# chriskery/slurm-bridge-operator

Measured on AMD Instinct MI355X. Metric: placements/sec + job×node fit evals/sec, 100k nodes×1M jobs, 1–8 MI355X, higher is better.
Workload: dtype int32

## Files before the change

include/fitgpu.h:

```cpp
#ifndef FITGPU_H
#define FITGPU_H

#include <stddef.h>
#include <stdint.h>

#ifdef __cplusplus
extern "C" {
#endif

#define FITGPU_ABI_VERSION 8

#define FIT_OK 0
#define FIT_E_INVAL (-1)
#define FIT_E_HIP (-2)
#define FIT_E_RCCL (-3)
#define FIT_E_OOM (-4)
#define FIT_E_NODEV (-5)
#define FIT_E_STATE (-6)
#define FIT_E_PARSE (-7)
#define FIT_E_UNLIMITED (-8)

#define FIT_UNPLACED (-1)
#define FIT_REJECTED (-2)

// ... 264 lines not shown
    int32_t need;
    int32_t evict_nodes;
    int32_t victims;
    int32_t top_prio;
    int32_t members;
    int32_t fit;
    int32_t able;
    int32_t outranked;
    int32_t reserved;
} fit_evict_k;
int fit_preempt_k(fit_ctx* ctx, int32_t j, const int32_t* cpu, const int32_t* mem, const int32_t* gpu,
                  const int32_t* wall, const uint16_t* part, const uint16_t* nodes_k ,
                  const int32_t* prio, int32_t kmax, fit_evict_k* out, int32_t* out_node ,
                  int32_t* out_victims );
int fit_preempt_k_device(fit_ctx* ctx, int32_t j, const int32_t* cpu, const int32_t* mem, const int32_t* gpu,
                         const int32_t* wall, const uint16_t* part, const uint16_t* nodes_k, const int32_t* prio,
                         int32_t kmax, fit_evict_k* out, int32_t* out_node, int32_t* out_victims);
int fit_preempt_k_ms(fit_ctx* ctx, double* ms);
int fit_preempt_k_message(const fit_evict_k* r, char* buf, int32_t buflen);

int fit_load_victims_tl(fit_ctx* ctx, const int32_t* vic_off , const int32_t* vic_prio,
                        const int32_t* vic_end, const int32_t* vic_cpu, const int32_t* vic_mem,
                        const int32_t* vic_gpu);
int fit_load_victims_tl_device(fit_ctx* ctx, const int32_t* vic_off, int64_t n_vic, const int32_t* vic_prio,
                               const int32_t* vic_end, const int32_t* vic_cpu, const int32_t* vic_mem,
                               const int32_t* vic_gpu);

int fit_preempt_tl(fit_ctx* ctx, int32_t j, const int32_t* cpu, const int32_t* mem, const int32_t* gpu,
                   const int32_t* wall, const uint16_t* part, const int32_t* prio, fit_evict* out);
int fit_preempt_tl_device(fit_ctx* ctx, int32_t j, const int32_t* cpu, const int32_t* mem, const int32_t* gpu,
                          const int32_t* wall, const uint16_t* part, const int32_t* prio, fit_evict* out);
int fit_preempt_tl_ms(fit_ctx* ctx, double* ms);

typedef struct {
    int64_t cpu, mem, gpu;
    int32_t nodes;
    int32_t max_cpu, max_mem, max_gpu;
} fit_free;
int fit_free_tl(fit_ctx* ctx, int32_t parts, fit_free* out );
int fit_free_tl_device(fit_ctx* ctx, int32_t parts, fit_free* out);
int fit_free_tl_ms(fit_ctx* ctx, double* ms);
int fit_free_message(const fit_free* r, char* buf, int32_t buflen);

int fit_parse_duration(const char* s, int64_t* out_ns);

typedef struct {
    int64_t nodes, mem_per_node, cpu_per_node, wall_ns;
} fit_resources;
int fit_parse_resources(const char* text, fit_resources* out);

typedef struct {
    int64_t cpus, memory, gpus, allo_cpus, allo_memory, allo_gpus;
} fit_node;
int fit_parse_nodes(const char* text, fit_node* out, int32_t cap);
int fit_parse_partition(const char* text, char* buf, int32_t buflen);
int fit_parse_partitions_names(const char* text, char* buf, int32_t buflen);

typedef struct {
    int64_t nodes, cpus_per_task, ntasks, ntasks_per_node, mem_per_cpu, wall_ns;
    char array[64];
} fit_job_resources;
int fit_extract_batch_resources(const char* script, fit_job_resources* out);
void fit_apply_spec(fit_job_resources* r, int64_t nodes, int64_t cpus_per_task,
                    int64_t mem_per_cpu, int64_t ntasks_per_node, const char* array,
                    int64_t ntasks);
int64_t fit_array_len(const char* array);
void fit_pod_request(const fit_job_resources* r, int64_t* cpu, int64_t* memory);
int fit_job_demand(const fit_job_resources* r, int32_t* cpu, int32_t* mem_mib, int32_t* wall_min,
                   uint16_t* nodes_k);
void fit_partition_capacity(const fit_node* nodes, int32_t n, int64_t* cpu, int64_t* memory,
                            int64_t* gpu, int64_t* pods);

int fit_ingest_nodes(const char* text, const char* partitions, int32_t np, int32_t cap,
                     int32_t* cpu_free, int32_t* mem_free, int32_t* gpu_free, int32_t* avail_min,
                     uint32_t* part_mask, char* names, int32_t names_len);
int fit_expand_hostlist(const char* expr, char* buf, int32_t buflen);
int fit_node_names(const char* entries, int32_t n, char* buf, int32_t buflen);

typedef struct fit_admitter fit_admitter;
typedef struct {
    int64_t priority;
    int32_t cpu;
    int32_t mem_mib;
    int32_t gpu;
    int32_t wall_min;
    uint16_t part;
    uint16_t nodes_k;
    uint16_t flags;
    uint16_t reserved;
} fit_admit_req;
#define FIT_REQ_ARRAY 1
typedef struct {
    int32_t node[FIT_MAX_K];
    int64_t batch;
    int32_t batch_jobs;
    int32_t order;
    int64_t ticket;
} fit_admit_res;
int fit_admitter_create(fit_ctx* ctx, int32_t max_batch, int32_t max_wait_us, fit_admitter** out);
int fit_admit(fit_admitter* a, const fit_admit_req* req, fit_admit_res* res);
int fit_admit_group(fit_admitter* a, const fit_admit_req* reqs, int32_t n, fit_admit_res* res);
int fit_admitter_load_nodes(fit_admitter* a, int32_t n, const int32_t* cpu_free,
                            const int32_t* mem_free, const int32_t* gpu_free,
                            const int32_t* avail_min, const uint32_t* part_mask);
#define FIT_TABLE_STATE 1
#define FIT_TABLE_PIN 2
typedef struct {
    int32_t n;
    const int32_t* cpu_free;
    const int32_t* mem_free;
    const int32_t* gpu_free;
    const int32_t* avail_min;
    const uint32_t* part_mask;
    const char* names;
    int32_t flags;
    int64_t generation;
} fit_node_table;
int fit_admitter_load_table(fit_admitter* a, const fit_node_table* t);
int64_t fit_admitter_generation(fit_admitter* a);
int fit_admitter_script(fit_admitter* a, const int64_t* tickets, int32_t n, const char* script,
                        char* out, int32_t outlen, int32_t* pinned);
int fit_admitter_partition_free(fit_admitter* a, int32_t p, int64_t* cpu, int64_t* mem_mib,
                                int64_t* gpu);
int fit_admitter_confirm(fit_admitter* a, int64_t ticket);
int fit_admitter_release(fit_admitter* a, int64_t ticket);
int fit_admitter_set_ttl(fit_admitter* a, int32_t loads);
int fit_admitter_explain(fit_admitter* a, const fit_admit_req* reqs, int32_t n, fit_why* out);
int fit_admitter_room(fit_admitter* a, const fit_admit_req* reqs, int32_t n, struct fit_room* out);
int fit_admitter_reservations(fit_admitter* a);
int fit_admitter_pending(fit_admitter* a);
void fit_admitter_destroy(fit_admitter* a);

typedef struct {
    const char* nodes;
    const char* cpus_per_task;
    const char* mem_per_cpu;
    const char* ntasks_per_node;
    const char* array;
    const char* ntasks;
} fit_pod_labels;
int fit_array_tasks(const char* array, int64_t* tasks, int64_t* max_running);
int32_t fit_set_max_array_size(int32_t n);
int fit_pod_demand(const fit_pod_labels* labels, const char* script, uint16_t part,
                   int64_t priority, fit_admit_req* out, int32_t cap);
int fit_script_with_nodelist(const char* script, const char* names, int32_t n_names,
                             const int32_t* node, int32_t k, char* out, int32_t outlen);
int fit_partition_limits(int64_t wall_time_s, int64_t cpu_per_node, int64_t mem_per_node,
                         int32_t* max_time_min, int32_t* max_cpus_per_node,
                         int32_t* max_mem_per_node);
int fit_node_columns(const fit_node* nodes, int32_t n, uint32_t part_mask, int32_t* cpu_free,
                     int32_t* mem_free, int32_t* gpu_free, int32_t* avail_min,
                     uint32_t* mask);

#ifdef __cplusplus
}
#endif
#endif
```

slurm-bridge-operator_amd/csrc/engine.cpp:

```cpp
#include <errno.h>
#include <fcntl.h>
#include <hip/hip_runtime_api.h>
#include <hip/hip_vector_types.h>
#include <rccl/rccl.h>
#include <sys/file.h>
#include <sys/stat.h>
#include <unistd.h>

#include <algorithm>
#include <chrono>
#include <cstdarg>
#include <cstdio>
#include <cstdlib>
#include <cstring>
#include <initializer_list>
#include <map>
#include <mutex>
#include <new>
#include <string>
#include <vector>

#include "../../include/fitgpu.h"
#include "fit_device.h"

// ... 33 lines not shown
            return fail(FIT_E_RCCL, "%s failed: %s", #expr, ncclGetErrorString(r_));        \
    } while (0)

template <class T>
struct DBuf {
    T* p = nullptr;
    size_t cap = 0;
    int ensure(size_t n) {
        if (n <= cap) return 0;
        if (p) (void)hipFree(p);
        p = nullptr;
        cap = 0;
        size_t want = std::max<size_t>(n, 64);
        if (hipMalloc(&p, want * sizeof(T)) != hipSuccess) {
            p = nullptr;
            return fail(FIT_E_OOM, "hipMalloc(%zu bytes) failed", want * sizeof(T));
        }
        cap = want;
        return 0;
    }
    void release() {
        if (p) (void)hipFree(p);
        p = nullptr;
        cap = 0;
    }
    DBuf() = default;
    DBuf(const DBuf&) = delete;
    DBuf& operator=(const DBuf&) = delete;
    ~DBuf() { release(); }
};

template <class T>
struct HBuf {
    T* p = nullptr;
    size_t cap = 0;
    int ensure(size_t n) {
        if (n <= cap) return 0;
        if (p) (void)hipHostFree(p);
        p = nullptr;
        cap = 0;
        size_t want = std::max<size_t>(n, 64);
        if (hipHostMalloc(&p, want * sizeof(T), hipHostMallocDefault) != hipSuccess) {
            p = nullptr;
            return fail(FIT_E_OOM, "hipHostMalloc(%zu bytes) failed", want * sizeof(T));
        }
        cap = want;
        return 0;
    }
    void release() {
        if (p) (void)hipHostFree(p);
        p = nullptr;
        cap = 0;
    }
    HBuf() = default;
    HBuf(const HBuf&) = delete;
    HBuf& operator=(const HBuf&) = delete;
    ~HBuf() { release(); }
};

template <class Row>
struct QueryBufs {
    DBuf<Row> out;
    DBuf<int32_t> bad;
    HBuf<Row> h;
    double ms = -1;
};

int find_root(int* par, int x) {
    while (par[x] != x) x = par[x] = par[par[x]];
    return x;
}

double now_ms() {
    using namespace std::chrono;
    return duration<double, std::milli>(steady_clock::now().time_since_epoch()).count();
}

struct DevArb {
    std::mutex mu;
    int fd = -1;
    std::string path;
};

constexpr const char* FIT_LOCK_DIR_DEFAULT = "/var/run/fitgpu";
int resolve_lock_dir(std::string& dir) {
    const char* e = getenv("FIT_LOCK_DIR");
    if (e && *e) {
        dir = e;
        return 0;
    }
    struct stat sb;
    if (stat(FIT_LOCK_DIR_DEFAULT, &sb) == 0 && S_ISDIR(sb.st_mode)) {
        dir = FIT_LOCK_DIR_DEFAULT;
        return 0;
    }
    dir = "/tmp";
    return 1;
}

DevArb* dev_arb(int device, std::string& err) {
    static std::mutex m;
    static std::map<int, DevArb*> tab;
    std::lock_guard<std::mutex> g(m);
    DevArb*& a = tab[device];
    if (!a) a = new DevArb();
    if (a->fd < 0) {
        char bus[64] = {0};
        if (hipDeviceGetPCIBusId(bus, sizeof bus, device) != hipSuccess) snprintf(bus, sizeof bus, "dev%d", device);
        for (char* q = bus; *q; ++q)
            if (*q == ':' || *q == '/') *q = '_';
        std::string dir;
        (void)resolve_lock_dir(dir);
        a->path = dir + "/fitgpu-" + bus + ".lock";
        a->fd = open(a->path.c_str(), O_RDWR | O_CREAT | O_CLOEXEC, 0666);
        if (a->fd >= 0) (void)fchmod(a->fd, 0666);
        else a->fd = open(a->path.c_str(), O_RDONLY | O_CLOEXEC);
        if (a->fd < 0) {
            err = a->path + ": " + strerror(errno);
            return nullptr;
        }
    }
    return a;
}

struct ArbGuard {
    DevArb* a = nullptr;
    double waited_ms = 0;
    int take(int device) {
        const double t0 = now_ms();
        std::string err;
        DevArb* d = dev_arb(device, err);
        if (!d) return fail(FIT_E_STATE, "device lock %s (set FIT_LOCK_DIR to a writable directory)", err.c_str());
        d->mu.lock();
        int r;
        do r = flock(d->fd, LOCK_EX);
        while (r != 0 && errno == EINTR);
        if (r != 0) {
            d->mu.unlock();
            return fail(FIT_E_STATE, "flock %s: %s", d->path.c_str(), strerror(errno));
        }
        a = d;
        waited_ms = now_ms() - t0;
        return 0;
    }
    ~ArbGuard() {
        if (!a) return;
        (void)flock(a->fd, LOCK_UN);
        a->mu.unlock();
    }
};

}

struct CtxHandles {
    ncclComm_t comm = nullptr;
    hipStream_t st = nullptr;
    hipEvent_t ev[6] = {};
    hipStream_t st2 = nullptr;
    hipEvent_t ev_join = nullptr;
    unsigned* resident = nullptr;
    CtxHandles() = default;
    CtxHandles(const CtxHandles&) = delete;
    CtxHandles& operator=(const CtxHandles&) = delete;
    ~CtxHandles() {
        for (auto& e : ev)
            if (e) (void)hipEventDestroy(e);
        if (ev_join) (void)hipEventDestroy(ev_join);
        if (resident) (void)hipHostFree(resident);
        if (st2) (void)hipStreamDestroy(st2);
        if (st) (void)hipStreamDestroy(st);
        if (comm) (void)ncclCommDestroy(comm);
    }
};

struct fit_ctx : CtxHandles {
    int device = 0;
    int rank = 0, world = 1;
    int shard_mode = FIT_SHARD_AUTO;
    fit_exchange_fn xchg = nullptr;
    void* xchg_user = nullptr;
    HBuf<uint8_t> h_x;
    DBuf<uint64_t> xcount;
    bool force_coll = false;
    bool collective() const { return world > 1 || force_coll; }
    bool persistent = true;
    int32_t small_batch = 2048;
    int32_t small_direct = 128;
    bool small_args = true, sync_spin = true;
    int cls_mode = 3;
    int32_t last_multi = 0;
    bool cls_nodes_ok = false;
    int32_t cls_maxn = 0;
    DBuf<int16_t> jcls;
    DBuf<uint8_t> cls_tab;
    DBuf<int4> cls_dem;
    DBuf<int32_t> cls_n;
    DBuf<unsigned> cls_err;
    HBuf<int32_t> h_cls_n;
    HBuf<unsigned> h_cls_err;
    DBuf<int32_t> small_placed;
    HBuf<int32_t> h_small;
    DBuf<uint8_t> jpack;
    HBuf<uint8_t> h_jpack;
    QueryBufs<fit_why> ex;
    QueryBufs<fit_eta> wh;
    QueryBufs<struct fit_room> rm;
    QueryBufs<fit_eta_k> wk;
    DBuf<int32_t> wk_node, wk_diff;
    HBuf<int32_t> h_wk_node;
    DBuf<unsigned long long> wk_top;
    DBuf<int32_t> ptlk_cnt;
    HBuf<int32_t> h_ptlk;
    DBuf<int32_t> tlr_node, tlr_start, tlr_state, tlr_inv, tlr_cnt, tlr_first, tlr_fill, tlr_touched, tlr_flag, tlr_g;
    DBuf<TlWin> tlr_win;
    DBuf<unsigned long long> tlr_tot;
    HBuf<int32_t> h_tlr_g;
    HBuf<unsigned long long> h_tlr_tot;
    double utl_ms = -1, htl_ms = -1;
    DBuf<int32_t> atl_tc, atl_tm, atl_tg, atl_g;
    HBuf<int32_t> h_atl;
    double atl_ms = -1;
    DBuf<int64_t> free_acc;
    DBuf<fit_free> free_rows;
    double free_ms = -1;
    DBuf<int32_t> vs_off, vs_prio, vs_cpu, vs_mem, vs_gpu, vic_bad, voff;
    HBuf<int32_t> h_vic_bad;
    DBuf<VicEnt> vent;
    bool have_vic = false;
    QueryBufs<fit_evict> pe;
    DBuf<int32_t> pe_prio;
    HBuf<int32_t> h_pe_prio;
    DBuf<uint4> pe_part;
    QueryBufs<fit_evict_k> pk;
    DBuf<int32_t> pk_node, pk_vic;
    HBuf<int32_t> h_pk_pick;
    DBuf<int32_t> vs_end, vtl_off;
    DBuf<VicTl> vtl_ent;
    bool have_vtl = false;
    int32_t vtl_shift = 0;
    QueryBufs<fit_evict> pt;
    int cus = 256;
    DBuf<uint8_t> ectl, ering;
    DBuf<CompState> ecs;
    DBuf<CompOut> eco;
    DBuf<int64_t> ebusy;
    HBuf<CompState> h_ecs;
    HBuf<CompOut> h_eco;
    HBuf<int64_t> h_ebusy;
    HBuf<uint32_t> h_err;
    HBuf<TripRec> h_trip;
    DBuf<NodeRec> rec_bak;
    unsigned wd_ticks = 1000000000u;
    HBuf<uint64_t> h_count;
    int wmin = 256, wmax = 8192;

    int32_t n = 0;
    int32_t nn = 0;
    int ncomp = 0;
    int comp_of_part[32];
    std::vector<int32_t> nb;
    DBuf<NodeRec> rec;
    DBuf<int32_t> col_cpu, col_mem, col_gpu, col_av, perm;
    DBuf<uint32_t> col_mask;
    DBuf<int32_t> rb_cpu, rb_mem, rb_gpu;
    std::vector<uint32_t> h_mask;
    std::vector<int32_t> h_perm;
    bool have_nodes = false;
    int64_t loads = 0;

    int32_t np = 0;
    int32_t ptab[128];
    DBuf<int32_t> d_ptab;

    DBuf<int32_t> jcpu, jmem, jgpu, jwall, out, jl, jpk;
    DBuf<uint16_t> jpart, jk;
    DBuf<int8_t> jcomp;
    DBuf<int32_t> jmin;
    DBuf<uint64_t> cand, bnd;
    DBuf<JobRec> wjob;
    DBuf<CompPlan> plan;
    DBuf<CommitResult> res;
    HBuf<CompPlan> h_plan;
    HBuf<CommitResult> h_res;
    DBuf<int32_t> jls;
    HBuf<int32_t> h_jls;

    int32_t tl_slots = 0, tl_slot_min = 0;
    bool have_tl = false;
    DBuf<Seg> slab;
    DBuf<TlHdr> tlhdr;
    DBuf<int32_t> outs, rel_off, rel_slot, rel_cpu, rel_mem, rel_gpu;
    DBuf<uint32_t> tl_err;
    HBuf<uint32_t> h_tl_err;
};

namespace {

int build_ptab(fit_ctx* c) {
    for (int p = 0; p < 32; ++p) c->ptab[96 + p] = c->comp_of_part[p];
    if (c->d_ptab.ensure(128)) return FIT_E_OOM;
    HIP_TRY(hipMemcpyAsync(c->d_ptab.p, c->ptab, sizeof c->ptab, hipMemcpyHostToDevice, c->st));
    return 0;
}

int load_nodes_common(fit_ctx* c, int32_t n) {
    int par[32];
    for (int i = 0; i < 32; ++i) par[i] = i;
    bool used[32] = {false};
    for (int32_t x = 0; x < n; ++x) {
        uint32_t m = c->h_mask[x];
        if (!m) continue;
        int lo = __builtin_ctz(m);
        for (uint32_t r = m; r; r &= r - 1) {
            int b = __builtin_ctz(r);
            used[b] = true;
            int ra = find_root(par, lo), rb = find_root(par, b);
            if (ra != rb) par[std::max(ra, rb)] = std::min(ra, rb);
        }
    }
    int root_comp[32];
    for (int i = 0; i < 32; ++i) root_comp[i] = -1;
    c->ncomp = 0;
    for (int p = 0; p < 32; ++p) {
        c->comp_of_part[p] = -1;
        if (!used[p]) continue;
        int r = find_root(par, p);
        if (root_comp[r] < 0) root_comp[r] = c->ncomp++;
        c->comp_of_part[p] = root_comp[r];
    }
    c->nb.assign(c->ncomp + 1, 0);
    for (int32_t x = 0; x < n; ++x)
        if (c->h_mask[x]) c->nb[c->comp_of_part[__builtin_ctz(c->h_mask[x])] + 1]++;
    for (int k = 0; k < c->ncomp; ++k) {
        if (c->nb[k + 1] > MAX_COMPONENT_NODES)
            return fail(FIT_E_INVAL, "partition component %d has %d nodes (limit %d)", k,
                        c->nb[k + 1], MAX_COMPONENT_NODES);
        c->nb[k + 1] += c->nb[k];
    }
    c->nn = c->nb[c->ncomp];
    {
        int parts_of[32] = {0};
        for (int p = 0; p < 32; ++p)
            if (c->comp_of_part[p] >= 0) ++parts_of[c->comp_of_part[p]];
        c->cls_nodes_ok = c->ncomp > 0 && c->ncomp <= 32;
        c->cls_maxn = 0;
        for (int k = 0; k < c->ncomp; ++k) {
            const int32_t nk = c->nb[k + 1] - c->nb[k];
            c->cls_maxn = std::max(c->cls_maxn, nk);
            if (parts_of[k] != 1) c->cls_nodes_ok = false;
        }
        if (c->cls_maxn > class_max_nodes() || class_lds_bytes(c->cls_maxn) > 160 * 1024)
            c->cls_nodes_ok = false;
    }
    std::vector<int32_t> fill(c->nb.begin(), c->nb.end() - 1), perm(std::max(c->nn, 1));
    for (int32_t x = 0; x < n; ++x)
        if (c->h_mask[x]) perm[fill[c->comp_of_part[__builtin_ctz(c->h_mask[x])]]++] = x;
    if (c->perm.ensure(std::max(c->nn, 1)) || c->rec.ensure(std::max(c->nn, 1))) return FIT_E_OOM;
    HIP_TRY(hipMemcpyAsync(c->perm.p, perm.data(), sizeof(int32_t) * c->nn, hipMemcpyHostToDevice,
                           c->st));
    HIP_TRY(launch_gather_nodes(c->st, c->col_cpu.p, c->col_mem.p, c->col_gpu.p, c->col_av.p,
                                c->col_mask.p, c->perm.p, c->nn, c->rec.p));
    int rc = build_ptab(c);
    if (rc) return rc;
    HIP_TRY(hipStreamSynchronize(c->st));
    perm.resize(c->nn);
    c->h_perm.swap(perm);
    c->n = n;
    c->have_nodes = true;
    c->have_tl = false;
    ++c->loads;
    return 0;
}

int alloc_cols(fit_ctx* c, int32_t n) {
    size_t m = std::max<int32_t>(n, 1);
    if (c->col_cpu.ensure(m) || c->col_mem.ensure(m) || c->col_gpu.ensure(m) ||
        c->col_av.ensure(m) || c->col_mask.ensure(m))
        return FIT_E_OOM;
    return 0;
}

int xchg(fit_ctx* c, int op, void* dbuf, int64_t count) {
    if (!c->collective() || count == 0) return 0;
    if (!c->xchg) {
        switch (op) {
            case FIT_XCHG_ALLGATHER_U64: {
                uint64_t* b = static_cast<uint64_t*>(dbuf);
                NCCL_TRY(ncclAllGather(b + (size_t)c->rank * count, b, count, ncclUint64, c->comm,
                                       c->st));
                return 0;
            }
            case FIT_XCHG_MIN_U64:
                NCCL_TRY(ncclAllReduce(dbuf, dbuf, count, ncclUint64, ncclMin, c->comm, c->st));
                return 0;
            case FIT_XCHG_MAX_I32:
                NCCL_TRY(ncclAllReduce(dbuf, dbuf, count, ncclInt32, ncclMax, c->comm, c->st));
                return 0;
            case FIT_XCHG_MIN_I32:
                NCCL_TRY(ncclAllReduce(dbuf, dbuf, count, ncclInt32, ncclMin, c->comm, c->st));
                return 0;
        }
        return fail(FIT_E_INVAL, "exchange op %d", op);
    }
    const size_t elem = (op == FIT_XCHG_ALLGATHER_U64 || op == FIT_XCHG_MIN_U64) ? 8 : 4;
    const size_t bytes = elem * (size_t)count * (op == FIT_XCHG_ALLGATHER_U64 ? c->world : 1);
    if (c->h_x.ensure(bytes)) return FIT_E_OOM;
    HIP_TRY(hipMemcpyAsync(c->h_x.p, dbuf, bytes, hipMemcpyDeviceToHost, c->st));
    HIP_TRY(hipStreamSynchronize(c->st));
    if (c->xchg(c->xchg_user, op, c->h_x.p, count) != 0)
        return fail(FIT_E_RCCL, "host exchange op %d failed", op);
    HIP_TRY(hipMemcpyAsync(dbuf, c->h_x.p, bytes, hipMemcpyHostToDevice, c->st));
    return 0;
}

const char* trip_site_name(unsigned s) {
    switch (s) {
        case TRIP_WORKER_RING: return "scan worker waiting for a task";
        case TRIP_ROUND_START: return "committer waiting for the round before last";
        case TRIP_HELPER_TILE: return "commit helper waiting for a scan tile";
        case TRIP_HELPER_SNAP: return "commit helper waiting for the decider";
        case TRIP_DECIDER_REC: return "decider waiting for a helper record";
        case TRIP_SINGLE_TILE: return "single-wave commit waiting for a scan tile";
        case TRIP_NO_PROGRESS: return "round resolved no job";
        case TRIP_NO_KERNEL: return "no scan kernel for the key count";
        default: return "unknown";
    }
}

int trip_error(fit_ctx* c, const char* engine) {
    const TripRec& t = *c->h_trip.p;
    return fail(FIT_E_HIP,
                "%s watchdog tripped (code %u): site %u (%s), component %u, round %u, arg %u, "
                "block %u, q_head %u, q_tail %u, pubt %u, tdone %u / need %u, waited %.3f ms, "
                "%.3f ms into the launch (deadline %.3f ms)",
                engine, c->h_err.p[0], t.site, trip_site_name(t.site), t.comp, t.round, t.arg,
                t.block, t.q_head, t.q_tail, t.pubt, t.tdone, t.need, t.waited / 1e5, t.when / 1e5,
                c->wd_ticks / 1e5);
}
struct EngineComps {
    std::vector<int> comps;
    int nc = 0;
    int32_t maxnodes = 0;
    int64_t wcap = 0;
};

EngineComps engine_comps(fit_ctx* c, const std::vector<int32_t>& jb, const std::vector<char>& owned) {
    EngineComps E;
    for (int k = 0; k < c->ncomp; ++k)
        if (owned[k] && jb[k + 1] > jb[k]) {
            E.comps.push_back(k);
            E.maxnodes = std::max(E.maxnodes, c->nb[k + 1] - c->nb[k]);
        }
    E.nc = (int)E.comps.size();
    E.wcap = std::min(c->wmax, 8192);
    return E;
}

int fold_comp_out(fit_ctx* c, const std::vector<int32_t>& jb, const std::vector<int>& comps, fit_stats& S) {
    double commit_max = 0;
    for (size_t i = 0; i < comps.size(); ++i) {
        const CompOut& o = c->h_eco.p[i];
        const int k = comps[i];
        if (o.done_jobs != jb[k + 1] - jb[k])
            return fail(FIT_E_HIP, "component %d resolved %lld of %d jobs", k, (long long)o.done_jobs,
                        jb[k + 1] - jb[k]);
        S.placed += o.placed;
        S.rounds = std::max<int64_t>(S.rounds, o.rounds);
        S.stops_rescan += o.stops_rescan;
        S.stops_dirty += o.stops_dirty;
        commit_max = std::max(commit_max, o.t_commit / 1e5);
    }
    S.ms_commit += commit_max;
    return 0;
}

template <class Slice>
int engine_plan(fit_ctx* c, const std::vector<int32_t>& jb, const EngineComps& E, int64_t keys, Slice slice) {
    const int nc = E.nc;
    const int64_t wcap = E.wcap, per_comp_cand = wcap * keys;
    if (c->ecs.ensure(nc) || c->eco.ensure(nc) || c->h_ecs.ensure(nc) || c->h_eco.ensure(nc) ||
        c->plan.ensure(2 * nc) ||
        c->cand.ensure((size_t)2 * nc * per_comp_cand + (size_t)2 * nc * PAIR_AREA) ||
        c->bnd.ensure((size_t)2 * nc * wcap) || c->wjob.ensure((size_t)2 * nc * wcap) ||
        c->ectl.ensure(engine_ctl_bytes()) || c->ering.ensure(engine_ring_bytes()) ||
        c->h_err.ensure(4))
        return FIT_E_OOM;
    if ((int64_t)2 * nc * per_comp_cand + (int64_t)2 * nc * PAIR_AREA > INT32_MAX)
        return fail(FIT_E_INVAL, "candidate buffer exceeds 2^31 entries (%d components)", nc);
    int32_t max_slices = 1;
    for (int i = 0; i < nc; ++i) {
        const int k = E.comps[i];
        CompState& s = c->h_ecs.p[i];
        s.nb = s.sb = c->nb[k];
        s.ne = s.se = c->nb[k + 1];
        slice(s.ne - s.nb, s);
        max_slices = std::max(max_slices, s.nslice);
        s.jstart = jb[k];
        s.jend = jb[k + 1];
        s.cand_off = (int64_t)i * per_comp_cand;
        s.slot0 = (int32_t)(i * wcap);
        s.cand_alt = (int64_t)(nc + i) * per_comp_cand;
        s.slot_alt = (int32_t)((nc + i) * wcap);
        s.pair_off = (int32_t)(2 * nc * per_comp_cand + (int64_t)2 * i * PAIR_AREA);
        s.wmin = std::min(c->wmin, (int)wcap);
        s.wmax = (int32_t)wcap;
    }
    if ((int64_t)2 * ring_comps(nc) * ((wcap + SCAN_JOBS - 1) / SCAN_JOBS + 1) * max_slices >
        (int64_t)engine_ring_tasks())
        return fail(FIT_E_INVAL, "task ring too small: %d components x %lld tiles x %d slices",
                    nc, (long long)((wcap + SCAN_JOBS - 1) / SCAN_JOBS), max_slices);
    return 0;
}

template <class Launch, class Settle>
int engine_launch(fit_ctx* c, const std::vector<int32_t>& jb, const EngineComps& E, int workers,
                  const char* name, Launch launch, Settle settle, fit_stats& S) {
    const int nc = E.nc;
    hipStream_t st = c->st;
    if (c->ebusy.ensure(2 * workers) || c->h_ebusy.ensure(2 * workers) || c->h_trip.ensure(1))
        return FIT_E_OOM;
    HIP_TRY(hipMemcpyAsync(c->ecs.p, c->h_ecs.p, sizeof(CompState) * nc, hipMemcpyHostToDevice, st));
    HIP_TRY(hipMemsetAsync(c->ectl.p, 0, engine_ctl_bytes(), st));
    HIP_TRY(hipMemsetAsync(c->ering.p, 0, engine_ring_bytes(), st));
    HIP_TRY(hipMemsetAsync(c->bnd.p, 0xff, sizeof(uint64_t) * 2 * nc * E.wcap, st));
    {
        ArbGuard arb;
        int rc = arb.take(c->device);
        if (rc) return rc;
        S.ms_arb_wait = arb.waited_ms;
        HIP_TRY(hipEventRecord(c->ev[0], st));
        rc = launch();
        if (rc) return rc;
        HIP_TRY(hipEventRecord(c->ev[1], st));
        HIP_TRY(hipMemcpyAsync(c->h_eco.p, c->eco.p, sizeof(CompOut) * nc, hipMemcpyDeviceToHost, st));
        HIP_TRY(hipMemcpyAsync(c->h_ebusy.p, c->ebusy.p, sizeof(int64_t) * 2 * workers,
                               hipMemcpyDeviceToHost, st));
        HIP_TRY(hipMemcpyAsync(c->h_err.p, c->ectl.p + engine_ctl_error_offset(), 4, hipMemcpyDeviceToHost, st));
        HIP_TRY(hipMemcpyAsync(c->h_trip.p, c->ectl.p + engine_ctl_trip_offset(), sizeof(TripRec),
                               hipMemcpyDeviceToHost, st));
        HIP_TRY(hipStreamSynchronize(st));
    }
    if (int rc = settle(c->h_err.p[0] ? trip_error(c, name) : 0)) return rc;
    float ms = 0.f;
    HIP_TRY(hipEventElapsedTime(&ms, c->ev[0], c->ev[1]));
    S.ms_device += ms;
    int64_t busy = 0;
    for (int i = 0; i < workers; ++i) {
        busy += c->h_ebusy.p[2 * i];
        S.evals += c->h_ebusy.p[2 * i + 1];
    }
    S.ms_scan += busy / 1e5 / workers;
    return fold_comp_out(c, jb, E.comps, S);
}

int run_persistent(fit_ctx* c, const std::vector<int32_t>& jb, const std::vector<char>& owned,
                   const int32_t* cpu, const int32_t* mem, const int32_t* gpu, const int32_t* wall,
                   const uint16_t* part, const uint16_t* nk, int32_t* out, int32_t kmax,
                   fit_stats& S) {
    hipStream_t st = c->st;
    const EngineComps E = engine_comps(c, jb, owned);
    const int nc = E.nc;
    if (nc == 0) return 0;
    int sub_target = 256, ks_min = 4;
    if (const char* e = getenv("FIT_SUB_TARGET")) sub_target = std::max(MIN_SUB, atoi(e));
    if (const char* e = getenv("FIT_KS_MIN")) ks_min = std::max(2, std::min(KS, atoi(e)));
    while (ks_min < kmax) ks_min *= 2;
    int rc = engine_plan(c, jb, E, (int64_t)MAX_SLICES * KS, [&](int32_t len, CompState& s) {
        for (s.ks = KS;; s.ks /= 2) {
            const int slices = MAX_SLICES * KS / s.ks;
            s.sub = std::max(MIN_SUB, (len + SCAN_WAVES * slices - 1) / (SCAN_WAVES * slices));
            s.nslice = std::max(1, (len + SCAN_WAVES * s.sub - 1) / (SCAN_WAVES * s.sub));
            if (s.sub <= sub_target || s.ks / 2 < ks_min) break;
        }
    });
    if (rc) return rc;
    size_t lds = engine_lds_bytes(E.maxnodes);
    if (const char* e = getenv("FIT_ENGINE_LDS_MIN")) lds = std::max(lds, (size_t)atol(e));
    int per_cu = engine_blocks_per_cu(lds);
    if (per_cu <= 0) return fail(FIT_E_HIP, "k_engine does not fit on a CU (lds %zu)", lds);
    int workers = std::max(8, std::max(1, per_cu - 1) * c->cus - nc);
    if (const char* e = getenv("FIT_WORKERS")) workers = std::max(1, atoi(e));
    EngineCompIds ids;
    memset(&ids, 0, sizeof ids);
    for (int i = 0; i < nc; ++i) ids.id[i] = (int8_t)E.comps[i];
    static const bool no_backup = getenv("FIT_REC_BACKUP") && atoi(getenv("FIT_REC_BACKUP")) == 0;
    if (c->rec_bak.ensure(std::max(c->nn, 1))) return FIT_E_OOM;
    if (!no_backup)
        HIP_TRY(hipMemcpyAsync(c->rec_bak.p, c->rec.p, sizeof(NodeRec) * c->nn, hipMemcpyDeviceToDevice, st));
    return engine_launch(
        c, jb, E, workers, "placement engine",
        [&]() -> int {
            HIP_TRY(launch_engine(nc + workers, lds, st, c->ectl.p, c->ering.p, c->ecs.p, c->eco.p,
                                  c->plan.p, nc, c->rec.p, c->jl.p, cpu, mem, gpu, wall, part, nk,
                                  c->cand.p, c->bnd.p, c->wjob.p, out, kmax, c->ebusy.p, c->jpk.p,
                                  c->wd_ticks, c->jmin.p, ids));
            return 0;
        },
        [&](int trip) -> int {
            if (!trip) return 0;
            if (no_backup) {
                c->have_nodes = c->have_tl = false;
                return trip;
            }
            HIP_TRY(hipMemcpyAsync(c->rec.p, c->rec_bak.p, sizeof(NodeRec) * c->nn, hipMemcpyDeviceToDevice, st));
            HIP_TRY(hipStreamSynchronize(st));
            return trip;
        },
        S);
}

int run_class(fit_ctx* c, int32_t J, const std::vector<int32_t>& jb, const std::vector<char>& owned,
              const int32_t* wall, const uint16_t* nk, int32_t* out, int32_t kmax, fit_stats& S) {
    const int C = c->ncomp;
    hipStream_t st = c->st;
    if (c->eco.ensure(C) || c->h_eco.ensure(C) || c->cls_err.ensure(1) || c->h_cls_err.ensure(1) ||
        c->rec_bak.ensure(std::max(c->nn, 1)))
        return FIT_E_OOM;
    int32_t* jbd = c->jls.p + joblists_scratch_ints(J) + 2;
    HIP_TRY(hipMemsetAsync(c->cls_err.p, 0, sizeof(unsigned), st));
    HIP_TRY(hipMemcpyAsync(c->rec_bak.p, c->rec.p, sizeof(NodeRec) * c->nn, hipMemcpyDeviceToDevice, st));
    const size_t lds = class_lds_bytes(c->cls_maxn);
    HIP_TRY(hipEventRecord(c->ev[0], st));
    uint32_t own = 0;
    for (int k = 0; k < C; ++k)
        if (owned[k]) own |= 1u << k;
    HIP_TRY(launch_class(st, C, lds, c->rec.p, c->nb.data(), own, jbd, c->jl.p, wall, nk, c->jcls.p,
                         c->cls_dem.p, c->cls_n.p, kmax, out, c->eco.p, c->cls_err.p));
    HIP_TRY(hipEventRecord(c->ev[1], st));
    HIP_TRY(launch_class_out(st, out, (int64_t)J * kmax, c->rec.p));
    HIP_TRY(hipMemcpyAsync(c->h_eco.p, c->eco.p, sizeof(CompOut) * C, hipMemcpyDeviceToHost, st));
    HIP_TRY(hipMemcpyAsync(c->h_cls_err.p, c->cls_err.p, sizeof(unsigned), hipMemcpyDeviceToHost, st));
    HIP_TRY(hipStreamSynchronize(st));
    if (c->h_cls_err.p[0]) {
        HIP_TRY(hipMemcpyAsync(c->rec.p, c->rec_bak.p, sizeof(NodeRec) * c->nn, hipMemcpyDeviceToDevice, st));
        HIP_TRY(hipStreamSynchronize(st));
        return fail(FIT_E_HIP, "class engine: an in-block wait exceeded its bound (error %u)", c->h_cls_err.p[0]);
    }
    float ms = 0.f;
    HIP_TRY(hipEventElapsedTime(&ms, c->ev[0], c->ev[1]));
    S.ms_device += ms;
    double commit_max = 0;
    for (int k = 0; k < C; ++k) {
        if (!owned[k]) continue;
        const CompOut& o = c->h_eco.p[k];
        if (o.done_jobs != jb[k + 1] - jb[k])
            return fail(FIT_E_HIP, "component %d resolved %lld of %d jobs", k, (long long)o.done_jobs,
                        jb[k + 1] - jb[k]);
        S.placed += o.placed;
        S.evals += o.evals;
        S.rounds = std::max<int64_t>(S.rounds, o.rounds);
        S.stops_rescan += o.stops_rescan;
        S.stops_dirty += o.stops_dirty;
        commit_max = std::max(commit_max, o.t_commit / 1e5);
    }
    S.ms_commit += commit_max;
    S.engine = 3;
    return 0;
}

int enqueue_classify(fit_ctx* c, int32_t J, const int32_t* cpu, const int32_t* mem, const int32_t* gpu,
                     const uint16_t* part) {
    const int C = c->ncomp;
    hipStream_t st = c->st;
    const size_t ts = (size_t)C * class_table_slots() * class_slot_bytes();
    if (c->jcls.ensure(std::max(J, 1)) || c->cls_tab.ensure(ts) || c->cls_dem.ensure((size_t)C * class_max()) ||
        c->cls_n.ensure(C) || c->h_cls_n.ensure(C))
        return FIT_E_OOM;
    HIP_TRY(hipMemsetAsync(c->cls_tab.p, 0, ts, st));
    HIP_TRY(hipMemsetAsync(c->cls_n.p, 0, sizeof(int32_t) * C, st));
    HIP_TRY(launch_classify(st, c->jcomp.p, cpu, mem, gpu, part, J, c->cls_tab.p, c->cls_dem.p, c->cls_n.p,
                            c->jcls.p));
    HIP_TRY(hipMemcpyAsync(c->h_cls_n.p, c->cls_n.p, sizeof(int32_t) * C, hipMemcpyDeviceToHost, st));
    return 0;
}

bool classes_fit(const fit_ctx* c) {
    for (int k = 0; k < c->ncomp; ++k)
        if (c->h_cls_n.p[k] > class_max()) return false;
    return true;
}

int build_job_lists(fit_ctx* c, int32_t J, fit_stats& S, std::vector<int32_t>& jb,
                    const int32_t* cpu = nullptr, const int32_t* mem = nullptr, const int32_t* gpu = nullptr,
                    const uint16_t* part = nullptr, bool classify = false, bool* cls_ok = nullptr) {
    const int C = c->ncomp;
    hipStream_t st = c->st;
    if (c->jl.ensure(std::max(J, 1)) || c->jpk.ensure(J + 1) ||
        c->jls.ensure(std::max<size_t>(joblists_scratch_ints(J), 1) + 2 * (C + 1) + 2) ||
        c->h_jls.ensure(2 * (C + 1) + 2))
        return FIT_E_OOM;
    int32_t* g = c->jls.p + joblists_scratch_ints(J);
    int32_t* jbd = g + 2;
    int32_t* mbd = jbd + C + 1;
    HIP_TRY(launch_joblists(st, c->jcomp.p, J, C, c->jls.p, g, jbd, mbd, c->jl.p, c->jpk.p));
    HIP_TRY(hipMemcpyAsync(c->h_jls.p, g, sizeof(int32_t) * (2 * (C + 1) + 2), hipMemcpyDeviceToHost, st));
    if (classify) {
        const int rc = enqueue_classify(c, J, cpu, mem, gpu, part);
        if (rc) return rc;
    }
    HIP_TRY(hipStreamSynchronize(st));
    if (c->h_jls.p[1]) return fail(FIT_E_INVAL, "a job has a negative demand or nodes_k > kmax");
    if (cls_ok) *cls_ok = classify && classes_fit(c);
    S.rejected = c->h_jls.p[0];
    jb.assign(c->h_jls.p + 2, c->h_jls.p + 2 + C + 1);
    c->last_multi = c->h_jls.p[2 + C + 1 + C];
    for (int k = 0; k < C; ++k) S.useful_evals += (int64_t)(jb[k + 1] - jb[k]) * c->n;
    return 0;
}

int classify_jobs(fit_ctx* c, int32_t J, const int32_t* cpu, const int32_t* mem, const int32_t* gpu,
                  const uint16_t* part, bool* cls_ok) {
    const int rc = enqueue_classify(c, J, cpu, mem, gpu, part);
    if (rc) return rc;
    HIP_TRY(hipStreamSynchronize(c->st));
    *cls_ok = classes_fit(c);
    return 0;
}

hipError_t sync_small(fit_ctx* c) {
    if (c->sync_spin) {
        hipError_t e = hipEventRecord(c->ev[2], c->st);
        if (e != hipSuccess) return e;
        const double t0 = now_ms();
        while ((e = hipEventQuery(c->ev[2])) == hipErrorNotReady && now_ms() - t0 < 2.0) {
        }
        if (e != hipErrorNotReady) return e;
    }
    return hipStreamSynchronize(c->st);
}

int place_direct(fit_ctx* c, int32_t J, const int32_t* cpu, const int32_t* mem, const int32_t* gpu,
                 const int32_t* wall, const uint16_t* part, const uint16_t* nk, int32_t kmax,
                 int32_t* out, int32_t* h_out, fit_stats& S, const SmallBatch* hb = nullptr) {
    const int C = c->ncomp;
    const int G = std::max(C, 1);
    hipStream_t st = c->st;
    const size_t rows = (size_t)J * kmax;
    const size_t nback = (h_out ? rows : 0) + 2 + G;
    if (c->small_placed.ensure(2 + G) || c->h_small.ensure(nback)) return FIT_E_OOM;
    int32_t* stat = h_out ? out + rows : c->small_placed.p;
    SmallComps sc;
    for (int k = 0; k <= 32; ++k) sc.nb[k] = c->nb[std::min(k, C)];
    HIP_TRY(hipEventRecord(c->ev[0], st));
    if (hb)
        HIP_TRY(launch_small_args(st, C, c->rec.p, sc, c->d_ptab.p, c->np, *hb, nk != nullptr, J, kmax, out, stat));
    else
        HIP_TRY(launch_small(st, C, c->rec.p, sc, c->d_ptab.p, c->np, cpu, mem, gpu, wall, part, nk, J, kmax,
                             out, stat));
    HIP_TRY(hipEventRecord(c->ev[1], st));
    HIP_TRY(hipMemcpyAsync(c->h_small.p, h_out ? out : stat, sizeof(int32_t) * nback, hipMemcpyDeviceToHost,
                           st));
    HIP_TRY(sync_small(c));
    const int32_t* hs = c->h_small.p + (h_out ? rows : 0);
    if (hs[1]) return fail(FIT_E_INVAL, "a job has a negative demand or nodes_k > kmax");
    if (h_out) memcpy(h_out, c->h_small.p, sizeof(int32_t) * rows);
    S.rejected = hs[0];
    for (int k = 0; k < C; ++k) S.placed += hs[2 + k];
    float ms = 0.f;
    HIP_TRY(hipEventElapsedTime(&ms, c->ev[0], c->ev[1]));
    S.ms_device = S.ms_commit = ms;
    S.rounds = C > 0 && J > S.rejected ? 1 : 0;
    S.components = C;
    S.engine = 2;
    return 0;
}

template <class Scan, class Commit>
int run_rounds(fit_ctx* c, const std::vector<int32_t>& jb, const std::vector<char>& owned, bool node_sharded,
               int keys, int slices, int min_sub, Scan scan, Commit commit, fit_stats& S) {
    const int C = c->ncomp;
    hipStream_t st = c->st;
    const int shards = node_sharded ? c->world : 1;
    const int srank = node_sharded ? c->rank : 0;
    std::vector<int32_t> cur(jb.begin(), jb.end() - 1), win(C, c->wmin);
    if (c->plan.ensure(C + 1) || c->res.ensure(C + 1) || c->h_plan.ensure(C + 1) ||
        c->h_res.ensure(C + 1))
        return FIT_E_OOM;
    float ms;
    for (;;) {
        int64_t blocks = 0, slots = 0, cand_n = 0, evals = 0;
        int epl = 1;
        int32_t maxlen = 0;
        for (int k = 0; k < C; ++k) {
            CompPlan& P = c->h_plan.p[k];
            memset(&P, 0, sizeof P);
            P.nb = c->nb[k];
            P.ne = c->nb[k + 1];
            const int32_t len = P.ne - P.nb;
            const int32_t per = (len + shards - 1) / shards;
            P.sb = std::min(P.ne, P.nb + per * srank);
            P.se = std::min(P.ne, P.sb + per);
            P.ks = keys;
            P.sub = std::max(min_sub, (per + SCAN_WAVES * slices - 1) / (SCAN_WAVES * slices));
            P.nslice = std::max(1, (per + SCAN_WAVES * P.sub - 1) / (SCAN_WAVES * P.sub));
            epl = std::max(epl, (shards * P.nslice * keys + 63) / 64);
            P.jbase = cur[k];
            P.w = owned[k] ? std::min(win[k], jb[k + 1] - cur[k]) : 0;
            P.blk0 = (int32_t)blocks;
            P.cand_off = cand_n;
            P.slot0 = (int32_t)slots;
            if (P.w > 0) {
                blocks += (int64_t)((P.w + SCAN_JOBS - 1) / SCAN_JOBS) * P.nslice;
                cand_n += (int64_t)P.w * P.nslice * keys;
                slots += P.w;
                evals += (int64_t)P.w * (P.se - P.sb);
                maxlen = std::max(maxlen, len);
            }
        }
        if (slots == 0) break;
        S.rounds++;
        S.evals += evals;
        if (c->cand.ensure((size_t)cand_n * shards) || c->bnd.ensure(slots) ||
            c->wjob.ensure(slots))
            return FIT_E_OOM;
        HIP_TRY(hipMemcpyAsync(c->plan.p, c->h_plan.p, sizeof(CompPlan) * C, hipMemcpyHostToDevice,
                               st));
        HIP_TRY(hipMemsetAsync(c->bnd.p, 0xff, sizeof(uint64_t) * slots, st));
        HIP_TRY(hipEventRecord(c->ev[0], st));
        HIP_TRY(scan((int)blocks, c->cand.p + (size_t)srank * cand_n));
        HIP_TRY(hipEventRecord(c->ev[1], st));
        if (node_sharded) {
            int rc = xchg(c, FIT_XCHG_ALLGATHER_U64, c->cand.p, cand_n);
            if (!rc) rc = xchg(c, FIT_XCHG_MIN_U64, c->bnd.p, slots);
            if (rc) return rc;
        }
        HIP_TRY(hipEventRecord(c->ev[2], st));
        HIP_TRY(commit(epl, maxlen, cand_n, shards));
        HIP_TRY(hipEventRecord(c->ev[3], st));
        HIP_TRY(hipMemcpyAsync(c->h_res.p, c->res.p, sizeof(CommitResult) * C,
                               hipMemcpyDeviceToHost, st));
        HIP_TRY(hipStreamSynchronize(st));
        HIP_TRY(hipEventElapsedTime(&ms, c->ev[0], c->ev[1]));
        S.ms_scan += ms;
        HIP_TRY(hipEventElapsedTime(&ms, c->ev[1], c->ev[2]));
        S.ms_exchange += ms;
        HIP_TRY(hipEventElapsedTime(&ms, c->ev[2], c->ev[3]));
        S.ms_commit += ms;
        for (int k = 0; k < C; ++k) {
            const CompPlan& P = c->h_plan.p[k];
            if (P.w == 0) continue;
            const CommitResult& R = c->h_res.p[k];
            if (R.done < 0 || R.done > P.w)
                return fail(FIT_E_HIP, "commit returned %d of window %d", R.done, P.w);
            cur[k] += R.done;
            S.placed += R.placed;
            if (R.stop == 1) S.stops_rescan++;
            if (R.stop == 2) S.stops_dirty++;
            const int32_t nw = R.stop ? 2 * R.done : 2 * P.w;
            win[k] = std::max(c->wmin, std::min(c->wmax, nw));
        }
    }
    S.ms_device = S.ms_scan + S.ms_exchange + S.ms_commit;
    return 0;
}

int place_impl(fit_ctx* c, int32_t J, const int32_t* cpu, const int32_t* mem, const int32_t* gpu,
               const int32_t* wall, const uint16_t* part, const uint16_t* nk, int32_t kmax,
               int32_t* out, fit_stats* stats, int32_t* h_out = nullptr, bool* h_out_done = nullptr,
               const SmallBatch* hb = nullptr) {
    const double t0 = now_ms();
    fit_stats S;
    memset(&S, 0, sizeof S);
    S.jobs = J;
    hipStream_t st = c->st;
    if (J <= c->small_direct && !c->collective()) {
        const int rc = place_direct(c, J, cpu, mem, gpu, wall, part, nk, kmax, out, h_out, S, hb);
        if (rc) return rc;
        if (h_out_done) *h_out_done = h_out != nullptr;
        S.unplaced = J - S.placed - S.rejected;
        S.ms_total = now_ms() - t0;
        if (stats) *stats = S;
        return 0;
    }
    if (c->jcomp.ensure(std::max(J, 1)) || c->jmin.ensure(3 * ENGINE_MAXC)) return FIT_E_OOM;
    HIP_TRY(hipMemsetAsync(c->jmin.p, JMIN_FILL, sizeof(int32_t) * 3 * ENGINE_MAXC, st));
    HIP_TRY(launch_prefilter(st, cpu, mem, gpu, wall, part, nk, J, kmax, c->d_ptab.p, c->np, out,
                             c->jcomp.p, c->jmin.p));
    const int C = c->ncomp;
    std::vector<int32_t> jb;
    const int pre_mode = !c->collective() ? 0
                         : (c->shard_mode == FIT_SHARD_AUTO ? (C >= c->world ? FIT_SHARD_COMPONENTS : FIT_SHARD_NODES)
                                                            : c->shard_mode);
    const bool cls_able = c->cls_nodes_ok && pre_mode != FIT_SHARD_NODES;
    const bool try_cls = (c->cls_mode == 1 || c->cls_mode == 2) && cls_able && (c->cls_mode == 2 || J > c->small_batch);
    bool cls_ok = false;
    int rc0 = build_job_lists(c, J, S, jb, cpu, mem, gpu, part, try_cls, &cls_ok);
    if (rc0) return rc0;
    const int32_t live = J - S.rejected;
    if (c->cls_mode == 3 && cls_able && live > c->small_batch && 2 * (int64_t)c->last_multi >= live) {
        rc0 = classify_jobs(c, J, cpu, mem, gpu, part, &cls_ok);
        if (rc0) return rc0;
    }
    const bool use_cls = cls_ok && (c->cls_mode == 2 || live > c->small_batch);

    int mode = 0;
    std::vector<char> owned(C, 1);
    if (c->collective()) {
        mode = c->shard_mode;
        if (mode == FIT_SHARD_AUTO) mode = C >= c->world ? FIT_SHARD_COMPONENTS : FIT_SHARD_NODES;
        if (mode == FIT_SHARD_COMPONENTS) {
            std::vector<int> order(C);
            for (int k = 0; k < C; ++k) order[k] = k;
            auto work = [&](int k) { return (int64_t)(jb[k + 1] - jb[k]) * (c->nb[k + 1] - c->nb[k]); };
            std::stable_sort(order.begin(), order.end(), [&](int a, int b) { return work(a) > work(b); });
            std::vector<int64_t> load(c->world, 0);
            for (int k : order) {
                int r = (int)(std::min_element(load.begin(), load.end()) - load.begin());
                load[r] += work(k) + 1;
                owned[k] = r == c->rank;
            }
        }
    }
    S.shard_mode = mode;
    S.components = C;
    const bool node_sharded = mode == FIT_SHARD_NODES;

    const bool small = J - S.rejected <= c->small_batch;
    if (use_cls) {
        int rc = run_class(c, J, jb, owned, wall, nk, out, kmax, S);
        if (rc) return rc;
    } else if (c->persistent && !node_sharded && !small) {
        int rc = run_persistent(c, jb, owned, cpu, mem, gpu, wall, part, nk, out, kmax, S);
        if (rc) return rc;
        S.engine = 1;
    } else {
        int rc = run_rounds(
            c, jb, owned, node_sharded, KS, MAX_SLICES, MIN_SUB,
            [&](int blocks, uint64_t* cand) {
                return launch_scan(blocks, st, c->rec.p, c->jl.p, cpu, mem, gpu, wall, part, nk, c->plan.p, C,
                                   cand, c->bnd.p, c->wjob.p);
            },
            [&](int epl, int32_t maxlen, int64_t cand_n, int shards) {
                return launch_commit(C, epl, (size_t)((maxlen + 31) / 32) * 4, st, c->rec.p, c->plan.p,
                                     c->cand.p, cand_n, shards, c->bnd.p, c->wjob.p, out, kmax, c->res.p);
            },
            S);
        if (rc) return rc;
    }
    if (mode == FIT_SHARD_COMPONENTS) {
        int rc = xchg(c, FIT_XCHG_MAX_I32, out, (int64_t)J * kmax);
        if (!rc) rc = xchg(c, FIT_XCHG_MIN_I32, c->rec.p, (int64_t)c->nn * 8);
        if (rc) return rc;
        if (c->xcount.ensure(c->world) || c->h_count.ensure(c->world)) return FIT_E_OOM;
        c->h_count.p[c->rank] = (uint64_t)S.placed;
        HIP_TRY(hipMemcpyAsync(c->xcount.p + c->rank, c->h_count.p + c->rank, 8,
                               hipMemcpyHostToDevice, st));
        rc = xchg(c, FIT_XCHG_ALLGATHER_U64, c->xcount.p, 1);
        if (rc) return rc;
        HIP_TRY(hipMemcpyAsync(c->h_count.p, c->xcount.p, 8 * c->world, hipMemcpyDeviceToHost, st));
        HIP_TRY(hipStreamSynchronize(st));
        S.placed = 0;
        for (int r = 0; r < c->world; ++r) S.placed += (int64_t)c->h_count.p[r];
    }
    S.unplaced = J - S.placed - S.rejected;
    S.ms_total = now_ms() - t0;
    if (stats) *stats = S;
    return 0;
}

int run_persistent_tl(fit_ctx* c, const std::vector<int32_t>& jb, const int32_t* cpu,
                      const int32_t* mem, const int32_t* gpu, const int32_t* wall,
                      const uint16_t* part, int32_t* out, int32_t* outs, fit_stats& S) {
    hipStream_t st = c->st;
    const EngineComps E = engine_comps(c, jb, std::vector<char>(c->ncomp, 1));
    const int nc = E.nc;
    if (nc == 0) return 0;
    const int R = engine_tl_runs(E.maxnodes);
    if (R < 1) return fail(FIT_E_INVAL, "partition component of %d nodes is too large for the "
                                        "timeline engine's LDS", E.maxnodes);
    int slices = TL_SLICES, tl_min_sub = TL_MIN_SUB;
    if (const char* e = getenv("FIT_TL_SLICES")) slices = std::max(1, std::min(atoi(e), TL_SLICES));
    if (const char* e = getenv("FIT_TL_MINSUB")) tl_min_sub = std::max(1, atoi(e));
    int rc = engine_plan(c, jb, E, (int64_t)slices * TL_KS, [&](int32_t len, CompState& s) {
        s.ks = TL_KS;
        s.sub = std::max(tl_min_sub, (len + SCAN_WAVES * slices - 1) / (SCAN_WAVES * slices));
        s.nslice = std::max(1, (len + SCAN_WAVES * s.sub - 1) / (SCAN_WAVES * s.sub));
    });
    if (rc) return rc;
    const size_t lds = engine_tl_lds_bytes(E.maxnodes);
    bool split = FIT_TL_SPLIT_DEF != 0;
    if (const char* e = getenv("FIT_TL_SPLIT")) split = atoi(e) != 0;
    const size_t lds_w = split ? engine_tl_scan_lds_bytes() : lds;
    const int per_cu = engine_tl_blocks_per_cu(lds, split ? 1 : 0);
    if (per_cu <= 0) return fail(FIT_E_HIP, "k_engine_tl does not fit on a CU (lds %zu)", lds);
    const int per_cu_w = split ? engine_tl_blocks_per_cu(lds_w, 2) : per_cu;
    if (per_cu_w <= 0) return fail(FIT_E_HIP, "k_engine_tl workers do not fit on a CU");
    int workers = split ? std::max(8, per_cu_w * std::max(1, c->cus - nc)) : std::max(8, per_cu * c->cus - nc);
    if (const char* e = getenv("FIT_WORKERS")) workers = std::max(1, atoi(e));
    if (split && !c->st2) {
        if (hipStreamCreateWithFlags(&c->st2, hipStreamNonBlocking) != hipSuccess ||
            hipEventCreateWithFlags(&c->ev_join, hipEventDisableTiming) != hipSuccess ||
            hipHostMalloc(&c->resident, 64, hipHostMallocMapped | hipHostMallocCoherent) != hipSuccess)
            return fail(FIT_E_HIP, "split launch: stream / event / mapped flag");
    }
    auto launch = [&](int blocks, size_t l, hipStream_t s, int mode, unsigned* dres) {
        return launch_engine_tl(blocks, l, s, c->ectl.p, c->ering.p, c->ecs.p, c->eco.p, c->plan.p, nc,
                                c->slab.p, c->tlhdr.p, c->jl.p, cpu, mem, gpu, wall, part, c->cand.p,
                                c->bnd.p, c->wjob.p, c->perm.p, out, outs, c->tl_slots, c->tl_slot_min, R,
                                c->ebusy.p, mode, dres, c->wd_ticks);
    };
    bool resident_late = false;
    rc = engine_launch(
        c, jb, E, workers, "timeline engine",
        [&]() -> int {
            if (!split) {
                HIP_TRY(launch(nc + workers, lds, st, 0, nullptr));
                return 0;
            }
            __atomic_store_n(c->resident, 0u, __ATOMIC_RELEASE);
            unsigned* dres = nullptr;
            HIP_TRY(hipHostGetDevicePointer(reinterpret_cast<void**>(&dres), c->resident, 0));
            HIP_TRY(launch(nc, lds, st, 1, dres));
            const auto t0 = std::chrono::steady_clock::now();
            while (__atomic_load_n(c->resident, __ATOMIC_ACQUIRE) < (unsigned)nc) {
                if (std::chrono::steady_clock::now() - t0 > std::chrono::seconds(10)) {
                    resident_late = true;
                    break;
                }
            }
            HIP_TRY(hipStreamWaitEvent(c->st2, c->ev[0], 0));
            HIP_TRY(launch(workers, lds_w, c->st2, 2, nullptr));
            HIP_TRY(hipEventRecord(c->ev_join, c->st2));
            HIP_TRY(hipStreamWaitEvent(st, c->ev_join, 0));
            return 0;
        },
        [&](int trip) -> int {
            if (trip || resident_late) c->have_tl = false;
            if (trip) return trip;
            if (resident_late) return fail(FIT_E_HIP, "timeline engine: committer blocks not resident after 10 s");
            return 0;
        },
        S);
    if (rc) return rc;
    S.engine = 1;
    return 0;
}

int place_tl_impl(fit_ctx* c, int32_t J, const int32_t* cpu, const int32_t* mem,
                  const int32_t* gpu, const int32_t* wall, const uint16_t* part, int32_t* out,
                  int32_t* outs, fit_stats* stats) {
    const double t0 = now_ms();
    fit_stats S;
    memset(&S, 0, sizeof S);
    S.jobs = J;
    hipStream_t st = c->st;
    if (c->jcomp.ensure(std::max(J, 1))) return FIT_E_OOM;
    HIP_TRY(launch_prefilter(st, cpu, mem, gpu, wall, part, nullptr, J, 1, c->d_ptab.p, c->np, out,
                             c->jcomp.p));
    if (J > 0) HIP_TRY(hipMemsetAsync(outs, 0xff, sizeof(int32_t) * J, st));
    const int C = c->ncomp;
    std::vector<int32_t> jb;
    int rc = build_job_lists(c, J, S, jb);
    if (rc) return rc;
    const bool node_sharded = c->collective();
    S.shard_mode = node_sharded ? FIT_SHARD_NODES : 0;
    S.components = C;
    if (c->persistent && !node_sharded && J - S.rejected > c->small_batch) {
        rc = run_persistent_tl(c, jb, cpu, mem, gpu, wall, part, out, outs, S);
        if (rc) return rc;
        S.unplaced = J - S.placed - S.rejected;
        S.ms_total = now_ms() - t0;
        if (stats) *stats = S;
        return 0;
    }
    int32_t maxlen = 1;
    for (int k = 0; k < C; ++k) maxlen = std::max(maxlen, c->nb[k + 1] - c->nb[k]);
    const size_t lds = commit_tl_lds_bytes(maxlen);
    const int runs = commit_tl_runs(maxlen);
    const int shards = node_sharded ? c->world : 1;
    int slices = std::max(1, TL_SLICES / shards), tl_min_sub = TL_MIN_SUB;
    if (const char* e = getenv("FIT_TL_SLICES")) slices = std::max(1, std::min(atoi(e), 512 / (TL_KS * shards)));
    if (const char* e = getenv("FIT_TL_MINSUB")) tl_min_sub = std::max(1, atoi(e));
    if (runs < 1)
        return fail(FIT_E_INVAL, "partition component of %d nodes is too large for the timeline "
                                 "commit's LDS", maxlen);
// ... 26 lines not shown
constexpr int32_t kExplainSortJobs = 256;

struct JobCols {
    const int32_t *cpu, *mem, *gpu, *wall;
    const uint16_t *part, *nk;
};

ExplainComps query_comps(const fit_ctx* c) {
    ExplainComps ec;
    ec.ncomp = c->ncomp;
    for (int k = 0; k <= 32; ++k) ec.nb[k] = c->nb[std::min(k, c->ncomp)];
    return ec;
}
int query_joblist(fit_ctx* c, int32_t J, int32_t threshold, const int32_t** jl, const int32_t** live) {
    const int C = c->ncomp;
    *jl = *live = nullptr;
    if (J <= threshold || C <= 1) return 0;
    if (c->jl.ensure(J) || c->jpk.ensure(J + 1) ||
        c->jls.ensure(std::max<size_t>(joblists_scratch_ints(J), 1) + 2 * (C + 1) + 2))
        return FIT_E_OOM;
    int32_t* g = c->jls.p + joblists_scratch_ints(J);
    int32_t* jbd = g + 2;
    HIP_TRY(launch_joblists(c->st, c->jcomp.p, J, C, c->jls.p, g, jbd, jbd + C + 1, c->jl.p, c->jpk.p));
    *jl = c->jl.p;
    *live = jbd + C;
    return 0;
}

template <class Classify, class Walk>
int query_impl(fit_ctx* c, int32_t J, int32_t* bad, Classify classify, Walk walk) {
    if (c->jcomp.ensure(std::max(J, 1))) return FIT_E_OOM;
    HIP_TRY(hipMemsetAsync(bad, 0, sizeof(int32_t), c->st));
    HIP_TRY(classify());
    const int32_t *jl, *live;
    if (const int rc = query_joblist(c, J, kExplainSortJobs, &jl, &live)) return rc;
    HIP_TRY(walk(query_comps(c), jl, live));
    return 0;
}

int explain_impl(fit_ctx* c, int32_t J, const JobCols& d, fit_why* out, int32_t* bad) {
    return query_impl(
        c, J, bad,
        [&] {
            return launch_explain_classify(c->st, c->d_ptab.p, c->np, d.cpu, d.mem, d.gpu, d.wall, d.part, d.nk, J,
                                           out, c->jcomp.p, bad);
        },
        [&](const ExplainComps& ec, const int32_t* jl, const int32_t* live) {
            return launch_explain(c->st, c->rec.p, ec, d.cpu, d.mem, d.gpu, d.wall, d.part, J, c->jcomp.p, jl, live,
                                  explain_slices(J, c->cls_maxn, c->cus), out);
        });
}

static_assert(ETA_NOW == FIT_ETA_NOW && ETA_PARTITION == FIT_ETA_PARTITION && ETA_LIMIT_TIME == FIT_ETA_LIMIT_TIME &&
                  ETA_LIMIT_CPUS == FIT_ETA_LIMIT_CPUS && ETA_LIMIT_MEM == FIT_ETA_LIMIT_MEM &&
                  ETA_NO_NODES == FIT_ETA_NO_NODES && ETA_LATER == FIT_ETA_LATER && ETA_HORIZON == FIT_ETA_HORIZON,
              "fit_device.h and fitgpu.h disagree");
static_assert(sizeof(fit_eta) == 32, "fit_eta is 32 bytes");
constexpr int kWhenMinNodes = 4;

int when_impl(fit_ctx* c, int32_t J, const JobCols& d, fit_eta* out, int32_t* bad) {
    return query_impl(
        c, J, bad,
        [&] {
            return launch_when_classify(c->st, c->d_ptab.p, c->np, d.cpu, d.mem, d.gpu, d.wall, d.part, J,
                                        c->tl_slot_min, out, c->jcomp.p, bad);
        },
        [&](const ExplainComps& ec, const int32_t* jl, const int32_t* live) {
            return launch_when(c->st, c->tlhdr.p, c->slab.p, ec, c->tl_slots, c->tl_slot_min, d.cpu, d.mem, d.gpu,
                               d.part, J, c->jcomp.p, jl, live,
                               explain_slices(J, c->cls_maxn, c->cus, kWhenMinNodes), out);
        });
}

static_assert(ROOM_SOME == FIT_ROOM_SOME && ROOM_PARTITION == FIT_ROOM_PARTITION &&
                  ROOM_LIMIT_TIME == FIT_ROOM_LIMIT_TIME && ROOM_LIMIT_CPUS == FIT_ROOM_LIMIT_CPUS &&
                  ROOM_LIMIT_MEM == FIT_ROOM_LIMIT_MEM && ROOM_NO_NODES == FIT_ROOM_NO_NODES &&
                  ROOM_NONE == FIT_ROOM_NONE,
              "fit_device.h and fitgpu.h disagree");
static_assert(sizeof(struct fit_room) == 40 && offsetof(struct fit_room, copies) == 16 &&
                  offsetof(struct fit_room, best_node) == 24,
              "fit_room is 40 bytes, copies at 16");
static_assert(FIT_ROOM_UNBOUNDED == INT32_MAX, "FIT_ROOM_UNBOUNDED is INT32_MAX");

int room_impl(fit_ctx* c, int32_t J, const JobCols& d, struct fit_room* out, int32_t* bad) {
    return query_impl(
        c, J, bad,
        [&] {
            return launch_room_classify(c->st, c->d_ptab.p, c->np, d.cpu, d.mem, d.gpu, d.wall, d.part, J, out,
                                        c->jcomp.p, bad);
        },
        [&](const ExplainComps& ec, const int32_t* jl, const int32_t* live) {
            return launch_room(c->st, c->rec.p, ec, d.cpu, d.mem, d.gpu, d.wall, d.part, J, c->jcomp.p, jl, live,
                               explain_slices(J, c->cls_maxn, c->cus), out);
        });
}

static_assert(PRE_FITS == FIT_PRE_FITS && PRE_PARTITION == FIT_PRE_PARTITION && PRE_LIMIT_TIME == FIT_PRE_LIMIT_TIME &&
                  PRE_LIMIT_CPUS == FIT_PRE_LIMIT_CPUS && PRE_LIMIT_MEM == FIT_PRE_LIMIT_MEM &&
                  PRE_NO_NODES == FIT_PRE_NO_NODES && PRE_EVICT == FIT_PRE_EVICT && PRE_NONE == FIT_PRE_NONE,
              "fit_device.h and fitgpu.h disagree");
static_assert(FIT_PRE_PARTITION == FIT_WHY_PARTITION && FIT_PRE_LIMIT_TIME == FIT_WHY_LIMIT_TIME &&
                  FIT_PRE_LIMIT_CPUS == FIT_WHY_LIMIT_CPUS && FIT_PRE_LIMIT_MEM == FIT_WHY_LIMIT_MEM &&
                  FIT_PRE_NO_NODES == FIT_WHY_NO_NODES,
              "codes 1..5 of FIT_PRE_* are FIT_WHY_*'s");
static_assert(sizeof(fit_evict) == 32 && offsetof(fit_evict, code) == 0 && offsetof(fit_evict, node) == 4 &&
                  offsetof(fit_evict, victims) == 8 && offsetof(fit_evict, top_prio) == 12 &&
                  offsetof(fit_evict, members) == 16 && offsetof(fit_evict, fit) == 20 &&
                  offsetof(fit_evict, able) == 24 && offsetof(fit_evict, outranked) == 28,
              "fit_evict is 32 bytes: code, node, victims, top_prio, then the four counters");

int preempt_impl(fit_ctx* c, int32_t J, const JobCols& d, const int32_t* prio, fit_evict* out, int32_t* bad) {
    const int S = preempt_slices(J, c->cls_maxn, c->cus);
    if (c->pe_part.ensure(preempt_partials(J, S))) return FIT_E_OOM;
    return query_impl(
        c, J, bad,
        [&] {
            return launch_preempt_classify(c->st, c->d_ptab.p, c->np, c->ncomp, d.cpu, d.mem, d.gpu, d.wall, d.part, J,
                                           out, c->jcomp.p, bad);
        },
        [&](const ExplainComps& ec, const int32_t* jl, const int32_t* live) {
            return launch_preempt(c->st, c->rec.p, c->voff.p, c->vent.p, ec, d.cpu, d.mem, d.gpu, d.wall, d.part, prio,
                                  J, c->jcomp.p, jl, live, S, c->pe_part.p, out);
        });
}

static_assert(sizeof(fit_evict_k) == 40 && offsetof(fit_evict_k, code) == 0 && offsetof(fit_evict_k, need) == 4 &&
                  offsetof(fit_evict_k, evict_nodes) == 8 && offsetof(fit_evict_k, victims) == 12 &&
                  offsetof(fit_evict_k, top_prio) == 16 && offsetof(fit_evict_k, members) == 20 &&
                  offsetof(fit_evict_k, fit) == 24 && offsetof(fit_evict_k, able) == 28 &&
                  offsetof(fit_evict_k, outranked) == 32 && offsetof(fit_evict_k, reserved) == 36,
              "fit_evict_k is 40 bytes: code, need, evict_nodes, victims, top_prio, the four counters, reserved");

int preempt_k_impl(fit_ctx* c, int32_t J, const JobCols& d, const int32_t* prio, int32_t kmax, fit_evict_k* out,
                   int32_t* out_node, int32_t* out_vic, int32_t* bad) {
    const int S = preempt_slices(J, c->cls_maxn, c->cus);
    if (c->pe_part.ensure(preempt_k_partials(J, S, kmax))) return FIT_E_OOM;
    return query_impl(
        c, J, bad,
        [&] {
            return launch_preempt_k_classify(c->st, c->d_ptab.p, c->np, c->ncomp, d.cpu, d.mem, d.gpu, d.wall, d.part,
                                             d.nk, kmax, J, out, out_node, out_vic, c->jcomp.p, bad);
        },
        [&](const ExplainComps& ec, const int32_t* jl, const int32_t* live) {
            return launch_preempt_k(c->st, c->rec.p, c->voff.p, c->vent.p, ec, d.cpu, d.mem, d.gpu, d.wall, d.part,
                                    prio, kmax, J, c->jcomp.p, jl, live, S, c->pe_part.p, out, out_node, out_vic);
        });
}

int load_victims_impl(fit_ctx* c, const int32_t* h_off, const int32_t* off, const int32_t* prio, const int32_t* cpu,
                      const int32_t* mem, const int32_t* gpu) {
    std::vector<int32_t> hv((size_t)c->nn + 1, 0);
    if (h_off)
        for (int32_t i = 0; i < c->nn; ++i) {
            const int32_t x = c->h_perm[i];
            hv[i + 1] = hv[i] + (h_off[x + 1] - h_off[x]);
        }
    c->have_vic = false;
    if (c->voff.ensure(hv.size()) || c->vent.ensure(std::max<int32_t>(hv[c->nn], 1))) return FIT_E_OOM;
    HIP_TRY(hipMemcpyAsync(c->voff.p, hv.data(), sizeof(int32_t) * hv.size(), hipMemcpyHostToDevice, c->st));
    if (hv[c->nn] > 0)
        HIP_TRY(launch_vic_build(c->st, off, prio, cpu, mem, gpu, c->perm.p, c->nn, c->voff.p, c->vent.p));
    HIP_TRY(hipStreamSynchronize(c->st));
    c->have_vic = true;
    return 0;
}

int check_victims_state(fit_ctx* c) {
    if (!c) return fail(FIT_E_INVAL, "null ctx");
    if (!c->have_nodes) return fail(FIT_E_STATE, "fit_load_nodes not called");
    if (c->collective())
        return fail(FIT_E_STATE, "fit_load_victims on a sharded context (world > 1 / FIT_FLAG_COLLECTIVES)");
    return 0;
}

int preempt_tl_impl(fit_ctx* c, int32_t J, const JobCols& d, const int32_t* prio, fit_evict* out, int32_t* bad) {
    const int S = preempt_slices(J, c->cls_maxn, c->cus);
    if (c->pe_part.ensure(preempt_partials(J, S))) return FIT_E_OOM;
    return query_impl(
        c, J, bad,
        [&] {
            return launch_preempt_classify(c->st, c->d_ptab.p, c->np, c->ncomp, d.cpu, d.mem, d.gpu, d.wall, d.part, J,
                                           out, c->jcomp.p, bad);
        },
        [&](const ExplainComps& ec, const int32_t* jl, const int32_t* live) {
            return launch_preempt_tl(c->st, c->tlhdr.p, c->slab.p, c->vtl_off.p, c->vtl_ent.p, ec, c->tl_slots,
                                     c->tl_slot_min, c->vtl_shift, d.cpu, d.mem, d.gpu, d.wall, d.part, prio, J,
                                     c->jcomp.p, jl, live, S, c->pe_part.p, out);
        });
}

int load_victims_tl_impl(fit_ctx* c, const int32_t* h_off, const int32_t* off, const int32_t* prio, const int32_t* end,
                         const int32_t* cpu, const int32_t* mem, const int32_t* gpu) {
    std::vector<int32_t> hv((size_t)c->nn + 1, 0);
    if (h_off)
        for (int32_t i = 0; i < c->nn; ++i) {
            const int32_t x = c->h_perm[i];
            hv[i + 1] = hv[i] + (h_off[x + 1] - h_off[x]);
        }
    c->have_vtl = false;
    if (c->vtl_off.ensure(hv.size()) || c->vtl_ent.ensure(std::max<int32_t>(hv[c->nn], 1))) return FIT_E_OOM;
    HIP_TRY(hipMemcpyAsync(c->vtl_off.p, hv.data(), sizeof(int32_t) * hv.size(), hipMemcpyHostToDevice, c->st));
    if (hv[c->nn] > 0)
        HIP_TRY(launch_vtl_build(c->st, off, prio, end, cpu, mem, gpu, c->perm.p, c->nn, c->vtl_off.p, c->vtl_ent.p));
    HIP_TRY(hipStreamSynchronize(c->st));
    c->vtl_shift = 0;
    c->have_vtl = true;
    return 0;
}

int check_victims_tl_state(fit_ctx* c) {
    if (!c) return fail(FIT_E_INVAL, "null ctx");
    if (!c->have_nodes) return fail(FIT_E_STATE, "fit_load_nodes not called");
    if (c->collective())
        return fail(FIT_E_STATE, "fit_load_victims_tl on a sharded context (world > 1 / FIT_FLAG_COLLECTIVES)");
    if (!c->have_tl) return fail(FIT_E_STATE, "fit_load_timeline not called");
    return 0;
}

static_assert(sizeof(fit_eta_k) == 40 && offsetof(fit_eta_k, members) == 20 && offsetof(fit_eta_k, reserved) == 36,
              "fit_eta_k is 40 bytes");

int whenk_slices(int32_t nj, int32_t maxn, int cus) {
    const int64_t groups = ((int64_t)std::max(nj, 1) + WHENK_GROUP - 1) / WHENK_GROUP;
    const int64_t want = std::max<int64_t>(2, ((int64_t)cus * 4 + groups - 1) / groups);
    const int64_t fit = ((int64_t)maxn + 255) / 256;
    return (int)std::max<int64_t>(1, std::min<int64_t>({want, fit, (int64_t)WHENK_MAX_SLICES}));
}

int when_k_impl(fit_ctx* c, int32_t J, const JobCols& d, int32_t kmax, fit_eta_k* out, int32_t* out_node,
                int32_t* bad) {
    hipStream_t st = c->st;
    const int C = c->ncomp, H = c->tl_slots;
    const int32_t chunk = std::min<int32_t>(J, WHENK_CHUNK);
    const int S = whenk_slices(chunk, c->cls_maxn, c->cus);
    if (c->jcomp.ensure(std::max(J, 1)) || c->wk_diff.ensure((size_t)chunk * (H + 1)) ||
        c->wk_top.ensure((size_t)chunk * S * WHENK_KEYS))
        return FIT_E_OOM;
    HIP_TRY(hipMemsetAsync(bad, 0, sizeof(int32_t), st));
    HIP_TRY(launch_whenk_classify(st, c->d_ptab.p, c->np, d.cpu, d.mem, d.gpu, d.wall, d.part, d.nk, kmax, J,
                                  c->tl_slot_min, out, out_node, c->jcomp.p, bad));
    if (C < 1) return 0;
    const int32_t *jl, *live;
    if (const int rc = query_joblist(c, J, WHENK_GROUP, &jl, &live)) return rc;
    const ExplainComps ec = query_comps(c);
    for (int32_t t0 = 0; t0 < J; t0 += WHENK_CHUNK)
        HIP_TRY(launch_whenk_chunk(st, c->tlhdr.p, c->slab.p, ec, H, c->tl_slot_min, d.cpu, d.mem, d.gpu, d.wall,
                                   d.part, t0, std::min<int32_t>(J - t0, WHENK_CHUNK), J, kmax, c->jcomp.p, jl, live, S,
                                   c->wk_diff.p, c->wk_top.p, out, out_node));
    return 0;
}

struct TlBack {
    void* host = nullptr;
    const void* dev = nullptr;
    size_t bytes = 0;
};
constexpr int kTlNoWrite = 1;

template <class Check, class Verdict, class Write>
int tl_write_impl(fit_ctx* c, const char* name, TlBack flags, Check check, Verdict verdict, TlBack result, Write write,
                  double* dev_ms) {
    hipStream_t st = c->st;
    float ms = 0.f;
    *dev_ms = 0;
    if (flags.bytes) {
        HIP_TRY(hipEventRecord(c->ev[0], st));
        HIP_TRY(check());
        HIP_TRY(hipEventRecord(c->ev[1], st));
        HIP_TRY(hipMemcpyAsync(flags.host, flags.dev, flags.bytes, hipMemcpyDeviceToHost, st));
        HIP_TRY(hipStreamSynchronize(st));
        const int rc = verdict();
        if (rc < 0) return rc;
        HIP_TRY(hipEventElapsedTime(&ms, c->ev[0], c->ev[1]));
        *dev_ms = ms;
        if (rc == kTlNoWrite) return 0;
    }
    HIP_TRY(hipEventRecord(c->ev[3], st));
    int kept = 0;
    hipError_t e = write(kept);
    if (e != hipSuccess && kept) return kept;
    if (e == hipSuccess) e = hipEventRecord(c->ev[4], st);
    if (e == hipSuccess && result.bytes)
        e = hipMemcpyAsync(result.host, result.dev, result.bytes, hipMemcpyDeviceToHost, st);
    if (e == hipSuccess) e = hipStreamSynchronize(st);
    if (e == hipSuccess) e = hipEventElapsedTime(&ms, c->ev[3], c->ev[4]);
    if (e != hipSuccess) {
        c->have_tl = false;
        return fail(FIT_E_HIP, "%s: %s; the timeline is dropped (fit_load_timeline)", name, hipGetErrorString(e));
    }
    *dev_ms += ms;
    return 0;
}

int place_tl_k_impl(fit_ctx* c, int32_t J, const JobCols& d, int32_t kmax, int32_t* out, int32_t* outs,
                    fit_stats* stats) {
    const double t0 = now_ms();
    fit_stats S;
    memset(&S, 0, sizeof S);
    S.jobs = J;
    S.engine = 4;
    const int C = c->ncomp, H = c->tl_slots;
    S.components = C;
    hipStream_t st = c->st;
    const size_t ns = 2 * ((size_t)C + 1) + 2;
    if (c->jcomp.ensure(J) || c->jl.ensure(J) || c->jpk.ensure((size_t)J + 1) ||
        c->jls.ensure(std::max<size_t>(joblists_scratch_ints(J), 1) + ns) || c->h_jls.ensure(ns) ||
        c->ptlk_cnt.ensure(1) || c->h_ptlk.ensure(1))
        return FIT_E_OOM;
    int32_t* g = c->jls.p + joblists_scratch_ints(J);
    int32_t* jbd = g + 2;
    int32_t maxlen = 0;
    int32_t chunk = PTLK_CHUNK;
    if (const char* e = getenv("FIT_PTLK_CHUNK")) chunk = std::max(1, std::min(atoi(e), PTLK_CHUNK));
    const int rc = tl_write_impl(
        c, "fit_place_tl_k", {c->h_jls.p, g, sizeof(int32_t) * ns},
        [&] {
            hipError_t e = launch_ptlk_classify(st, c->d_ptab.p, c->np, d.cpu, d.mem, d.gpu, d.wall, d.part, d.nk, kmax,
                                                J, out, outs, c->jcomp.p);
            if (e == hipSuccess)
                e = launch_joblists(st, c->jcomp.p, J, C, c->jls.p, g, jbd, jbd + C + 1, c->jl.p, c->jpk.p);
            return e;
        },
        [&]() -> int {
            if (c->h_jls.p[1]) return fail(FIT_E_INVAL, "a job has a negative demand or nodes_k > kmax");
            S.rejected = c->h_jls.p[0];
            for (int k = 0; k < C; ++k) maxlen = std::max(maxlen, c->h_jls.p[2 + k + 1] - c->h_jls.p[2 + k]);
            if (maxlen <= 0) return kTlNoWrite;
            HIP_TRY(hipMemsetAsync(c->ptlk_cnt.p, 0, sizeof(int32_t), st));
            return 0;
        },
        {c->h_ptlk.p, c->ptlk_cnt.p, sizeof(int32_t)},
        [&](int& kept) {
            const int threads = ptlk_threads(c->cls_maxn);
            const ExplainComps ec = query_comps(c);
            hipError_t e = hipSuccess;
            int32_t done = 0;
            for (; done < maxlen && e == hipSuccess; done += chunk)
                e = launch_ptlk_commit(st, threads, c->tlhdr.p, c->slab.p, ec, H, c->tl_slot_min, c->jl.p, jbd, done,
                                       chunk, d.cpu, d.mem, d.gpu, d.wall, d.part, d.nk, kmax, out, outs,
                                       c->ptlk_cnt.p);
            if (e != hipSuccess && done <= chunk)
                kept = fail(FIT_E_HIP, "k_ptlk_commit launch failed: %s", hipGetErrorString(e));
            return e;
        },
        &S.ms_device);
    if (rc) return rc;
    if (maxlen > 0) S.placed = c->h_ptlk.p[0];
    S.unplaced = J - S.placed - S.rejected;
    S.ms_total = now_ms() - t0;
// ... 200 lines not shown
}

template <class Row, class Impl, class Bad>
int query_device(fit_ctx* c, QueryBufs<Row>& Q, int32_t j, const JobCols& d, Row* out, Impl impl, Bad bad) {
    HIP_TRY(hipSetDevice(c->device));
    if (Q.bad.ensure(1) || Q.h.ensure(1)) return FIT_E_OOM;
    HIP_TRY(hipEventRecord(c->ev[0], c->st));
    const int rc = impl(c, j, d, out, Q.bad.p);
    if (rc) return rc;
    HIP_TRY(hipEventRecord(c->ev[1], c->st));
    HIP_TRY(hipMemcpyAsync(Q.h.p, Q.bad.p, sizeof(int32_t), hipMemcpyDeviceToHost, c->st));
    HIP_TRY(hipStreamSynchronize(c->st));
    if (Q.h.p[0].code) return bad();
    float ms = 0.f;
    HIP_TRY(hipEventElapsedTime(&ms, c->ev[0], c->ev[1]));
    Q.ms = ms;
    return 0;
}

int bad_explain_job() { return fail(FIT_E_INVAL, "a job has a negative demand or nodes_k > %d", FIT_MAX_K); }
int bad_when_job() { return fail(FIT_E_INVAL, "a job has a negative demand"); }
int bad_room_job() { return fail(FIT_E_INVAL, "a job has a negative demand"); }

int load_timeline_impl(fit_ctx* c, int32_t slots, int32_t slot_min, int64_t ne) {
    if (c->tlhdr.ensure(std::max(c->nn, 1)) ||
        c->slab.ensure((size_t)std::max(c->nn, 1) * TL_MAX_SLOTS) || c->tl_err.ensure(1) ||
        c->h_tl_err.ensure(1))
        return FIT_E_OOM;
    c->have_vtl = false;
    HIP_TRY(hipMemsetAsync(c->tl_err.p, 0, 4, c->st));
    HIP_TRY(launch_build_tl(c->st, c->col_cpu.p, c->col_mem.p, c->col_gpu.p, c->col_av.p,
                            c->col_mask.p, c->perm.p, c->nn, slots, slot_min, ne >= 0 ? c->rel_off.p : nullptr,
                            c->rel_slot.p, c->rel_cpu.p, c->rel_mem.p, c->rel_gpu.p, c->slab.p,
                            c->tlhdr.p, c->tl_err.p));
    HIP_TRY(hipMemcpyAsync(c->h_tl_err.p, c->tl_err.p, 4, hipMemcpyDeviceToHost, c->st));
    HIP_TRY(hipStreamSynchronize(c->st));
    if (c->h_tl_err.p[0])
        return fail(FIT_E_INVAL, "release events: slots must be non-decreasing per node and "
                                 "amounts >= 0");
    c->tl_slots = slots;
    c->tl_slot_min = slot_min;
    c->have_tl = true;
    return 0;
}

int check_timeline_args(fit_ctx* c, int32_t slots, int32_t slot_min) {
    if (!c) return fail(FIT_E_INVAL, "null ctx");
    if (!c->have_nodes) return fail(FIT_E_STATE, "fit_load_nodes not called");
    if (slots < 1 || slots > TL_MAX_SLOTS || slot_min < 1)
        return fail(FIT_E_INVAL, "horizon of %d slots x %d min (1..%d slots)", slots, slot_min,
                    TL_MAX_SLOTS);
    if (c->nn > (int32_t)TL_POS_MASK)
        return fail(FIT_E_INVAL, "%d nodes: the timeline key's %d-bit position holds at most %d", c->nn,
                    TL_POS_BITS, (int32_t)TL_POS_MASK);
    return 0;
}

}

extern "C" {

int fit_abi_version(void) { return FITGPU_ABI_VERSION; }

int fit_lock_dir(char* buf, int32_t buflen) {
    std::string dir;
    const int shared = resolve_lock_dir(dir);
    if (!buf || buflen <= (int32_t)dir.size()) return fail(FIT_E_INVAL, "fit_lock_dir: buffer too small");
    memcpy(buf, dir.c_str(), dir.size() + 1);
    return shared;
}

const char* fit_strerror(int code) {
    switch (code) {
        case FIT_OK: return "ok";
        case FIT_E_INVAL: return "invalid argument";
        case FIT_E_HIP: return "HIP runtime error";
        case FIT_E_RCCL: return "RCCL error";
        case FIT_E_OOM: return "out of memory";
        case FIT_E_NODEV: return "no usable gfx950 device";
        case FIT_E_STATE: return "call out of order";
        case FIT_E_PARSE: return "parse error";
        case FIT_E_UNLIMITED: return "duration is unlimited";
        default: return "unknown error";
    }
}

const char* fit_last_error(void) { return g_last_error.c_str(); }

int fit_nccl_unique_id(void* out128) {
    if (!out128) return fail(FIT_E_INVAL, "null id buffer");
    ncclUniqueId id;
    NCCL_TRY(ncclGetUniqueId(&id));
    static_assert(sizeof(ncclUniqueId) == 128, "ncclUniqueId size");
    memcpy(out128, &id, sizeof id);
    return 0;
}

int fit_create(const fit_opts* opts, fit_ctx** out_ctx) {
    if (!out_ctx) return fail(FIT_E_INVAL, "null out_ctx");
    *out_ctx = nullptr;
    fit_opts o;
    memset(&o, 0, sizeof o);
    o.device = -1;
    o.world = 1;
    if (opts) o = *opts;
    if (o.world < 1 || o.rank < 0 || o.rank >= o.world)
        return fail(FIT_E_INVAL, "rank %d / world %d", o.rank, o.world);
    int ndev = 0;
    if (hipGetDeviceCount(&ndev) != hipSuccess || ndev == 0)
        return fail(FIT_E_NODEV, "no HIP device visible");
    int dev = o.device;
    if (dev < 0 && hipGetDevice(&dev) != hipSuccess) dev = 0;
    if (dev >= ndev) return fail(FIT_E_INVAL, "device %d of %d", dev, ndev);
    hipDeviceProp_t prop;
    HIP_TRY(hipGetDeviceProperties(&prop, dev));
    if (strncmp(prop.gcnArchName, "gfx950", 6) != 0)
        return fail(FIT_E_NODEV, "device %d is %s, this build targets gfx950", dev,
                    prop.gcnArchName);
    HIP_TRY(hipSetDevice(dev));
    fit_ctx* c = new (std::nothrow) fit_ctx();
    if (!c) return fail(FIT_E_OOM, "context allocation");
    c->device = dev;
    c->cus = prop.multiProcessorCount;
    if (const char* ev = getenv("FIT_WATCHDOG_MS"))
        c->wd_ticks = (unsigned)std::min<double>(4.29e9, std::max(1.0, atof(ev) * 1e5));
    if (const char* ev = getenv("FIT_SMALL_BATCH")) c->small_batch = atoi(ev);
    if (const char* ev = getenv("FIT_SMALL_DIRECT")) c->small_direct = atoi(ev);
    if (const char* ev = getenv("FIT_SMALL_ARGS")) c->small_args = atoi(ev) != 0;
    if (const char* ev = getenv("FIT_SYNC_SPIN")) c->sync_spin = atoi(ev) != 0;
    if (const char* ev = getenv("FIT_CLASS")) c->cls_mode = atoi(ev) ? 1 : 0;
    if (const char* ev = getenv("FIT_ENGINE")) {
        c->persistent = strcmp(ev, "rounds") != 0;
        if (strcmp(ev, "persistent") == 0 || strcmp(ev, "class") == 0) c->small_batch = -1;
        c->small_direct = strcmp(ev, "direct") == 0 ? INT32_MAX : -1;
        c->cls_mode = strcmp(ev, "class") == 0 ? 2 : 0;
    }
    c->rank = o.rank;
    c->world = o.world;
    c->force_coll = (o.flags & FIT_FLAG_COLLECTIVES) != 0;
    c->shard_mode = o.shard_mode;
    c->xchg = o.exchange;
    c->xchg_user = o.exchange_user;
    if (o.window_min > 0) c->wmin = o.window_min;
    if (o.window_max > 0) c->wmax = std::max(o.window_max, c->wmin);
    for (int p = 0; p < 32; ++p) {
        c->comp_of_part[p] = -1;
        c->ptab[p] = c->ptab[32 + p] = c->ptab[64 + p] = -1;
        c->ptab[96 + p] = -1;
    }
    int rc = 0;
    if (hipStreamCreateWithFlags(&c->st, hipStreamNonBlocking) != hipSuccess) rc = FIT_E_HIP;
    for (auto& e : c->ev)
        if (!rc && hipEventCreate(&e) != hipSuccess) rc = FIT_E_HIP;
    if (!rc && c->world == 1 && c->force_coll && !c->xchg) {
        ncclUniqueId id;
        ncclResult_t r = ncclGetUniqueId(&id);
        if (r == ncclSuccess) r = ncclCommInitRank(&c->comm, 1, id, 0);
        if (r != ncclSuccess) rc = fail(FIT_E_RCCL, "ncclCommInitRank(1 rank): %s", ncclGetErrorString(r));
    } else if (!rc && c->world > 1 && !c->xchg) {
        if (!o.nccl_id) {
            rc = fail(FIT_E_INVAL, "world > 1 needs nccl_id");
        } else {
            ncclUniqueId id;
            memcpy(&id, o.nccl_id, sizeof id);
            ncclResult_t r = ncclCommInitRank(&c->comm, c->world, id, c->rank);
            if (r != ncclSuccess)
                rc = fail(FIT_E_RCCL, "ncclCommInitRank: %s", ncclGetErrorString(r));
        }
    } else if (rc) {
        fail(rc, "stream/event creation failed");
    }
    if (rc) {
        delete c;
        return rc;
    }
    *out_ctx = c;
    return 0;
}

int fit_set_watchdog_us(fit_ctx* c, int64_t us) {
    if (!c) return fail(FIT_E_INVAL, "null ctx");
    if (us <= 0) {
        c->wd_ticks = 1000000000u;
        if (const char* ev = getenv("FIT_WATCHDOG_MS"))
            c->wd_ticks = (unsigned)std::min<double>(4.29e9, std::max(1.0, atof(ev) * 1e5));
        return 0;
    }
    c->wd_ticks = (unsigned)std::min<int64_t>(us * 100, 4290000000ll);
    return 0;
}

void fit_destroy(fit_ctx* ctx) {
    if (!ctx) return;
    (void)hipSetDevice(ctx->device);
    (void)hipStreamSynchronize(ctx->st);
    delete ctx;
}

static int load_node_cols(fit_ctx* c, int32_t n, const int32_t* cpu, const int32_t* mem, const int32_t* gpu,
                          const int32_t* av, const uint32_t* mask, hipMemcpyKind kind) {
    if (!c) return fail(FIT_E_INVAL, "null ctx");
    if (n < 0 || n > FIT_MAX_NODES || (n > 0 && (!cpu || !mem || !gpu || !av || !mask)))
        return fail(FIT_E_INVAL, "bad node arrays");
    c->have_nodes = c->have_tl = false;
    c->have_vic = c->have_vtl = false;
    HIP_TRY(hipSetDevice(c->device));
    if (alloc_cols(c, n)) return FIT_E_OOM;
    const size_t b = sizeof(int32_t) * n;
    HIP_TRY(hipMemcpyAsync(c->col_cpu.p, cpu, b, kind, c->st));
    HIP_TRY(hipMemcpyAsync(c->col_mem.p, mem, b, kind, c->st));
    HIP_TRY(hipMemcpyAsync(c->col_gpu.p, gpu, b, kind, c->st));
    HIP_TRY(hipMemcpyAsync(c->col_av.p, av, b, kind, c->st));
    HIP_TRY(hipMemcpyAsync(c->col_mask.p, mask, b, kind, c->st));
    return 0;
}

int fit_load_nodes(fit_ctx* c, int32_t n, const int32_t* cpu, const int32_t* mem,
                   const int32_t* gpu, const int32_t* av, const uint32_t* mask) {
    const int rc = load_node_cols(c, n, cpu, mem, gpu, av, mask, hipMemcpyHostToDevice);
    if (rc) return rc;
    c->h_mask.assign(mask, mask + n);
    return load_nodes_common(c, n);
}

int fit_load_nodes_device(fit_ctx* c, int32_t n, const int32_t* cpu, const int32_t* mem,
                          const int32_t* gpu, const int32_t* av, const uint32_t* mask) {
    const int rc = load_node_cols(c, n, cpu, mem, gpu, av, mask, hipMemcpyDeviceToDevice);
    if (rc) return rc;
    c->h_mask.resize(n);
    HIP_TRY(hipMemcpyAsync(c->h_mask.data(), mask, sizeof(uint32_t) * n, hipMemcpyDeviceToHost, c->st));
    HIP_TRY(hipStreamSynchronize(c->st));
    return load_nodes_common(c, n);
}

int fit_load_partitions(fit_ctx* c, int32_t p, const int32_t* max_time,
                        const int32_t* max_cpus, const int32_t* max_mem) {
    if (!c) return fail(FIT_E_INVAL, "null ctx");
    if (p < 0 || p > FIT_MAX_PARTITIONS || (p > 0 && (!max_time || !max_cpus || !max_mem)))
        return fail(FIT_E_INVAL, "bad partition table (p=%d)", p);
    HIP_TRY(hipSetDevice(c->device));
    c->np = p;
    for (int i = 0; i < 32; ++i) {
        c->ptab[i] = i < p ? max_time[i] : -1;
        c->ptab[32 + i] = i < p ? max_cpus[i] : -1;
        c->ptab[64 + i] = i < p ? max_mem[i] : -1;
    }
    int rc = build_ptab(c);
    if (rc) return rc;
    HIP_TRY(hipStreamSynchronize(c->st));
    return 0;
}

static int check_place_args(fit_ctx* c, int32_t j, std::initializer_list<const void*> arrays, int32_t kmax) {
    const int rc = check_job_args(c, j, arrays, nullptr, 0);
    if (rc) return rc;
    if (kmax < 1 || kmax > FIT_MAX_K)
        return fail(FIT_E_INVAL, "kmax=%d outside [1, %d]", kmax, FIT_MAX_K);
    return 0;
}

constexpr int32_t kPackJobs = 16384;

int fit_place(fit_ctx* c, int32_t j, const int32_t* cpu, const int32_t* mem, const int32_t* gpu,
              const int32_t* wall, const uint16_t* part, const uint16_t* nk, int32_t kmax,
              int32_t* out, fit_stats* stats) {
    int rc = check_place_args(c, j, {cpu, mem, gpu, wall, part, out}, kmax);
    if (rc) return rc;
    HIP_TRY(hipSetDevice(c->device));
    size_t m = std::max(j, 1);
    if (c->out.ensure(m * kmax + 2 + FIT_MAX_PARTITIONS + 1)) return FIT_E_OOM;
    if (c->small_args && j <= SMALL_ARGJ && j <= c->small_direct && !c->collective()) {
        SmallBatch hb;
        memcpy(hb.cpu, cpu, sizeof(int32_t) * j);
        memcpy(hb.mem, mem, sizeof(int32_t) * j);
        memcpy(hb.gpu, gpu, sizeof(int32_t) * j);
        memcpy(hb.wall, wall, sizeof(int32_t) * j);
        memcpy(hb.part, part, sizeof(uint16_t) * j);
        if (nk) memcpy(hb.nk, nk, sizeof(uint16_t) * j);
        bool done = false;
        rc = place_impl(c, j, nullptr, nullptr, nullptr, nullptr, nullptr, nk, kmax, c->out.p, stats, out, &done,
                        &hb);
        if (rc) return rc;
        if (!done) return fail(FIT_E_HIP, "direct placement did not return its placements");
        return 0;
    }
    JobCols d;
    rc = j <= kPackJobs ? stage_packed(c, j, cpu, mem, gpu, wall, part, nk, d)
                        : stage_columns(c, j, cpu, mem, gpu, wall, part, true, nk, d);
    if (rc) return rc;
    bool done = false;
    rc = place_impl(c, j, d.cpu, d.mem, d.gpu, d.wall, d.part, d.nk, kmax, c->out.p, stats, out, &done);
    if (rc) return rc;
    if (done) return 0;
    HIP_TRY(hipMemcpyAsync(out, c->out.p, sizeof(int32_t) * j * kmax, hipMemcpyDeviceToHost,
                           c->st));
    HIP_TRY(hipStreamSynchronize(c->st));
    return 0;
}

int fit_place_device(fit_ctx* c, int32_t j, const int32_t* cpu, const int32_t* mem,
                     const int32_t* gpu, const int32_t* wall, const uint16_t* part,
                     const uint16_t* nk, int32_t kmax, int32_t* out, fit_stats* stats) {
    int rc = check_place_args(c, j, {cpu, mem, gpu, wall, part, out}, kmax);
    if (rc) return rc;
    HIP_TRY(hipSetDevice(c->device));
    rc = place_impl(c, j, cpu, mem, gpu, wall, part, nk, kmax, out, stats);
    if (rc) return rc;
    HIP_TRY(hipStreamSynchronize(c->st));
    return 0;
}

int fit_explain(fit_ctx* c, int32_t j, const int32_t* cpu, const int32_t* mem, const int32_t* gpu,
                const int32_t* wall, const uint16_t* part, const uint16_t* nk, fit_why* out) {
    const int rc = check_job_args(c, j, {cpu, mem, gpu, wall, part, out}, "fit_explain", -1);
    if (rc || j == 0) return rc;
    return query_host(c, c->ex, j, cpu, mem, gpu, wall, part, nk, out, explain_impl, bad_explain_job);
}

int fit_explain_device(fit_ctx* c, int32_t j, const int32_t* cpu, const int32_t* mem, const int32_t* gpu,
                       const int32_t* wall, const uint16_t* part, const uint16_t* nk, fit_why* out) {
    const int rc = check_job_args(c, j, {cpu, mem, gpu, wall, part, out}, "fit_explain", -1);
    if (rc || j == 0) return rc;
    return query_device(c, c->ex, j, {cpu, mem, gpu, wall, part, nk}, out, explain_impl, bad_explain_job);
}

int fit_explain_ms(fit_ctx* c, double* ms) {
    if (!c || !ms) return fail(FIT_E_INVAL, "null argument");
    if (c->ex.ms < 0) return fail(FIT_E_STATE, "no fit_explain_device yet");
    *ms = c->ex.ms;
    return 0;
}

int fit_when(fit_ctx* c, int32_t j, const int32_t* cpu, const int32_t* mem, const int32_t* gpu,
             const int32_t* wall, const uint16_t* part, fit_eta* out) {
    const int rc = check_job_args(c, j, {cpu, mem, gpu, wall, part, out}, "fit_when", 1);
    if (rc || j == 0) return rc;
    return query_host(c, c->wh, j, cpu, mem, gpu, wall, part, nullptr, out, when_impl, bad_when_job);
}

int fit_when_device(fit_ctx* c, int32_t j, const int32_t* cpu, const int32_t* mem, const int32_t* gpu,
                    const int32_t* wall, const uint16_t* part, fit_eta* out) {
    const int rc = check_job_args(c, j, {cpu, mem, gpu, wall, part, out}, "fit_when", 1);
    if (rc || j == 0) return rc;
    return query_device(c, c->wh, j, {cpu, mem, gpu, wall, part, nullptr}, out, when_impl, bad_when_job);
}

int fit_when_ms(fit_ctx* c, double* ms) {
    if (!c || !ms) return fail(FIT_E_INVAL, "null argument");
    if (c->wh.ms < 0) return fail(FIT_E_STATE, "no fit_when_device yet");
    *ms = c->wh.ms;
    return 0;
}

static int check_when_k_args(fit_ctx* c, int32_t j, std::initializer_list<const void*> arrays, int32_t kmax) {
    const int rc = check_job_args(c, j, arrays, "fit_when_k", 1);
    if (rc) return rc;
    if (kmax < 1 || kmax > FIT_MAX_K) return fail(FIT_E_INVAL, "kmax=%d (1..%d)", kmax, FIT_MAX_K);
    return 0;
}

static int bad_when_k_job() { return fail(FIT_E_INVAL, "a job has a negative demand or nodes_k > kmax"); }

int fit_when_k(fit_ctx* c, int32_t j, const int32_t* cpu, const int32_t* mem, const int32_t* gpu,
               const int32_t* wall, const uint16_t* part, const uint16_t* nk, int32_t kmax, fit_eta_k* out,
               int32_t* out_node) {
    const int rc = check_when_k_args(c, j, {cpu, mem, gpu, wall, part, out, out_node}, kmax);
    if (rc || j == 0) return rc;
    const size_t nn = (size_t)j * kmax;
    if (c->wk_node.ensure(nn) || c->h_wk_node.ensure(nn)) return FIT_E_OOM;
    const int r = query_host(
        c, c->wk, j, cpu, mem, gpu, wall, part, nk, out,
        [&](fit_ctx* x, int32_t n, const JobCols& d, fit_eta_k* rows, int32_t* bad) {
            const int e = when_k_impl(x, n, d, kmax, rows, x->wk_node.p, bad);
            if (e) return e;
            HIP_TRY(hipMemcpyAsync(x->h_wk_node.p, x->wk_node.p, sizeof(int32_t) * nn, hipMemcpyDeviceToHost, x->st));
            return 0;
        },
        bad_when_k_job);
    if (r) return r;
    memcpy(out_node, c->h_wk_node.p, sizeof(int32_t) * nn);
    return 0;
}

int fit_when_k_device(fit_ctx* c, int32_t j, const int32_t* cpu, const int32_t* mem, const int32_t* gpu,
                      const int32_t* wall, const uint16_t* part, const uint16_t* nk, int32_t kmax, fit_eta_k* out,
// ... 507 lines not shown

int fit_unplace_tl_device(fit_ctx* c, int32_t j, const int32_t* cpu, const int32_t* mem, const int32_t* gpu,
                          const int32_t* wall, const uint16_t* nk, int32_t kmax, const int32_t* node,
                          const int32_t* start, int64_t* applied) {
    const int rc = check_tl_rows_args(c, j, {cpu, mem, gpu, wall, node, start}, kmax, "fit_unplace_tl");
    if (rc) return rc;
    if (j == 0) {
        if (applied) *applied = 0;
        return 0;
    }
    HIP_TRY(hipSetDevice(c->device));
    return unplace_tl_impl(c, j, {cpu, mem, gpu, wall, nk, kmax, node, start}, applied);
}

int fit_unplace_tl_ms(fit_ctx* c, double* ms) { return tl_ms_get(c, &fit_ctx::utl_ms, "fit_unplace_tl", ms); }

int fit_hold_tl(fit_ctx* c, int32_t j, const int32_t* cpu, const int32_t* mem, const int32_t* gpu,
                const int32_t* wall, const uint16_t* nk, int32_t kmax, const int32_t* node, const int32_t* start,
                int32_t* out_state, int64_t* applied, int64_t* refused) {
    int rc = check_tl_rows_args(c, j, {cpu, mem, gpu, wall, node, start, out_state}, kmax, "fit_hold_tl");
    if (rc) return rc;
    if (j == 0) {
        if (applied) *applied = 0;
        if (refused) *refused = 0;
        return 0;
    }
    HIP_TRY(hipSetDevice(c->device));
    TlRows r;
    rc = stage_rows(c, j, cpu, mem, gpu, wall, nk, kmax, node, start, r);
    if (rc) return rc;
    if (c->tlr_state.ensure(j)) return FIT_E_OOM;
    rc = hold_tl_impl(c, j, r, c->tlr_state.p, applied, refused);
    if (rc) return rc;
    HIP_TRY(hipMemcpyAsync(out_state, c->tlr_state.p, sizeof(int32_t) * (size_t)j, hipMemcpyDeviceToHost, c->st));
    HIP_TRY(hipStreamSynchronize(c->st));
    return 0;
}

int fit_hold_tl_device(fit_ctx* c, int32_t j, const int32_t* cpu, const int32_t* mem, const int32_t* gpu,
                       const int32_t* wall, const uint16_t* nk, int32_t kmax, const int32_t* node,
                       const int32_t* start, int32_t* out_state, int64_t* applied, int64_t* refused) {
    const int rc = check_tl_rows_args(c, j, {cpu, mem, gpu, wall, node, start, out_state}, kmax, "fit_hold_tl");
    if (rc) return rc;
    if (j == 0) {
        if (applied) *applied = 0;
        if (refused) *refused = 0;
        return 0;
    }
    HIP_TRY(hipSetDevice(c->device));
    return hold_tl_impl(c, j, {cpu, mem, gpu, wall, nk, kmax, node, start}, out_state, applied, refused);
}

int fit_hold_tl_ms(fit_ctx* c, double* ms) { return tl_ms_get(c, &fit_ctx::htl_ms, "fit_hold_tl", ms); }

static int check_advance_tl_args(fit_ctx* c, int32_t a, const int32_t* tc, const int32_t* tm, const int32_t* tg) {
    const int rc = check_job_args(c, 0, {}, "fit_advance_tl", 1);
    if (rc) return rc;
    if (a < 0) return fail(FIT_E_INVAL, "a=%d", a);
    if (a > 0 && ((!tc != !tm) || (!tc != !tg))) return fail(FIT_E_INVAL, "some but not all tail pointers are NULL");
    return 0;
}

int fit_advance_tl(fit_ctx* c, int32_t a, const int32_t* tc, const int32_t* tm, const int32_t* tg) {
    const int rc = check_advance_tl_args(c, a, tc, tm, tg);
    if (rc || a == 0) return rc;
    HIP_TRY(hipSetDevice(c->device));
    if (!tc || c->n == 0) return advance_tl_impl(c, a, nullptr, nullptr, nullptr);
    const size_t m = c->n, b = sizeof(int32_t) * m;
    if (c->atl_tc.ensure(m) || c->atl_tm.ensure(m) || c->atl_tg.ensure(m)) return FIT_E_OOM;
    HIP_TRY(hipMemcpyAsync(c->atl_tc.p, tc, b, hipMemcpyHostToDevice, c->st));
    HIP_TRY(hipMemcpyAsync(c->atl_tm.p, tm, b, hipMemcpyHostToDevice, c->st));
    HIP_TRY(hipMemcpyAsync(c->atl_tg.p, tg, b, hipMemcpyHostToDevice, c->st));
    return advance_tl_impl(c, a, c->atl_tc.p, c->atl_tm.p, c->atl_tg.p);
}

int fit_advance_tl_device(fit_ctx* c, int32_t a, const int32_t* tc, const int32_t* tm, const int32_t* tg) {
    const int rc = check_advance_tl_args(c, a, tc, tm, tg);
    if (rc || a == 0) return rc;
    HIP_TRY(hipSetDevice(c->device));
    return advance_tl_impl(c, a, tc, tm, tg);
}

int fit_advance_tl_ms(fit_ctx* c, double* ms) { return tl_ms_get(c, &fit_ctx::atl_ms, "fit_advance_tl", ms); }

static int free_tl_impl(fit_ctx* c, int32_t parts, fit_free* rows) {
    static_assert(sizeof(fit_free) == FREE_ROW_BYTES, "fit_free is 40 bytes");
    const size_t n = (size_t)parts * c->tl_slots;
    if (c->free_acc.ensure(n * (FREE_ROW_BYTES / sizeof(int64_t)))) return FIT_E_OOM;
    int32_t chunk = FREE_CHUNK;
    if (const char* e = getenv("FIT_FREE_CHUNK")) chunk = std::max(1, std::min(atoi(e), FREE_MAX_CHUNK));
    HIP_TRY(hipEventRecord(c->ev[0], c->st));
    HIP_TRY(launch_free_tl(c->st, c->tlhdr.p, c->slab.p, c->nn, c->tl_slots, parts, chunk, c->free_acc.p, rows));
    HIP_TRY(hipEventRecord(c->ev[1], c->st));
    return 0;
}
static int free_tl_done(fit_ctx* c) {
    float ms = 0.f;
    HIP_TRY(hipStreamSynchronize(c->st));
    HIP_TRY(hipEventElapsedTime(&ms, c->ev[0], c->ev[1]));
    c->free_ms = ms;
    return 0;
}
static int check_free_tl_args(fit_ctx* c, int32_t parts, const fit_free* out) {
    if (!c || !out) return fail(FIT_E_INVAL, "null argument");
    if (parts < 1 || parts > 32) return fail(FIT_E_INVAL, "parts=%d (1..32)", parts);
    return check_job_args(c, 0, {}, "fit_free_tl", 1);
}

int fit_free_tl(fit_ctx* c, int32_t parts, fit_free* out) {
    int rc = check_free_tl_args(c, parts, out);
    if (rc) return rc;
    HIP_TRY(hipSetDevice(c->device));
    const size_t n = (size_t)parts * c->tl_slots;
    if (c->free_rows.ensure(n)) return FIT_E_OOM;
    rc = free_tl_impl(c, parts, c->free_rows.p);
    if (rc) return rc;
    HIP_TRY(hipMemcpyAsync(out, c->free_rows.p, sizeof(fit_free) * n, hipMemcpyDeviceToHost, c->st));
    return free_tl_done(c);
}

int fit_free_tl_device(fit_ctx* c, int32_t parts, fit_free* out) {
    int rc = check_free_tl_args(c, parts, out);
    if (rc) return rc;
    if ((uintptr_t)out & 7u) return fail(FIT_E_INVAL, "out is not 8-byte aligned");
    HIP_TRY(hipSetDevice(c->device));
    rc = free_tl_impl(c, parts, out);
    return rc ? rc : free_tl_done(c);
}

int fit_free_tl_ms(fit_ctx* c, double* ms) { return tl_ms_get(c, &fit_ctx::free_ms, "fit_free_tl", ms); }

int fit_read_timeline(fit_ctx* c, int32_t* cpu, int32_t* mem, int32_t* gpu) {
    if (!c) return fail(FIT_E_INVAL, "null ctx");
    if (!c->have_tl) return fail(FIT_E_STATE, "fit_load_timeline not called");
    if (c->n > 0 && (!cpu || !mem || !gpu)) return fail(FIT_E_INVAL, "null output");
    HIP_TRY(hipSetDevice(c->device));
    const size_t cells = (size_t)c->n * c->tl_slots;
    DBuf<int32_t> d[3];
    for (auto& x : d)
        if (x.ensure(std::max<size_t>(cells, 1))) return FIT_E_OOM;
    int rc = 0;
    for (auto& x : d)
        if (hipMemsetAsync(x.p, 0xff, sizeof(int32_t) * cells, c->st) != hipSuccess) rc = FIT_E_HIP;
    if (rc || launch_expand_tl(c->st, c->perm.p, c->slab.p, c->tlhdr.p, c->nn, c->tl_slots, d[0].p,
                         d[1].p, d[2].p) != hipSuccess ||
        hipMemcpyAsync(cpu, d[0].p, sizeof(int32_t) * cells, hipMemcpyDeviceToHost, c->st) != hipSuccess ||
        hipMemcpyAsync(mem, d[1].p, sizeof(int32_t) * cells, hipMemcpyDeviceToHost, c->st) != hipSuccess ||
        hipMemcpyAsync(gpu, d[2].p, sizeof(int32_t) * cells, hipMemcpyDeviceToHost, c->st) != hipSuccess ||
        hipStreamSynchronize(c->st) != hipSuccess)
        rc = fail(FIT_E_HIP, "timeline read-back failed");
    return rc;
}

}

namespace fitgpu {
void set_last_error(const char* msg) { g_last_error = msg; }

int64_t ctx_load_count(const fit_ctx* c) { return c && c->have_nodes ? c->loads : 0; }
int ctx_table(fit_ctx* c, std::vector<int32_t>& cpu, std::vector<int32_t>& mem,
              std::vector<int32_t>& gpu, std::vector<int32_t>& avail, std::vector<uint32_t>& mask) {
    if (!c) return fail(FIT_E_INVAL, "null ctx");
    if (!c->have_nodes) return fail(FIT_E_STATE, "no node table loaded");
    const size_t m = std::max<int32_t>(c->n, 1);
    cpu.resize(m), mem.resize(m), gpu.resize(m), avail.resize(m);
    const int rc = fit_read_nodes(c, cpu.data(), mem.data(), gpu.data());
    if (rc) return rc;
    HIP_TRY(hipMemcpy(avail.data(), c->col_av.p, sizeof(int32_t) * c->n, hipMemcpyDeviceToHost));
    cpu.resize(c->n), mem.resize(c->n), gpu.resize(c->n), avail.resize(c->n);
    mask = c->h_mask;
    return 0;
}
}
```

slurm-bridge-operator_amd/csrc/fit_device.h:

```cpp
#pragma once
#include <hip/hip_runtime_api.h>
#include <hip/hip_vector_types.h>
#include <stdint.h>

namespace fitgpu {

#ifndef FIT_KS
#define FIT_KS 16
#endif
constexpr int KS = FIT_KS;
static_assert(KS >= 2 && KS <= 16 && (KS & (KS - 1)) == 0, "FIT_KS must be a power of two in [2, 16]");
constexpr int SCAN_WAVES = 8;
constexpr int SCAN_JOBS = 64;
#ifndef FIT_MIN_SUB
#define FIT_MIN_SUB 64
#endif
constexpr int MIN_SUB = FIT_MIN_SUB;
#ifndef FIT_MAX_SLICES
#define FIT_MAX_SLICES (128 / FIT_KS)
#endif
constexpr int MAX_SLICES = FIT_MAX_SLICES;
#ifndef FIT_TL_KS
#define FIT_TL_KS 4
#endif
// ... 197 lines not shown
                            int32_t n, int32_t H, int32_t chunk, int32_t* g);
hipError_t launch_utl_group(hipStream_t st, int32_t nn, int32_t H, int32_t slot_min, const int32_t* jcpu,
                            const int32_t* jmem, const int32_t* jgpu, const int32_t* jwall, const uint16_t* jk,
                            int32_t kmax, const int32_t* node, const int32_t* start, int32_t t0, int32_t nj,
                            int32_t windows, int32_t n, const int32_t* inv, int32_t* cnt, int32_t* first,
                            int32_t* fill, int32_t* touched, TlWin* win, int32_t* flag, int32_t* g);
hipError_t launch_utl_chunk(hipStream_t st, TlHdr* hdr, Seg* slab, int32_t nn, int32_t H, int32_t slot_min,
                            const int32_t* jcpu, const int32_t* jmem, const int32_t* jgpu, const int32_t* jwall,
                            const uint16_t* jk, int32_t kmax, const int32_t* node, const int32_t* start, int32_t t0,
                            int32_t nj, int32_t windows, int32_t n, const int32_t* inv, int32_t* cnt, int32_t* first,
                            int32_t* fill, int32_t* touched, TlWin* win, int32_t* g);

hipError_t launch_atl_check(hipStream_t st, const int32_t* tc, const int32_t* tm, const int32_t* tg, int32_t n,
                            int32_t* flag);
hipError_t launch_atl_advance(hipStream_t st, TlHdr* hdr, Seg* slab, int32_t nn, int32_t n, int32_t H, int32_t a,
                              const int32_t* tc, const int32_t* tm, const int32_t* tg);

hipError_t launch_htl_hold(hipStream_t st, TlHdr* hdr, Seg* slab, int32_t nn, int32_t H, int32_t slot_min,
                           const int32_t* jcpu, const int32_t* jmem, const int32_t* jgpu, const int32_t* jwall,
                           const uint16_t* jk, int32_t kmax, const int32_t* node, const int32_t* start, int32_t nj,
                           int32_t windows, int32_t n, const int32_t* inv, int32_t* cnt, int32_t* first,
                           int32_t* fill, int32_t* touched, TlWin* win, int32_t* flag, int32_t* g);
hipError_t launch_htl_final(hipStream_t st, const uint16_t* jk, int32_t kmax, const int32_t* start, int32_t nj,
                            const int32_t* flag, int32_t* out_state, unsigned long long* tot);

constexpr int FREE_ROW_BYTES = 40;
constexpr int FREE_CHUNK = 64;
constexpr int FREE_MAX_CHUNK = 1 << 16;
hipError_t launch_free_tl(hipStream_t st, const TlHdr* hdr, const Seg* slab, int32_t nn, int32_t H, int32_t parts,
                          int32_t chunk, void* scratch, void* out);

enum RoomCode : int32_t {
    ROOM_SOME = LIM_NONE,
    ROOM_PARTITION = LIM_PARTITION,
    ROOM_LIMIT_TIME = LIM_LIMIT_TIME,
    ROOM_LIMIT_CPUS = LIM_LIMIT_CPUS,
    ROOM_LIMIT_MEM = LIM_LIMIT_MEM,
    ROOM_NO_NODES = 5,
    ROOM_NONE = 6,
};
hipError_t launch_room_classify(hipStream_t st, const int32_t* ptab, int32_t np, const int32_t* jcpu,
                                const int32_t* jmem, const int32_t* jgpu, const int32_t* jwall, const uint16_t* jpart,
                                int32_t nj, void* out, int8_t* jcomp, int32_t* bad);
hipError_t launch_room(hipStream_t st, const NodeRec* rec, const ExplainComps& C, const int32_t* jcpu,
                       const int32_t* jmem, const int32_t* jgpu, const int32_t* jwall, const uint16_t* jpart,
                       int32_t nj, const int8_t* jcomp, const int32_t* jl, const int32_t* live, int slices, void* out);

enum PreemptCode : int32_t {
    PRE_FITS = LIM_NONE,
    PRE_PARTITION = LIM_PARTITION,
    PRE_LIMIT_TIME = LIM_LIMIT_TIME,
    PRE_LIMIT_CPUS = LIM_LIMIT_CPUS,
    PRE_LIMIT_MEM = LIM_LIMIT_MEM,
    PRE_NO_NODES = 5,
    PRE_EVICT = 6,
    PRE_NONE = 7,
};
struct alignas(16) VicEnt {
    int32_t prio, cpu, mem, gpu;
};
constexpr int PRE_CHUNK = 16384;
hipError_t launch_vic_check(hipStream_t st, const int32_t* off, int32_t n, int64_t nvic, const int32_t* prio,
                            const int32_t* cpu, const int32_t* mem, const int32_t* gpu, int32_t* bad);
hipError_t launch_vic_build(hipStream_t st, const int32_t* off, const int32_t* prio, const int32_t* cpu,
                            const int32_t* mem, const int32_t* gpu, const int32_t* perm, int32_t nn,
                            const int32_t* voff, VicEnt* vent);
hipError_t launch_preempt_classify(hipStream_t st, const int32_t* ptab, int32_t np, int ncomp, const int32_t* jcpu,
                                   const int32_t* jmem, const int32_t* jgpu, const int32_t* jwall,
                                   const uint16_t* jpart, int32_t nj, void* out, int8_t* jcomp, int32_t* bad);
int preempt_slices(int32_t nj, int32_t maxn, int cus);
size_t preempt_partials(int32_t nj, int slices);
hipError_t launch_preempt(hipStream_t st, const NodeRec* rec, const int32_t* voff, const VicEnt* vent,
                          const ExplainComps& C, const int32_t* jcpu, const int32_t* jmem, const int32_t* jgpu,
                          const int32_t* jwall, const uint16_t* jpart, const int32_t* jprio, int32_t nj,
                          const int8_t* jcomp, const int32_t* jl, const int32_t* live, int slices, void* part,
                          void* out);

hipError_t launch_preempt_k_classify(hipStream_t st, const int32_t* ptab, int32_t np, int ncomp, const int32_t* jcpu,
                                     const int32_t* jmem, const int32_t* jgpu, const int32_t* jwall,
                                     const uint16_t* jpart, const uint16_t* jk, int32_t kmax, int32_t nj, void* out,
                                     int32_t* out_node, int32_t* out_vic, int8_t* jcomp, int32_t* bad);
size_t preempt_k_partials(int32_t nj, int slices, int32_t kmax);
hipError_t launch_preempt_k(hipStream_t st, const NodeRec* rec, const int32_t* voff, const VicEnt* vent,
                            const ExplainComps& C, const int32_t* jcpu, const int32_t* jmem, const int32_t* jgpu,
                            const int32_t* jwall, const uint16_t* jpart, const int32_t* jprio, int32_t kmax,
                            int32_t nj, const int8_t* jcomp, const int32_t* jl, const int32_t* live, int slices,
                            void* part, void* out, int32_t* out_node, int32_t* out_vic);

struct alignas(32) VicTl {
    int32_t prio, end, cpu, mem, gpu, pad[3];
};
hipError_t launch_vtl_check(hipStream_t st, const int32_t* off, int32_t n, int64_t nvic, const int32_t* prio,
                            const int32_t* end, const int32_t* cpu, const int32_t* mem, const int32_t* gpu, int32_t H,
                            int32_t* bad);
hipError_t launch_vtl_build(hipStream_t st, const int32_t* off, const int32_t* prio, const int32_t* end,
                            const int32_t* cpu, const int32_t* mem, const int32_t* gpu, const int32_t* perm, int32_t nn,
                            const int32_t* voff, VicTl* vent);
hipError_t launch_preempt_final(hipStream_t st, const int32_t* jl, const int32_t* live, int32_t nj, int32_t t0,
                                int32_t nt, int ncomp, int slices, const int8_t* jcomp, const void* part, void* out);
hipError_t launch_preempt_tl(hipStream_t st, const TlHdr* hdr, const Seg* slab, const int32_t* voff, const VicTl* vent,
                             const ExplainComps& C, int32_t H, int32_t slot_min, int32_t shift, const int32_t* jcpu,
                             const int32_t* jmem, const int32_t* jgpu, const int32_t* jwall, const uint16_t* jpart,
                             const int32_t* jprio, int32_t nj, const int8_t* jcomp, const int32_t* jl,
                             const int32_t* live, int slices, void* part, void* out);

enum TripSite : unsigned {
    TRIP_NONE = 0,
    TRIP_WORKER_RING = 1,
    TRIP_ROUND_START = 2,
    TRIP_HELPER_TILE = 3,
    TRIP_HELPER_SNAP = 4,
    TRIP_DECIDER_REC = 5,
    TRIP_SINGLE_TILE = 6,
    TRIP_NO_PROGRESS = 7,
    TRIP_NO_KERNEL = 8,
    TRIP_PEER = 9,
};
struct TripRec {
    unsigned claim, site, comp, round;
    unsigned arg, q_head, q_tail, pubt;
    unsigned tdone, need, block, pad;
    unsigned long long waited;
    unsigned long long when;
};


hipError_t launch_scan(int blocks, hipStream_t st, const NodeRec* rec, const int32_t* jl,
                       const int32_t* jcpu, const int32_t* jmem, const int32_t* jgpu,
                       const int32_t* jwall, const uint16_t* jpart, const uint16_t* jk,
                       const CompPlan* plan, int ncomp, uint64_t* cand, uint64_t* bnd,
                       JobRec* wjob);
hipError_t launch_commit(int ncomp, int epl, size_t lds_bytes, hipStream_t st, NodeRec* rec,
                         const CompPlan* plan, const uint64_t* cand, int64_t rank_stride,
                         int nranks, const uint64_t* bnd, const JobRec* wjob, int32_t* out,
                         int kmax, CommitResult* res);
hipError_t launch_prefilter(hipStream_t st, const int32_t* jcpu, const int32_t* jmem,
                            const int32_t* jgpu, const int32_t* jwall, const uint16_t* jpart, const uint16_t* jk,
                            int32_t nj, int32_t kmax, const int32_t* ptab, int32_t np,
                            int32_t* out, int8_t* jcomp, int32_t* jmin = nullptr);
size_t joblists_scratch_ints(int32_t nj);
hipError_t launch_joblists(hipStream_t st, const int8_t* jcomp, int32_t nj, int ncomp,
                           int32_t* scratch, int32_t* g, int32_t* jb, int32_t* mb, int32_t* jl,
                           int32_t* jpk);
hipError_t launch_small_args(hipStream_t st, int ncomp, NodeRec* rec, const SmallComps& C, const int32_t* ptab,
                             int32_t np, const SmallBatch& B, bool has_nk, int32_t nj, int32_t kmax, int32_t* out,
                             int32_t* stat);
hipError_t launch_small(hipStream_t st, int ncomp, NodeRec* rec, const SmallComps& C,
                        const int32_t* ptab, int32_t np, const int32_t* jcpu, const int32_t* jmem,
                        const int32_t* jgpu, const int32_t* jwall, const uint16_t* jpart,
                        const uint16_t* jk, int32_t nj, int32_t kmax, int32_t* out, int32_t* stat);
hipError_t launch_gather_nodes(hipStream_t st, const int32_t* cpu, const int32_t* mem,
                               const int32_t* gpu, const int32_t* av, const uint32_t* mask,
                               const int32_t* perm, int32_t nn, NodeRec* rec);
hipError_t launch_scatter_nodes(hipStream_t st, const NodeRec* rec, int32_t nn, int32_t* cpu,
                                int32_t* mem, int32_t* gpu);
size_t engine_lds_bytes(int32_t max_component_nodes);
size_t class_lds_bytes(int32_t max_component_nodes);
int class_max();
int class_table_slots();
size_t class_slot_bytes();
int class_max_nodes();
hipError_t launch_classify(hipStream_t st, const int8_t* jcomp, const int32_t* jcpu, const int32_t* jmem,
                           const int32_t* jgpu, const uint16_t* jpart, int32_t nj, void* tab, int4* dem,
                           int32_t* ncls, int16_t* jcls);
hipError_t launch_class(hipStream_t st, int ncomp, size_t lds, NodeRec* rec, const int32_t* nbv, uint32_t owned,
                        const int32_t* jb, const int32_t* jl, const int32_t* jwall, const uint16_t* jk,
                        const int16_t* jcls, const int4* dem, const int32_t* ncls, int32_t kmax, int32_t* out,
                        CompOut* co, unsigned* err);
hipError_t launch_class_out(hipStream_t st, int32_t* out, int64_t n, const NodeRec* rec);
size_t engine_ctl_bytes();
size_t engine_ctl_error_offset();
size_t engine_ctl_trip_offset();
size_t engine_ring_bytes();
size_t engine_ring_tasks();
int engine_ring_groups();
int engine_blocks_per_cu(size_t lds);
hipError_t launch_engine(int blocks, size_t lds, hipStream_t st, void* ctl, void* ring,
                         const void* cs, void* co, CompPlan* plans, int ncomp, NodeRec* rec,
                         const int32_t* jl, const int32_t* jcpu, const int32_t* jmem,
                         const int32_t* jgpu, const int32_t* jwall, const uint16_t* jpart,
                         const uint16_t* jk, uint64_t* cand, uint64_t* bnd, JobRec* wjob,
                         int32_t* out, int kmax, int64_t* wbusy, const int32_t* jpk, unsigned wd,
                         const int32_t* jmin, const EngineCompIds& ids);
hipError_t launch_build_tl(hipStream_t st, const int32_t* cpu, const int32_t* mem,
                           const int32_t* gpu, const int32_t* av, const uint32_t* mask,
                           const int32_t* perm, int32_t nn, int32_t H, int32_t slot_min,
                           const int32_t* off, const int32_t* rs, const int32_t* rc,
                           const int32_t* rm, const int32_t* rg, Seg* slab, TlHdr* hdr,
                           uint32_t* err);
hipError_t launch_scan_tl(int blocks, hipStream_t st, const Seg* slab, const TlHdr* hdr,
                          const int32_t* jl, const int32_t* jcpu, const int32_t* jmem,
                          const int32_t* jgpu, const int32_t* jwall, const uint16_t* jpart,
                          const CompPlan* plan, int ncomp, uint64_t* cand, uint64_t* bnd,
                          JobRec* wjob, int32_t H, int32_t slot_min);
size_t commit_tl_lds_bytes(int32_t max_component_nodes);
int commit_tl_runs(int32_t max_component_nodes);
hipError_t launch_commit_tl(int ncomp, int epl, size_t lds, hipStream_t st, Seg* slab,
                            TlHdr* hdr, const CompPlan* plan, const uint64_t* cand,
                            int64_t rank_stride, int nranks, const uint64_t* bnd,
                            const JobRec* wjob, const int32_t* perm, int32_t* out, int32_t* outs,
                            CommitResult* res, int32_t H, int32_t R);
int engine_tl_runs(int32_t max_component_nodes);
size_t engine_tl_lds_bytes(int32_t max_component_nodes);
int engine_tl_blocks_per_cu(size_t lds, int mode);
size_t engine_tl_scan_lds_bytes();
hipError_t launch_engine_tl(int blocks, size_t lds, hipStream_t st, void* ctl, void* ring,
                            const void* cs, void* co, CompPlan* plans, int ncomp, Seg* slab,
                            TlHdr* hdr, const int32_t* jl, const int32_t* jcpu,
                            const int32_t* jmem, const int32_t* jgpu, const int32_t* jwall,
                            const uint16_t* jpart, uint64_t* cand, uint64_t* bnd, JobRec* wjob,
                            const int32_t* perm, int32_t* out, int32_t* outs, int32_t H,
                            int32_t slot_min, int32_t R, int64_t* wbusy, int mode,
                            unsigned* resident, unsigned wd);
hipError_t launch_expand_tl(hipStream_t st, const int32_t* perm, const Seg* slab,
                            const TlHdr* hdr, int32_t nn, int32_t H, int32_t* oc, int32_t* om,
                            int32_t* og);

}
```

slurm-bridge-operator_amd/csrc/fit_kernels.hip:

```cpp
#include "fit_common.h"

namespace fitgpu {

__global__ __launch_bounds__(SCAN_WAVES * 64) void k_scan(
    const NodeRec* __restrict__ rec, const int32_t* __restrict__ jl,
    const int32_t* __restrict__ jcpu, const int32_t* __restrict__ jmem,
    const int32_t* __restrict__ jgpu, const int32_t* __restrict__ jwall,
    const uint16_t* __restrict__ jpart, const uint16_t* __restrict__ jk,
    const CompPlan* __restrict__ plan, int ncomp, uint64_t* __restrict__ cand,
    uint64_t* __restrict__ bnd, JobRec* __restrict__ wjob) {
    __shared__ uint64_t xk[SCAN_WAVES / 2][KS][64];
    const int c = find_comp(plan, ncomp, blockIdx.x);
    const CompPlan P = plan[c];
    const int local = blockIdx.x - P.blk0;
    const int tile = __builtin_amdgcn_readfirstlane(local / P.nslice);
    const int s = __builtin_amdgcn_readfirstlane(local - tile * P.nslice);
    scan_tile<false, KS>(P, tile, s, rec, jl, jcpu, jmem, jgpu, jwall, jpart, jk, cand, bnd, wjob, xk);
}

template <int EPL>
__global__ __launch_bounds__(64) void k_commit(
    NodeRec* __restrict__ rec, const CompPlan* __restrict__ plan,
    const uint64_t* __restrict__ cand, int64_t rank_stride, int nranks,
    const uint64_t* __restrict__ bnd, const JobRec* __restrict__ wjob,
    int32_t* __restrict__ out, int kmax, CommitResult* __restrict__ res) {
    extern __shared__ uint32_t bitmap[];
    const int c = blockIdx.x;
    const CompPlan P = plan[c];
    if (P.w == 0) {
        if (threadIdx.x == 0) res[c] = CommitResult{0, 0, 0, 0};
        return;
    }
    const CommitResult R =
        commit_window<EPL>(c, P, rec, cand, rank_stride, nranks, bnd, wjob, out, kmax, bitmap);
    if (threadIdx.x == 0) res[c] = R;
}

__device__ __forceinline__ int job_code(int q, const int32_t* __restrict__ jcpu, const int32_t* __restrict__ jmem,
                                        const int32_t* __restrict__ jgpu, const int32_t* __restrict__ jwall,
                                        const uint16_t* __restrict__ jpart, const uint16_t* __restrict__ jk,
                                        int32_t kmax, const int32_t* __restrict__ ptab, int32_t np,
                                        bool* rej, int* k) {
    const int p = jpart[q];
    *k = jk ? max((int)jk[q], 1) : 1;
    bool r = p >= np;
    if (!r) {
        const int mt = ptab[p], mc = ptab[32 + p], mm = ptab[64 + p];
        r = (mt >= 0 && jwall[q] > mt) || (mc >= 0 && jcpu[q] > mc) || (mm >= 0 && jmem[q] > mm);
    }
    *rej = r;
    int comp = r ? -2 : ptab[96 + p];
    if (comp >= 0 && *k > 1) comp |= 0x40;
    if (*k > kmax || jcpu[q] < 0 || jmem[q] < 0 || jwall[q] < 0 || (jgpu && jgpu[q] < 0)) comp = -3;
    return comp;
}

template <bool MIN>
__global__ __launch_bounds__(256) void k_prefilter(
    const int32_t* __restrict__ jcpu, const int32_t* __restrict__ jmem,
    const int32_t* __restrict__ jgpu, const int32_t* __restrict__ jwall, const uint16_t* __restrict__ jpart,
    const uint16_t* __restrict__ jk, int32_t nj, int32_t kmax,
    const int32_t* __restrict__ ptab ,
    int32_t np, int32_t* __restrict__ out, int8_t* __restrict__ jcomp, int32_t* __restrict__ jmin) {
    __shared__ int32_t smin[MIN ? 3 * ENGINE_MAXC : 1];
    if constexpr (MIN) {
        if (threadIdx.x < 3 * ENGINE_MAXC) smin[threadIdx.x] = INT32_MAX;
        __syncthreads();
    }
    const int q = blockIdx.x * blockDim.x + threadIdx.x;
    if (q < nj) {
        bool rej;
        int k;
        const int code = job_code(q, jcpu, jmem, jgpu, jwall, jpart, jk, kmax, ptab, np, &rej, &k);
        jcomp[q] = (int8_t)code;
        for (int i = 0; i < kmax; ++i) out[(int64_t)q * kmax + i] = (rej && i < k) ? -2 : -1;
        if constexpr (MIN) {
            if (code >= 0) {
                const int cc = code & 0x3f;
                atomicMin(&smin[3 * cc], jcpu[q]);
                atomicMin(&smin[3 * cc + 1], jmem[q]);
                atomicMin(&smin[3 * cc + 2], jgpu ? jgpu[q] : 0);
            }
        }
    }
    if constexpr (MIN) {
        __syncthreads();
        if (threadIdx.x < 3 * ENGINE_MAXC) {
            const int32_t v = smin[threadIdx.x];
            if (v != INT32_MAX &&
                v < __hip_atomic_load(&jmin[threadIdx.x], __ATOMIC_RELAXED, __HIP_MEMORY_SCOPE_AGENT))
                atomicMin(&jmin[threadIdx.x], v);
        }
    }
}

__global__ void k_gather_nodes(const int32_t* __restrict__ cpu, const int32_t* __restrict__ mem,
                               const int32_t* __restrict__ gpu, const int32_t* __restrict__ av,
                               const uint32_t* __restrict__ mask, const int32_t* __restrict__ perm,
                               int32_t nn, NodeRec* __restrict__ rec) {
    const int i = blockIdx.x * blockDim.x + threadIdx.x;
    if (i >= nn) return;
    const int x = perm[i];
    NodeRec r;
    r.cpu = max(cpu[x], -1);
    r.mem = max(mem[x], -1);
    r.gpu = max(gpu[x], -1);
    r.avail = max(av[x], -1);
    r.mask = mask[x];
    r.orig = x;
    r.pad0 = r.pad1 = 0;
    rec[i] = r;
}

__global__ void k_scatter_nodes(const NodeRec* __restrict__ rec, int32_t nn,
                                int32_t* __restrict__ cpu, int32_t* __restrict__ mem,
                                int32_t* __restrict__ gpu) {
    const int i = blockIdx.x * blockDim.x + threadIdx.x;
    if (i >= nn) return;
    const NodeRec r = rec[i];
    if (r.cpu >= 0) cpu[r.orig] = r.cpu;
    if (r.mem >= 0) mem[r.orig] = r.mem;
    if (r.gpu >= 0) gpu[r.orig] = r.gpu;
}


constexpr int JL_BLOCK = 1024;
constexpr int JL_MAXC = ENGINE_MAXC;

__global__ __launch_bounds__(JL_BLOCK) void k_jl_count(const int8_t* __restrict__ jcomp, int32_t nj,
                                                       int ncomp, int32_t* __restrict__ bc,
                                                       int32_t* __restrict__ bm,
                                                       int32_t* __restrict__ g) {
    __shared__ int32_t wc[JL_BLOCK / 64][JL_MAXC], wm[JL_BLOCK / 64][JL_MAXC];
    const int q = blockIdx.x * JL_BLOCK + threadIdx.x;
    const int wave = threadIdx.x >> 6, lane = threadIdx.x & 63;
    const int k = q < nj ? jcomp[q] : -1;
    const int comp = k >= 0 ? (k & 0x3f) : -1;
    const bool multi = k >= 0 && (k & 0x40);
    for (int cc = 0; cc < ncomp; ++cc) {
        const uint64_t m = __ballot(comp == cc), mm = __ballot(comp == cc && multi);
        if (lane == 0) {
            wc[wave][cc] = __popcll(m);
            wm[wave][cc] = __popcll(mm);
        }
    }
    __shared__ int32_t brj, bbad;
    if (threadIdx.x == 0) brj = bbad = 0;
    __syncthreads();
    const uint64_t rj = __ballot(k == -2), bad = __ballot(k == -3);
    if (lane == 0 && rj) atomicAdd(&brj, (int)__popcll(rj));
    if (lane == 0 && bad) bbad = 1;
    __syncthreads();
    if (threadIdx.x == 0 && brj) atomicAdd(&g[0], brj);
    if (threadIdx.x == 0 && bbad) atomicOr(&g[1], 1);
    if ((int)threadIdx.x < ncomp) {
        int a = 0, b = 0;
        for (int w = 0; w < JL_BLOCK / 64; ++w) {
            a += wc[w][threadIdx.x];
            b += wm[w][threadIdx.x];
        }
        bc[blockIdx.x * JL_MAXC + threadIdx.x] = a;
        bm[blockIdx.x * JL_MAXC + threadIdx.x] = b;
    }
}

__global__ __launch_bounds__(1024) void k_jl_scan(int nblocks, int ncomp, int32_t* __restrict__ bc,
                                                  int32_t* __restrict__ bm, int32_t* __restrict__ jb,
                                                  int32_t* __restrict__ mb) {
    __shared__ int32_t pa[32][JL_MAXC + 1], pb[32][JL_MAXC + 1];
    const int cc = threadIdx.x & 31, r = threadIdx.x >> 5;
    const int chunk = (nblocks + 31) / 32, i0 = r * chunk, i1 = min(nblocks, i0 + chunk);
    int a = 0, b = 0;
    if (cc < ncomp)
        for (int i = i0; i < i1; ++i) {
            a += bc[i * JL_MAXC + cc];
            b += bm[i * JL_MAXC + cc];
        }
    pa[r][cc] = a;
    pb[r][cc] = b;
    __syncthreads();
    if (threadIdx.x < 32) {
        int x = 0, y = 0;
        for (int k = 0; k < 32; ++k) {
            const int u = pa[k][cc], v = pb[k][cc];
            pa[k][cc] = x;
            pb[k][cc] = y;
            x += u;
            y += v;
        }
        pa[0][JL_MAXC] = 0;
        if (cc < ncomp) {
            jb[cc] = x;
            mb[cc] = y;
        }
    }
    __syncthreads();
    if (threadIdx.x == 0) {
        int x = 0, y = 0;
        for (int k = 0; k < ncomp; ++k) {
            const int u = jb[k], v = mb[k];
            jb[k] = x;
            mb[k] = y;
            x += u;
            y += v;
        }
        jb[ncomp] = x;
        mb[ncomp] = y;
    }
    if (cc < ncomp) {
        a = pa[r][cc];
        b = pb[r][cc];
        for (int i = i0; i < i1; ++i) {
            const int u = bc[i * JL_MAXC + cc], v = bm[i * JL_MAXC + cc];
            bc[i * JL_MAXC + cc] = a;
            bm[i * JL_MAXC + cc] = b;
            a += u;
            b += v;
        }
    }
}

__global__ __launch_bounds__(JL_BLOCK) void k_jl_scatter(
    const int8_t* __restrict__ jcomp, int32_t nj, int ncomp, const int32_t* __restrict__ bc,
    const int32_t* __restrict__ bm, const int32_t* __restrict__ jb, const int32_t* __restrict__ mb,
    int32_t* __restrict__ jl, int32_t* __restrict__ jpk) {
    __shared__ int32_t wc[JL_BLOCK / 64][JL_MAXC], wm[JL_BLOCK / 64][JL_MAXC];
    const int q = blockIdx.x * JL_BLOCK + threadIdx.x;
    const int wave = threadIdx.x >> 6, lane = threadIdx.x & 63;
    const int k = q < nj ? jcomp[q] : -1;
    const int comp = k >= 0 ? (k & 0x3f) : -1;
    const bool multi = k >= 0 && (k & 0x40);
    int rank = 0, mrank = 0;
    for (int cc = 0; cc < ncomp; ++cc) {
        const uint64_t m = __ballot(comp == cc), mm = __ballot(comp == cc && multi);
        if (lane == 0) {
            wc[wave][cc] = __popcll(m);
            wm[wave][cc] = __popcll(mm);
        }
        if (comp == cc) {
            rank = __builtin_amdgcn_mbcnt_hi((uint32_t)(m >> 32), __builtin_amdgcn_mbcnt_lo((uint32_t)m, 0));
            mrank = __builtin_amdgcn_mbcnt_hi((uint32_t)(mm >> 32), __builtin_amdgcn_mbcnt_lo((uint32_t)mm, 0));
        }
    }
    __syncthreads();
    if (comp >= 0) {
        int wo = 0, wmo = 0;
        for (int w = 0; w < wave; ++w) {
            wo += wc[w][comp];
            wmo += wm[w][comp];
        }
        const int pos = jb[comp] + bc[blockIdx.x * JL_MAXC + comp] + wo + rank;
        const int before = mb[comp] + bm[blockIdx.x * JL_MAXC + comp] + wmo + mrank;
        jl[pos] = q;
        jpk[pos + 1] = before + (multi ? 1 : 0);
    }
    if (q == 0) jpk[0] = 0;
}
}

namespace fitgpu {

hipError_t launch_scan(int blocks, hipStream_t st, const NodeRec* rec, const int32_t* jl,
                       const int32_t* jcpu, const int32_t* jmem, const int32_t* jgpu,
                       const int32_t* jwall, const uint16_t* jpart, const uint16_t* jk,
// ... 190 lines not shown
            rk[i] = x.mask;
            ro[i] = x.orig;
        }
        for (int base = 0; base < nj; base += SMALL_THREADS) {
            const int q = base + (int)threadIdx.x;
            bool mine = false;
            int k = 1;
            if (q < nj) {
                bool rej;
                const int code = job_code(q, jcpu, jmem, jgpu, jwall, jpart, jk, kmax, ptab, np, &rej, &k);
                mine = code >= 0 && (code & 0x3f) == c;
            }
            const uint64_t m = __ballot(mine);
            if (lane == 0) wcnt[wave] = __popcll(m);
            __syncthreads();
            int off = 0, tot = 0;
#pragma unroll
            for (int w = 0; w < SMALL_THREADS / 64; ++w) {
                const int n = wcnt[w];
                off += w < wave ? n : 0;
                tot += n;
            }
            if (mine) {
                const int at = off + __popcll(m & ((1ull << lane) - 1ull));
                list[at] = q * 32 + k;
                ljob[at] = make_int4(jcpu[q], jmem[q], jgpu[q], jwall[q]);
                lpart[at] = jpart[q];
            }
            __syncthreads();
            for (int t = 0; t < tot; ++t) {
                const int e = list[t];
                const int4 f = ljob[t];
                JobRec J;
                J.q = e >> 5;
                J.cpu = f.x;
                J.mem = f.y;
                J.gpu = f.z;
                J.wall = f.w;
                J.pbit = 1u << lpart[t];
                placed += regs ? small_place_job_regs(rec, nb, rpt, J, e & 31, kmax, out, wmin, sel, rc, rm, rg, ra,
                                                      rk, ro)
                               : small_place_job(rec, nb, ne, J, e & 31, kmax, out, wmin, sel);
            }
            __syncthreads();
        }
    }
    if (threadIdx.x == 0) {
        stat[2 + c] = placed;
        if (c == 0) {
            stat[0] = s_rej;
            stat[1] = 0;
        }
    }
}

__global__ __launch_bounds__(SMALL_THREADS) void k_small(
    NodeRec* rec, SmallComps C, int32_t ncomp, const int32_t* __restrict__ ptab, int32_t np,
    const int32_t* __restrict__ jcpu, const int32_t* __restrict__ jmem,
    const int32_t* __restrict__ jgpu, const int32_t* __restrict__ jwall,
    const uint16_t* __restrict__ jpart, const uint16_t* __restrict__ jk, int32_t nj, int32_t kmax,
    int32_t* __restrict__ out, int32_t* __restrict__ stat) {
    small_body(rec, C, ncomp, ptab, np, jcpu, jmem, jgpu, jwall, jpart, jk, nj, kmax, out, stat);
}

__global__ __launch_bounds__(SMALL_THREADS) void k_small_args(
    NodeRec* rec, SmallComps C, int32_t ncomp, const int32_t* __restrict__ ptab, int32_t np, SmallBatch B,
    int32_t has_nk, int32_t nj, int32_t kmax, int32_t* __restrict__ out, int32_t* __restrict__ stat) {
    __shared__ SmallBatch sb;
    for (int i = threadIdx.x; i < nj; i += SMALL_THREADS) {
        sb.cpu[i] = B.cpu[i];
        sb.mem[i] = B.mem[i];
        sb.gpu[i] = B.gpu[i];
        sb.wall[i] = B.wall[i];
        sb.part[i] = B.part[i];
        sb.nk[i] = B.nk[i];
    }
    __syncthreads();
    small_body(rec, C, ncomp, ptab, np, sb.cpu, sb.mem, sb.gpu, sb.wall, sb.part, has_nk ? sb.nk : nullptr, nj, kmax,
               out, stat);
}

hipError_t launch_small_args(hipStream_t st, int ncomp, NodeRec* rec, const SmallComps& C, const int32_t* ptab,
                             int32_t np, const SmallBatch& B, bool has_nk, int32_t nj, int32_t kmax, int32_t* out,
                             int32_t* stat) {
    if (nj > SMALL_ARGJ) return hipErrorInvalidValue;
    hipLaunchKernelGGL(k_small_args, dim3(ncomp > 0 ? ncomp : 1), dim3(SMALL_THREADS), 0, st, rec, C, ncomp, ptab,
                       np, B, has_nk ? 1 : 0, nj, kmax, out, stat);
    return hipGetLastError();
}

hipError_t launch_small(hipStream_t st, int ncomp, NodeRec* rec, const SmallComps& C,
                        const int32_t* ptab, int32_t np, const int32_t* jcpu, const int32_t* jmem,
                        const int32_t* jgpu, const int32_t* jwall, const uint16_t* jpart,
                        const uint16_t* jk, int32_t nj, int32_t kmax, int32_t* out, int32_t* stat) {
    hipLaunchKernelGGL(k_small, dim3(ncomp > 0 ? ncomp : 1), dim3(SMALL_THREADS), 0, st, rec, C, ncomp, ptab,
                       np, jcpu, jmem, jgpu, jwall, jpart, jk, nj, kmax, out, stat);
    return hipGetLastError();
}

#ifdef FIT_STAMPS
extern "C" int fit_debug_commit_stamps(unsigned long long* out ) {
    return hipMemcpyFromSymbol(out, HIP_SYMBOL(g_stamps), sizeof(g_stamps)) == hipSuccess ? 0 : -2;
}
#endif

hipError_t launch_prefilter(hipStream_t st, const int32_t* jcpu, const int32_t* jmem,
                            const int32_t* jgpu, const int32_t* jwall, const uint16_t* jpart, const uint16_t* jk,
                            int32_t nj, int32_t kmax, const int32_t* ptab, int32_t np,
                            int32_t* out, int8_t* jcomp, int32_t* jmin) {
    if (nj == 0) return hipSuccess;
    if (jmin)
        hipLaunchKernelGGL(k_prefilter<true>, dim3((nj + 255) / 256), dim3(256), 0, st, jcpu, jmem, jgpu,
                           jwall, jpart, jk, nj, kmax, ptab, np, out, jcomp, jmin);
    else
        hipLaunchKernelGGL(k_prefilter<false>, dim3((nj + 255) / 256), dim3(256), 0, st, jcpu, jmem, jgpu,
                           jwall, jpart, jk, nj, kmax, ptab, np, out, jcomp, jmin);
    return hipGetLastError();
}

size_t joblists_scratch_ints(int32_t nj) { return (size_t)2 * ((nj + JL_BLOCK - 1) / JL_BLOCK) * JL_MAXC; }

hipError_t launch_joblists(hipStream_t st, const int8_t* jcomp, int32_t nj, int ncomp,
                           int32_t* scratch, int32_t* g, int32_t* jb, int32_t* mb, int32_t* jl,
                           int32_t* jpk) {
    if (ncomp > JL_MAXC) return hipErrorInvalidValue;
    const int nblocks = (nj + JL_BLOCK - 1) / JL_BLOCK;
    int32_t* bc = scratch;
    int32_t* bm = scratch + (size_t)nblocks * JL_MAXC;
    hipError_t e = hipMemsetAsync(g, 0, 2 * sizeof(int32_t), st);
    if (e != hipSuccess) return e;
    if (nj > 0) {
        hipLaunchKernelGGL(k_jl_count, dim3(nblocks), dim3(JL_BLOCK), 0, st, jcomp, nj, ncomp, bc, bm, g);
    }
    hipLaunchKernelGGL(k_jl_scan, dim3(1), dim3(1024), 0, st, nblocks, ncomp, bc, bm, jb, mb);
    if (nj > 0) {
        hipLaunchKernelGGL(k_jl_scatter, dim3(nblocks), dim3(JL_BLOCK), 0, st, jcomp, nj, ncomp, bc,
                           bm, jb, mb, jl, jpk);
    } else {
        e = hipMemsetAsync(jpk, 0, sizeof(int32_t), st);
        if (e != hipSuccess) return e;
    }
    return hipGetLastError();
}

hipError_t launch_gather_nodes(hipStream_t st, const int32_t* cpu, const int32_t* mem,
                               const int32_t* gpu, const int32_t* av, const uint32_t* mask,
                               const int32_t* perm, int32_t nn, NodeRec* rec) {
    if (nn == 0) return hipSuccess;
    hipLaunchKernelGGL(k_gather_nodes, dim3((nn + 255) / 256), dim3(256), 0, st, cpu, mem, gpu,
                       av, mask, perm, nn, rec);
    return hipGetLastError();
}

hipError_t launch_scatter_nodes(hipStream_t st, const NodeRec* rec, int32_t nn, int32_t* cpu,
                                int32_t* mem, int32_t* gpu) {
    if (nn == 0) return hipSuccess;
    hipLaunchKernelGGL(k_scatter_nodes, dim3((nn + 255) / 256), dim3(256), 0, st, rec, nn, cpu,
                       mem, gpu);
    return hipGetLastError();
}

}
```

slurm-bridge-operator_amd/fitgpu/_lib.py:

```python
from __future__ import annotations

import ctypes as C
import os

_HERE = os.path.dirname(os.path.abspath(__file__))
LIB_PATH = os.environ.get("FITGPU_LIB") or os.path.join(_HERE, "libfitgpu.so")

FIT_OK = 0
FIT_E_INVAL = -1
FIT_E_HIP = -2
FIT_E_RCCL = -3
FIT_E_OOM = -4
FIT_E_NODEV = -5
FIT_E_STATE = -6
FIT_E_PARSE = -7
FIT_E_UNLIMITED = -8
FIT_UNPLACED = -1
FIT_REJECTED = -2

EXPORTS = [
    "fit_create", "fit_destroy", "fit_abi_version", "fit_strerror", "fit_last_error",
    "fit_nccl_unique_id", "fit_load_nodes", "fit_load_nodes_device", "fit_load_partitions",
    "fit_place", "fit_place_device", "fit_read_nodes", "fit_partition_free",
    "fit_parse_duration", "fit_parse_resources", "fit_parse_nodes", "fit_parse_partition",
    "fit_parse_partitions_names", "fit_extract_batch_resources", "fit_apply_spec", "fit_array_len",
    "fit_pod_request", "fit_job_demand", "fit_partition_capacity",
    "fit_load_timeline", "fit_load_timeline_device", "fit_place_tl", "fit_place_tl_device",
    "fit_read_timeline", "fit_ingest_nodes", "fit_expand_hostlist",
    "fit_admitter_create", "fit_admit", "fit_admit_group", "fit_admitter_load_nodes",
    "fit_admitter_partition_free", "fit_admitter_confirm", "fit_admitter_release", "fit_admitter_set_ttl",
    "fit_admitter_reservations", "fit_admitter_pending", "fit_admitter_destroy",
    "fit_array_tasks", "fit_pod_demand", "fit_script_with_nodelist", "fit_partition_limits",
    "fit_node_columns", "fit_node_names", "fit_admitter_load_table", "fit_admitter_generation",
    "fit_admitter_script", "fit_set_max_array_size", "fit_release_events", "fit_set_watchdog_us",
    "fit_lock_dir", "fit_explain", "fit_explain_device", "fit_admitter_explain", "fit_why_message",
    "fit_explain_ms", "fit_when", "fit_when_device", "fit_when_ms", "fit_when_message",
    "fit_room", "fit_room_device", "fit_room_ms", "fit_room_message", "fit_admitter_room",
    "fit_when_k", "fit_when_k_device", "fit_when_k_ms", "fit_when_k_message",
    "fit_place_tl_k", "fit_place_tl_k_device",
    "fit_unplace_tl", "fit_unplace_tl_device", "fit_unplace_tl_ms",
    "fit_advance_tl", "fit_advance_tl_device", "fit_advance_tl_ms",
    "fit_hold_tl", "fit_hold_tl_device", "fit_hold_tl_ms",
    "fit_free_tl", "fit_free_tl_device", "fit_free_tl_ms", "fit_free_message",
    "fit_load_victims", "fit_load_victims_device", "fit_preempt", "fit_preempt_device", "fit_preempt_ms",
    "fit_preempt_message",
    "fit_preempt_k", "fit_preempt_k_device", "fit_preempt_k_ms", "fit_preempt_k_message",
    "fit_load_victims_tl", "fit_load_victims_tl_device", "fit_preempt_tl", "fit_preempt_tl_device",
    "fit_preempt_tl_ms",
]


XCHG_FN = C.CFUNCTYPE(C.c_int, C.c_void_p, C.c_int, C.c_void_p, C.c_int64)
FIT_XCHG_ALLGATHER_U64, FIT_XCHG_MIN_U64, FIT_XCHG_MAX_I32, FIT_XCHG_MIN_I32 = 1, 2, 3, 4
FIT_SHARD_AUTO, FIT_SHARD_NODES, FIT_SHARD_COMPONENTS = 0, 1, 2
FIT_FLAG_COLLECTIVES = 1


class FitOpts(C.Structure):
    _fields_ = [("device", C.c_int32), ("rank", C.c_int32), ("world", C.c_int32),
                ("nccl_id", C.c_void_p), ("shard_mode", C.c_int32), ("window_min", C.c_int32),
                ("window_max", C.c_int32), ("flags", C.c_int32), ("exchange", XCHG_FN),
                ("exchange_user", C.c_void_p)]


class FitStats(C.Structure):
    _fields_ = [("jobs", C.c_int64), ("placed", C.c_int64), ("unplaced", C.c_int64),
                ("rejected", C.c_int64), ("rounds", C.c_int64), ("evals", C.c_int64),
                ("useful_evals", C.c_int64), ("stops_rescan", C.c_int64),
                ("stops_dirty", C.c_int64), ("ms_total", C.c_double), ("ms_scan", C.c_double),
                ("ms_commit", C.c_double), ("ms_exchange", C.c_double), ("ms_device", C.c_double),
                ("shard_mode", C.c_int32),
                ("components", C.c_int32), ("engine", C.c_int32), ("reserved", C.c_int32),
                ("ms_arb_wait", C.c_double)]

    def as_dict(self):
        return {k: getattr(self, k) for k, _ in self._fields_}


FIT_MAX_K = 8
FIT_HOLD_HELD, FIT_HOLD_REFUSED, FIT_HOLD_SKIPPED = 1, 0, -1


class FitAdmitReq(C.Structure):
    _fields_ = [("priority", C.c_int64), ("cpu", C.c_int32), ("mem_mib", C.c_int32),
                ("gpu", C.c_int32), ("wall_min", C.c_int32), ("part", C.c_uint16),
                ("nodes_k", C.c_uint16), ("flags", C.c_uint16), ("reserved", C.c_uint16)]


FIT_REQ_ARRAY = 1


class FitAdmitRes(C.Structure):
    _fields_ = [("node", C.c_int32 * FIT_MAX_K), ("batch", C.c_int64), ("batch_jobs", C.c_int32),
                ("order", C.c_int32), ("ticket", C.c_int64)]


FIT_WHY_FITS, FIT_WHY_PARTITION, FIT_WHY_LIMIT_TIME, FIT_WHY_LIMIT_CPUS = 0, 1, 2, 3
FIT_WHY_LIMIT_MEM, FIT_WHY_NO_NODES, FIT_WHY_RESOURCES = 4, 5, 6


class FitWhy(C.Structure):
    _fields_ = [(n, C.c_int32) for n in ("code", "need", "members", "fit", "short_cpu", "short_mem", "short_gpu",
                                         "short_time")]


FIT_ETA_NOW, FIT_ETA_PARTITION, FIT_ETA_LIMIT_TIME, FIT_ETA_LIMIT_CPUS = 0, 1, 2, 3
FIT_ETA_LIMIT_MEM, FIT_ETA_NO_NODES, FIT_ETA_LATER, FIT_ETA_HORIZON = 4, 5, 6, 7


class FitEta(C.Structure):
    _fields_ = [(n, C.c_int32) for n in ("code", "dur", "start", "node", "wait_min", "members", "hosts", "now")]


class FitEtaK(C.Structure):
    _fields_ = [(n, C.c_int32) for n in ("code", "dur", "need", "start", "wait_min", "members", "hosts", "now",
                                         "ready", "reserved")]


FIT_ROOM_SOME, FIT_ROOM_PARTITION, FIT_ROOM_LIMIT_TIME, FIT_ROOM_LIMIT_CPUS = 0, 1, 2, 3
FIT_ROOM_LIMIT_MEM, FIT_ROOM_NO_NODES, FIT_ROOM_NONE = 4, 5, 6
FIT_ROOM_UNBOUNDED = 2**31 - 1


class FitRoom(C.Structure):
    _fields_ = [("code", C.c_int32), ("members", C.c_int32), ("nodes", C.c_int32), ("best", C.c_int32),
                ("copies", C.c_int64), ("best_node", C.c_int32), ("by_gpu", C.c_int32), ("by_cpu", C.c_int32),
                ("by_mem", C.c_int32)]


FIT_PRE_FITS, FIT_PRE_PARTITION, FIT_PRE_LIMIT_TIME, FIT_PRE_LIMIT_CPUS = 0, 1, 2, 3
FIT_PRE_LIMIT_MEM, FIT_PRE_NO_NODES, FIT_PRE_EVICT, FIT_PRE_NONE = 4, 5, 6, 7


class FitEvict(C.Structure):
    _fields_ = [(n, C.c_int32) for n in ("code", "node", "victims", "top_prio", "members", "fit", "able", "outranked")]


class FitEvictK(C.Structure):
    _fields_ = [(n, C.c_int32) for n in ("code", "need", "evict_nodes", "victims", "top_prio", "members", "fit", "able",
                                         "outranked", "reserved")]


class FitFree(C.Structure):
    _fields_ = [("cpu", C.c_int64), ("mem", C.c_int64), ("gpu", C.c_int64), ("nodes", C.c_int32),
                ("max_cpu", C.c_int32), ("max_mem", C.c_int32), ("max_gpu", C.c_int32)]


FIT_TABLE_STATE = 1
FIT_TABLE_PIN = 2


class FitNodeTable(C.Structure):
    _fields_ = [("n", C.c_int32), ("cpu_free", C.c_void_p), ("mem_free", C.c_void_p), ("gpu_free", C.c_void_p),
                ("avail_min", C.c_void_p), ("part_mask", C.c_void_p), ("names", C.c_char_p), ("flags", C.c_int32),
                ("generation", C.c_int64)]


class FitPodLabels(C.Structure):
    _fields_ = [(n, C.c_char_p) for n in ("nodes", "cpus_per_task", "mem_per_cpu", "ntasks_per_node", "array",
                                          "ntasks")]


class FitResources(C.Structure):
    _fields_ = [("nodes", C.c_int64), ("mem_per_node", C.c_int64), ("cpu_per_node", C.c_int64),
                ("wall_ns", C.c_int64)]


class FitNode(C.Structure):
    _fields_ = [("cpus", C.c_int64), ("memory", C.c_int64), ("gpus", C.c_int64),
                ("allo_cpus", C.c_int64), ("allo_memory", C.c_int64), ("allo_gpus", C.c_int64)]


class FitJobResources(C.Structure):
    _fields_ = [("nodes", C.c_int64), ("cpus_per_task", C.c_int64), ("ntasks", C.c_int64),
                ("ntasks_per_node", C.c_int64), ("mem_per_cpu", C.c_int64), ("wall_ns", C.c_int64),
                ("array", C.c_char * 64)]


_lib = None


def lib() -> C.CDLL:
    global _lib
    if _lib is None:
        if not os.path.exists(LIB_PATH):
            raise ImportError(f"{LIB_PATH} not built: run `make -C slurm-bridge-operator_amd`")
        L = C.CDLL(LIB_PATH)
        P = C.c_void_p
        i32, i64, u16p = C.c_int32, C.c_int64, C.POINTER(C.c_uint16)
        L.fit_strerror.restype = C.c_char_p
        L.fit_strerror.argtypes = [C.c_int]
        L.fit_last_error.restype = C.c_char_p
        L.fit_create.argtypes = [C.POINTER(FitOpts), C.POINTER(P)]
        L.fit_destroy.argtypes = [P]
        L.fit_destroy.restype = None
        L.fit_nccl_unique_id.argtypes = [P]
        if hasattr(L, "fit_set_watchdog_us"):
            L.fit_set_watchdog_us.argtypes = [P, i64]
        if hasattr(L, "fit_lock_dir"):
            L.fit_lock_dir.argtypes = [C.c_char_p, i32]
        for name in ("fit_load_nodes", "fit_load_nodes_device"):
            getattr(L, name).argtypes = [P, i32, P, P, P, P, P]
        L.fit_load_partitions.argtypes = [P, i32, P, P, P]
        for name in ("fit_place", "fit_place_device"):
            getattr(L, name).argtypes = [P, i32, P, P, P, P, P, P, i32, P, C.POINTER(FitStats)]
        for name in ("fit_explain", "fit_explain_device"):
            getattr(L, name).argtypes = [P, i32, P, P, P, P, P, P, P]
        L.fit_admitter_explain.argtypes = [P, C.POINTER(FitAdmitReq), i32, P]
        L.fit_why_message.argtypes = [C.POINTER(FitWhy), C.c_char_p, i32]
        L.fit_explain_ms.argtypes = [P, C.POINTER(C.c_double)]
        for name in ("fit_when", "fit_when_device"):
            getattr(L, name).argtypes = [P, i32, P, P, P, P, P, P]
        L.fit_when_ms.argtypes = [P, C.POINTER(C.c_double)]
        L.fit_when_message.argtypes = [C.POINTER(FitEta), C.c_char_p, i32]
        for name in ("fit_when_k", "fit_when_k_device"):
            getattr(L, name).argtypes = [P, i32, P, P, P, P, P, P, i32, P, P]
        L.fit_when_k_ms.argtypes = [P, C.POINTER(C.c_double)]
        L.fit_when_k_message.argtypes = [C.POINTER(FitEtaK), C.c_char_p, i32]
        for name in ("fit_room", "fit_room_device"):
            getattr(L, name).argtypes = [P, i32, P, P, P, P, P, P]
        L.fit_room_ms.argtypes = [P, C.POINTER(C.c_double)]
        L.fit_room_message.argtypes = [C.POINTER(FitRoom), C.c_char_p, i32]
        L.fit_admitter_room.argtypes = [P, C.POINTER(FitAdmitReq), i32, P]
        L.fit_load_victims.argtypes = [P, P, P, P, P, P]
        L.fit_load_victims_device.argtypes = [P, P, i64, P, P, P, P]
        for name in ("fit_preempt", "fit_preempt_device"):
            getattr(L, name).argtypes = [P, i32, P, P, P, P, P, P, P]
        L.fit_preempt_ms.argtypes = [P, C.POINTER(C.c_double)]
        L.fit_preempt_message.argtypes = [C.POINTER(FitEvict), C.c_char_p, i32]
        for name in ("fit_preempt_k", "fit_preempt_k_device"):
            getattr(L, name).argtypes = [P, i32, P, P, P, P, P, P, P, i32, P, P, P]
        L.fit_preempt_k_ms.argtypes = [P, C.POINTER(C.c_double)]
        L.fit_preempt_k_message.argtypes = [C.POINTER(FitEvictK), C.c_char_p, i32]
        L.fit_load_victims_tl.argtypes = [P, P, P, P, P, P, P]
        L.fit_load_victims_tl_device.argtypes = [P, P, i64, P, P, P, P, P]
        for name in ("fit_preempt_tl", "fit_preempt_tl_device"):
            getattr(L, name).argtypes = [P, i32, P, P, P, P, P, P, P]
        L.fit_preempt_tl_ms.argtypes = [P, C.POINTER(C.c_double)]
        L.fit_read_nodes.argtypes = [P, P, P, P]
        L.fit_load_timeline.argtypes = [P, i32, i32, P, P, P, P, P]
        L.fit_load_timeline_device.argtypes = [P, i32, i32, P, i64, P, P, P, P]
        for name in ("fit_place_tl", "fit_place_tl_device"):
            getattr(L, name).argtypes = [P, i32, P, P, P, P, P, P, P, C.POINTER(FitStats)]
        for name in ("fit_place_tl_k", "fit_place_tl_k_device"):
            getattr(L, name).argtypes = [P, i32, P, P, P, P, P, P, i32, P, P, C.POINTER(FitStats)]
        for name in ("fit_unplace_tl", "fit_unplace_tl_device"):
            getattr(L, name).argtypes = [P, i32, P, P, P, P, P, i32, P, P, C.POINTER(i64)]
        L.fit_unplace_tl_ms.argtypes = [P, C.POINTER(C.c_double)]
        for name in ("fit_advance_tl", "fit_advance_tl_device"):
            getattr(L, name).argtypes = [P, i32, P, P, P]
        L.fit_advance_tl_ms.argtypes = [P, C.POINTER(C.c_double)]
        for name in ("fit_hold_tl", "fit_hold_tl_device"):
            getattr(L, name).argtypes = [P, i32, P, P, P, P, P, i32, P, P, P, C.POINTER(i64), C.POINTER(i64)]
        L.fit_hold_tl_ms.argtypes = [P, C.POINTER(C.c_double)]
        for name in ("fit_free_tl", "fit_free_tl_device"):
            getattr(L, name).argtypes = [P, i32, P]
        L.fit_free_tl_ms.argtypes = [P, C.POINTER(C.c_double)]
        L.fit_free_message.argtypes = [C.POINTER(FitFree), C.c_char_p, i32]
        L.fit_read_timeline.argtypes = [P, P, P, P]
        L.fit_ingest_nodes.argtypes = [C.c_char_p, C.c_char_p, i32, i32, P, P, P, P, P, C.c_char_p, i32]
        L.fit_expand_hostlist.argtypes = [C.c_char_p, C.c_char_p, i32]
        L.fit_partition_free.argtypes = [P, i32, C.POINTER(i64), C.POINTER(i64), C.POINTER(i64)]
        L.fit_admitter_create.argtypes = [P, i32, i32, C.POINTER(P)]
        L.fit_admit.argtypes = [P, C.POINTER(FitAdmitReq), C.POINTER(FitAdmitRes)]
        L.fit_admitter_load_nodes.argtypes = [P, i32, P, P, P, P, P]
        L.fit_admitter_partition_free.argtypes = [P, i32, C.POINTER(i64), C.POINTER(i64),
                                                  C.POINTER(i64)]
        L.fit_admit_group.argtypes = [P, C.POINTER(FitAdmitReq), i32, C.POINTER(FitAdmitRes)]
        for name in ("fit_admitter_confirm", "fit_admitter_release"):
            getattr(L, name).argtypes = [P, i64]
        L.fit_admitter_set_ttl.argtypes = [P, i32]
        L.fit_admitter_reservations.argtypes = [P]
        L.fit_admitter_pending.argtypes = [P]
        L.fit_admitter_destroy.argtypes = [P]
        L.fit_admitter_destroy.restype = None
        L.fit_array_tasks.argtypes = [C.c_char_p, C.POINTER(i64), C.POINTER(i64)]
        L.fit_pod_demand.argtypes = [C.POINTER(FitPodLabels), C.c_char_p, C.c_uint16, i64, C.POINTER(FitAdmitReq),
                                     i32]
        L.fit_script_with_nodelist.argtypes = [C.c_char_p, C.c_char_p, i32, C.POINTER(i32), i32, C.c_char_p, i32]
        L.fit_partition_limits.argtypes = [i64, i64, i64, C.POINTER(i32), C.POINTER(i32), C.POINTER(i32)]
        L.fit_node_columns.argtypes = [C.POINTER(FitNode), i32, C.c_uint32, P, P, P, P, P]
        L.fit_node_names.argtypes = [C.c_char_p, i32, C.c_char_p, i32]
        L.fit_admitter_load_table.argtypes = [P, C.POINTER(FitNodeTable)]
        L.fit_admitter_generation.argtypes = [P]
        L.fit_admitter_generation.restype = i64
        L.fit_admitter_script.argtypes = [P, C.POINTER(i64), i32, C.c_char_p, C.c_char_p, i32, C.POINTER(i32)]
        L.fit_set_max_array_size.argtypes = [i32]
        L.fit_set_max_array_size.restype = i32
        L.fit_release_events.argtypes = [i32, i32, P, P, P, P, P, P, i32, i32, P, P, P, P, P, i32]
        L.fit_parse_duration.argtypes = [C.c_char_p, C.POINTER(i64)]
        L.fit_parse_resources.argtypes = [C.c_char_p, C.POINTER(FitResources)]
        L.fit_parse_nodes.argtypes = [C.c_char_p, C.POINTER(FitNode), i32]
        L.fit_parse_partition.argtypes = [C.c_char_p, C.c_char_p, i32]
        L.fit_parse_partitions_names.argtypes = [C.c_char_p, C.c_char_p, i32]
        L.fit_extract_batch_resources.argtypes = [C.c_char_p, C.POINTER(FitJobResources)]
        L.fit_apply_spec.argtypes = [C.POINTER(FitJobResources), i64, i64, i64, i64, C.c_char_p, i64]
        L.fit_apply_spec.restype = None
        L.fit_array_len.argtypes = [C.c_char_p]
        L.fit_array_len.restype = i64
        L.fit_pod_request.argtypes = [C.POINTER(FitJobResources), C.POINTER(i64), C.POINTER(i64)]
        L.fit_pod_request.restype = None
        L.fit_job_demand.argtypes = [C.POINTER(FitJobResources), C.POINTER(i32), C.POINTER(i32),
                                     C.POINTER(i32), u16p]
        L.fit_partition_capacity.argtypes = [C.POINTER(FitNode), i32, C.POINTER(i64),
                                             C.POINTER(i64), C.POINTER(i64), C.POINTER(i64)]
        L.fit_partition_capacity.restype = None
        _lib = L
    return _lib


class FitError(RuntimeError):
    def __init__(self, code: int, where: str):
        L = lib()
        msg = L.fit_strerror(code).decode()
        detail = (L.fit_last_error() or b"").decode()
        super().__init__(f"{where}: {msg} ({code}): {detail}")
        self.code = code


def check(rc: int, where: str) -> int:
    if rc < 0:
        raise FitError(rc, where)
    return rc
```

Baseline: 39.12 million.

## Cache node partition layout across loads and queue engine resets early

Keeps the partition-component layout (union-find, counts, permutation) across node loads and reuses it when the mask is unchanged. A device-side mask diff kernel handles device-resident inputs, and the reuse path skips the permutation upload and ptab rebuild and waits on a column event instead of a full stream sync. Engine control, ring and bound resets plus the record backup are now queued before job-list building so they can overlap host work. The trade-off is extra state to keep consistent and a memcmp over the mask on every host load; the change also adds a standalone layout API.

```diff
diff --git a/include/fitgpu.h b/include/fitgpu.h
--- a/include/fitgpu.h
+++ b/include/fitgpu.h
@@ -440,6 +440,12 @@
                      int32_t* mem_free, int32_t* gpu_free, int32_t* avail_min,
                      uint32_t* mask);
 
+typedef struct fit_layout fit_layout;
+int fit_layout_create(fit_layout** out);
+void fit_layout_destroy(fit_layout* l);
+int fit_layout_load(fit_layout* l, int32_t n, const uint32_t* part_mask);
+int fit_layout_read(const fit_layout* l, int32_t* comp_of_part, int32_t* nb, int32_t* perm);
+
 #ifdef __cplusplus
 }
 #endif
diff --git a/slurm-bridge-operator_amd/csrc/engine.cpp b/slurm-bridge-operator_amd/csrc/engine.cpp
--- a/slurm-bridge-operator_amd/csrc/engine.cpp
+++ b/slurm-bridge-operator_amd/csrc/engine.cpp
@@ -209,10 +209,84 @@
 
 }
 
+struct NodeLayout {
+    bool lay_ok = false;
+    int32_t n = 0;
+    int32_t nn = 0;
+    int ncomp = 0;
+    int comp_of_part[32];
+    std::vector<int32_t> nb;
+    std::vector<uint32_t> h_mask;
+    bool cls_nodes_ok = false;
+    int32_t cls_maxn = 0;
+
+    bool layout_matches(int32_t n_, const uint32_t* mask) const {
+        return lay_ok && n_ == n && (n_ == 0 || memcmp(mask, h_mask.data(), sizeof(uint32_t) * n_) == 0);
+    }
+    int layout_count(int32_t n_) {
+        lay_ok = false;
+        n = n_;
+        int par[32];
+        for (int i = 0; i < 32; ++i) par[i] = i;
+        bool used[32] = {false};
+        for (int32_t x = 0; x < n; ++x) {
+            uint32_t m = h_mask[x];
+            if (!m) continue;
+            int lo = __builtin_ctz(m);
+            for (uint32_t r = m; r; r &= r - 1) {
+                int b = __builtin_ctz(r);
+                used[b] = true;
+                int ra = find_root(par, lo), rb = find_root(par, b);
+                if (ra != rb) par[std::max(ra, rb)] = std::min(ra, rb);
+            }
+        }
+        int root_comp[32];
+        for (int i = 0; i < 32; ++i) root_comp[i] = -1;
+        ncomp = 0;
+        for (int p = 0; p < 32; ++p) {
+            comp_of_part[p] = -1;
+            if (!used[p]) continue;
+            int r = find_root(par, p);
+            if (root_comp[r] < 0) root_comp[r] = ncomp++;
+            comp_of_part[p] = root_comp[r];
+        }
+        nb.assign(ncomp + 1, 0);
+        for (int32_t x = 0; x < n; ++x)
+            if (h_mask[x]) nb[comp_of_part[__builtin_ctz(h_mask[x])] + 1]++;
+        for (int k = 0; k < ncomp; ++k) {
+            if (nb[k + 1] > MAX_COMPONENT_NODES)
+                return fail(FIT_E_INVAL, "partition component %d has %d nodes (limit %d)", k, nb[k + 1],
+                            MAX_COMPONENT_NODES);
+            nb[k + 1] += nb[k];
+        }
+        nn = nb[ncomp];
+        {
+            int parts_of[32] = {0};
+            for (int p = 0; p < 32; ++p)
+                if (comp_of_part[p] >= 0) ++parts_of[comp_of_part[p]];
+            cls_nodes_ok = ncomp > 0 && ncomp <= 32;
+            cls_maxn = 0;
+            for (int k = 0; k < ncomp; ++k) {
+                const int32_t nk = nb[k + 1] - nb[k];
+                cls_maxn = std::max(cls_maxn, nk);
+                if (parts_of[k] != 1) cls_nodes_ok = false;
+            }
+            if (cls_maxn > class_max_nodes() || class_lds_bytes(cls_maxn) > 160 * 1024) cls_nodes_ok = false;
+        }
+        return 0;
+    }
+    void layout_fill(int32_t* perm) const {
+        std::vector<int32_t> fill(nb.begin(), nb.end() - 1);
+        for (int32_t x = 0; x < n; ++x)
+            if (h_mask[x]) perm[fill[comp_of_part[__builtin_ctz(h_mask[x])]]++] = x;
+    }
+};
+
 struct CtxHandles {
     ncclComm_t comm = nullptr;
     hipStream_t st = nullptr;
     hipEvent_t ev[6] = {};
+    hipEvent_t ev_cols = nullptr;
     hipStream_t st2 = nullptr;
     hipEvent_t ev_join = nullptr;
     unsigned* resident = nullptr;
@@ -223,6 +297,7 @@
         for (auto& e : ev)
             if (e) (void)hipEventDestroy(e);
         if (ev_join) (void)hipEventDestroy(ev_join);
+        if (ev_cols) (void)hipEventDestroy(ev_cols);
         if (resident) (void)hipHostFree(resident);
         if (st2) (void)hipStreamDestroy(st2);
         if (st) (void)hipStreamDestroy(st);
@@ -230,7 +305,7 @@
     }
 };
 
-struct fit_ctx : CtxHandles {
+struct fit_ctx : CtxHandles, NodeLayout {
     int device = 0;
     int rank = 0, world = 1;
     int shard_mode = FIT_SHARD_AUTO;
@@ -246,8 +321,6 @@
     bool small_args = true, sync_spin = true;
     int cls_mode = 3;
     int32_t last_multi = 0;
-    bool cls_nodes_ok = false;
-    int32_t cls_maxn = 0;
     DBuf<int16_t> jcls;
     DBuf<uint8_t> cls_tab;
     DBuf<int4> cls_dem;
@@ -311,17 +384,13 @@
     HBuf<uint64_t> h_count;
     int wmin = 256, wmax = 8192;
 
-    int32_t n = 0;
-    int32_t nn = 0;
-    int ncomp = 0;
-    int comp_of_part[32];
-    std::vector<int32_t> nb;
     DBuf<NodeRec> rec;
     DBuf<int32_t> col_cpu, col_mem, col_gpu, col_av, perm;
     DBuf<uint32_t> col_mask;
     DBuf<int32_t> rb_cpu, rb_mem, rb_gpu;
-    std::vector<uint32_t> h_mask;
-    std::vector<int32_t> h_perm;
+    HBuf<int32_t> h_perm;
+    DBuf<uint32_t> mask_diff;
+    HBuf<uint32_t> h_mask_diff;
     bool have_nodes = false;
     int64_t loads = 0;
 
@@ -360,72 +429,46 @@
     return 0;
 }
 
-int load_nodes_common(fit_ctx* c, int32_t n) {
-    int par[32];
-    for (int i = 0; i < 32; ++i) par[i] = i;
-    bool used[32] = {false};
-    for (int32_t x = 0; x < n; ++x) {
-        uint32_t m = c->h_mask[x];
-        if (!m) continue;
-        int lo = __builtin_ctz(m);
-        for (uint32_t r = m; r; r &= r - 1) {
-            int b = __builtin_ctz(r);
-            used[b] = true;
-            int ra = find_root(par, lo), rb = find_root(par, b);
-            if (ra != rb) par[std::max(ra, rb)] = std::min(ra, rb);
-        }
-    }
-    int root_comp[32];
-    for (int i = 0; i < 32; ++i) root_comp[i] = -1;
-    c->ncomp = 0;
-    for (int p = 0; p < 32; ++p) {
-        c->comp_of_part[p] = -1;
-        if (!used[p]) continue;
-        int r = find_root(par, p);
-        if (root_comp[r] < 0) root_comp[r] = c->ncomp++;
-        c->comp_of_part[p] = root_comp[r];
-    }
-    c->nb.assign(c->ncomp + 1, 0);
-    for (int32_t x = 0; x < n; ++x)
-        if (c->h_mask[x]) c->nb[c->comp_of_part[__builtin_ctz(c->h_mask[x])] + 1]++;
-    for (int k = 0; k < c->ncomp; ++k) {
-        if (c->nb[k + 1] > MAX_COMPONENT_NODES)
-            return fail(FIT_E_INVAL, "partition component %d has %d nodes (limit %d)", k,
-                        c->nb[k + 1], MAX_COMPONENT_NODES);
-        c->nb[k + 1] += c->nb[k];
-    }
-    c->nn = c->nb[c->ncomp];
-    {
-        int parts_of[32] = {0};
-        for (int p = 0; p < 32; ++p)
-            if (c->comp_of_part[p] >= 0) ++parts_of[c->comp_of_part[p]];
-        c->cls_nodes_ok = c->ncomp > 0 && c->ncomp <= 32;
-        c->cls_maxn = 0;
-        for (int k = 0; k < c->ncomp; ++k) {
-            const int32_t nk = c->nb[k + 1] - c->nb[k];
-            c->cls_maxn = std::max(c->cls_maxn, nk);
-            if (parts_of[k] != 1) c->cls_nodes_ok = false;
-        }
-        if (c->cls_maxn > class_max_nodes() || class_lds_bytes(c->cls_maxn) > 160 * 1024)
-            c->cls_nodes_ok = false;
-    }
-    std::vector<int32_t> fill(c->nb.begin(), c->nb.end() - 1), perm(std::max(c->nn, 1));
-    for (int32_t x = 0; x < n; ++x)
-        if (c->h_mask[x]) perm[fill[c->comp_of_part[__builtin_ctz(c->h_mask[x])]]++] = x;
-    if (c->perm.ensure(std::max(c->nn, 1)) || c->rec.ensure(std::max(c->nn, 1))) return FIT_E_OOM;
-    HIP_TRY(hipMemcpyAsync(c->perm.p, perm.data(), sizeof(int32_t) * c->nn, hipMemcpyHostToDevice,
-                           c->st));
+int gather_loaded(fit_ctx* c) {
     HIP_TRY(launch_gather_nodes(c->st, c->col_cpu.p, c->col_mem.p, c->col_gpu.p, c->col_av.p,
                                 c->col_mask.p, c->perm.p, c->nn, c->rec.p));
-    int rc = build_ptab(c);
-    if (rc) return rc;
-    HIP_TRY(hipStreamSynchronize(c->st));
-    perm.resize(c->nn);
-    c->h_perm.swap(perm);
-    c->n = n;
+    return 0;
+}
+
+void nodes_loaded(fit_ctx* c) {
     c->have_nodes = true;
     c->have_tl = false;
     ++c->loads;
+}
+
+int load_nodes_reuse(fit_ctx* c) {
+    const int rc = gather_loaded(c);
+    if (rc) return rc;
+    hipError_t e;
+    if (c->sync_spin) {
+        const double t0 = now_ms();
+        while ((e = hipEventQuery(c->ev_cols)) == hipErrorNotReady && now_ms() - t0 < 2.0) {
+        }
+        if (e != hipErrorNotReady) HIP_TRY(e);
+    }
+    HIP_TRY(hipEventSynchronize(c->ev_cols));
+    nodes_loaded(c);
+    return 0;
+}
+
+int load_nodes_rebuild(fit_ctx* c, int32_t n) {
+    int rc = c->layout_count(n);
+    if (rc) return rc;
+    const size_t m = std::max(c->nn, 1);
+    if (c->h_perm.ensure(m) || c->perm.ensure(m) || c->rec.ensure(m)) return FIT_E_OOM;
+    c->layout_fill(c->h_perm.p);
+    HIP_TRY(hipMemcpyAsync(c->perm.p, c->h_perm.p, sizeof(int32_t) * c->nn, hipMemcpyHostToDevice, c->st));
+    rc = gather_loaded(c);
+    if (!rc) rc = build_ptab(c);
+    if (rc) return rc;
+    HIP_TRY(hipStreamSynchronize(c->st));
+    c->lay_ok = true;
+    nodes_loaded(c);
     return 0;
 }
 
@@ -571,15 +614,17 @@
 
 template <class Launch, class Settle>
 int engine_launch(fit_ctx* c, const std::vector<int32_t>& jb, const EngineComps& E, int workers,
-                  const char* name, Launch launch, Settle settle, fit_stats& S) {
+                  const char* name, Launch launch, Settle settle, fit_stats& S, bool resets_queued = false) {
     const int nc = E.nc;
     hipStream_t st = c->st;
     if (c->ebusy.ensure(2 * workers) || c->h_ebusy.ensure(2 * workers) || c->h_trip.ensure(1))
         return FIT_E_OOM;
     HIP_TRY(hipMemcpyAsync(c->ecs.p, c->h_ecs.p, sizeof(CompState) * nc, hipMemcpyHostToDevice, st));
-    HIP_TRY(hipMemsetAsync(c->ectl.p, 0, engine_ctl_bytes(), st));
-    HIP_TRY(hipMemsetAsync(c->ering.p, 0, engine_ring_bytes(), st));
-    HIP_TRY(hipMemsetAsync(c->bnd.p, 0xff, sizeof(uint64_t) * 2 * nc * E.wcap, st));
+    if (!resets_queued) {
+        HIP_TRY(hipMemsetAsync(c->ectl.p, 0, engine_ctl_bytes(), st));
+        HIP_TRY(hipMemsetAsync(c->ering.p, 0, engine_ring_bytes(), st));
+        HIP_TRY(hipMemsetAsync(c->bnd.p, 0xff, sizeof(uint64_t) * 2 * nc * E.wcap, st));
+    }
     {
         ArbGuard arb;
         int rc = arb.take(c->device);
@@ -610,10 +655,29 @@
     return fold_comp_out(c, jb, E.comps, S);
 }
 
+bool rec_backup_off() {
+    static const bool off = getenv("FIT_REC_BACKUP") && atoi(getenv("FIT_REC_BACKUP")) == 0;
+    return off;
+}
+
+int queue_engine_resets(fit_ctx* c) {
+    hipStream_t st = c->st;
+    const size_t bnds = (size_t)2 * ENGINE_MAXC * std::min(c->wmax, 8192);
+    if (c->rec_bak.ensure(std::max(c->nn, 1)) || c->ectl.ensure(engine_ctl_bytes()) ||
+        c->ering.ensure(engine_ring_bytes()) || c->bnd.ensure(bnds))
+        return FIT_E_OOM;
+    if (!rec_backup_off())
+        HIP_TRY(hipMemcpyAsync(c->rec_bak.p, c->rec.p, sizeof(NodeRec) * c->nn, hipMemcpyDeviceToDevice, st));
+    HIP_TRY(hipMemsetAsync(c->ectl.p, 0, engine_ctl_bytes(), st));
+    HIP_TRY(hipMemsetAsync(c->ering.p, 0, engine_ring_bytes(), st));
+    HIP_TRY(hipMemsetAsync(c->bnd.p, 0xff, sizeof(uint64_t) * bnds, st));
+    return 0;
+}
+
 int run_persistent(fit_ctx* c, const std::vector<int32_t>& jb, const std::vector<char>& owned,
                    const int32_t* cpu, const int32_t* mem, const int32_t* gpu, const int32_t* wall,
                    const uint16_t* part, const uint16_t* nk, int32_t* out, int32_t kmax,
-                   fit_stats& S) {
+                   fit_stats& S, bool resets_queued) {
     hipStream_t st = c->st;
     const EngineComps E = engine_comps(c, jb, owned);
     const int nc = E.nc;
@@ -640,10 +704,12 @@
     EngineCompIds ids;
     memset(&ids, 0, sizeof ids);
     for (int i = 0; i < nc; ++i) ids.id[i] = (int8_t)E.comps[i];
-    static const bool no_backup = getenv("FIT_REC_BACKUP") && atoi(getenv("FIT_REC_BACKUP")) == 0;
-    if (c->rec_bak.ensure(std::max(c->nn, 1))) return FIT_E_OOM;
-    if (!no_backup)
-        HIP_TRY(hipMemcpyAsync(c->rec_bak.p, c->rec.p, sizeof(NodeRec) * c->nn, hipMemcpyDeviceToDevice, st));
+    const bool no_backup = rec_backup_off();
+    if (!resets_queued) {
+        if (c->rec_bak.ensure(std::max(c->nn, 1))) return FIT_E_OOM;
+        if (!no_backup)
+            HIP_TRY(hipMemcpyAsync(c->rec_bak.p, c->rec.p, sizeof(NodeRec) * c->nn, hipMemcpyDeviceToDevice, st));
+    }
     return engine_launch(
         c, jb, E, workers, "placement engine",
         [&]() -> int {
@@ -663,7 +729,7 @@
             HIP_TRY(hipStreamSynchronize(st));
             return trip;
         },
-        S);
+        S, resets_queued);
 }
 
 int run_class(fit_ctx* c, int32_t J, const std::vector<int32_t>& jb, const std::vector<char>& owned,
@@ -941,7 +1007,9 @@
     const bool cls_able = c->cls_nodes_ok && pre_mode != FIT_SHARD_NODES;
     const bool try_cls = (c->cls_mode == 1 || c->cls_mode == 2) && cls_able && (c->cls_mode == 2 || J > c->small_batch);
     bool cls_ok = false;
-    int rc0 = build_job_lists(c, J, S, jb, cpu, mem, gpu, part, try_cls, &cls_ok);
+    const bool resets_queued = c->persistent && pre_mode != FIT_SHARD_NODES && J > c->small_batch;
+    int rc0 = resets_queued ? queue_engine_resets(c) : 0;
+    if (!rc0) rc0 = build_job_lists(c, J, S, jb, cpu, mem, gpu, part, try_cls, &cls_ok);
     if (rc0) return rc0;
     const int32_t live = J - S.rejected;
     if (c->cls_mode == 3 && cls_able && live > c->small_batch && 2 * (int64_t)c->last_multi >= live) {
@@ -977,7 +1045,7 @@
         int rc = run_class(c, J, jb, owned, wall, nk, out, kmax, S);
         if (rc) return rc;
     } else if (c->persistent && !node_sharded && !small) {
-        int rc = run_persistent(c, jb, owned, cpu, mem, gpu, wall, part, nk, out, kmax, S);
+        int rc = run_persistent(c, jb, owned, cpu, mem, gpu, wall, part, nk, out, kmax, S, resets_queued);
         if (rc) return rc;
         S.engine = 1;
     } else {
@@ -1310,7 +1378,7 @@
     std::vector<int32_t> hv((size_t)c->nn + 1, 0);
     if (h_off)
         for (int32_t i = 0; i < c->nn; ++i) {
-            const int32_t x = c->h_perm[i];
+            const int32_t x = c->h_perm.p[i];
             hv[i + 1] = hv[i] + (h_off[x + 1] - h_off[x]);
         }
     c->have_vic = false;
@@ -1352,7 +1420,7 @@
     std::vector<int32_t> hv((size_t)c->nn + 1, 0);
     if (h_off)
         for (int32_t i = 0; i < c->nn; ++i) {
-            const int32_t x = c->h_perm[i];
+            const int32_t x = c->h_perm.p[i];
             hv[i + 1] = hv[i] + (h_off[x + 1] - h_off[x]);
         }
     c->have_vtl = false;
@@ -1859,6 +1927,7 @@
     if (hipStreamCreateWithFlags(&c->st, hipStreamNonBlocking) != hipSuccess) rc = FIT_E_HIP;
     for (auto& e : c->ev)
         if (!rc && hipEventCreate(&e) != hipSuccess) rc = FIT_E_HIP;
+    if (!rc && hipEventCreateWithFlags(&c->ev_cols, hipEventDisableTiming) != hipSuccess) rc = FIT_E_HIP;
     if (!rc && c->world == 1 && c->force_coll && !c->xchg) {
         ncclUniqueId id;
         ncclResult_t r = ncclGetUniqueId(&id);
@@ -1904,14 +1973,16 @@
     delete ctx;
 }
 
-static int load_node_cols(fit_ctx* c, int32_t n, const int32_t* cpu, const int32_t* mem, const int32_t* gpu,
-                          const int32_t* av, const uint32_t* mask, hipMemcpyKind kind) {
+static int check_node_args(fit_ctx* c, int32_t n, const int32_t* cpu, const int32_t* mem, const int32_t* gpu,
+                           const int32_t* av, const uint32_t* mask) {
     if (!c) return fail(FIT_E_INVAL, "null ctx");
     if (n < 0 || n > FIT_MAX_NODES || (n > 0 && (!cpu || !mem || !gpu || !av || !mask)))
         return fail(FIT_E_INVAL, "bad node arrays");
-    c->have_nodes = c->have_tl = false;
-    c->have_vic = c->have_vtl = false;
-    HIP_TRY(hipSetDevice(c->device));
+    return 0;
+}
+
+static int load_node_cols(fit_ctx* c, int32_t n, const int32_t* cpu, const int32_t* mem, const int32_t* gpu,
+                          const int32_t* av, const uint32_t* mask, hipMemcpyKind kind) {
     if (alloc_cols(c, n)) return FIT_E_OOM;
     const size_t b = sizeof(int32_t) * n;
     HIP_TRY(hipMemcpyAsync(c->col_cpu.p, cpu, b, kind, c->st));
@@ -1919,25 +1990,66 @@
     HIP_TRY(hipMemcpyAsync(c->col_gpu.p, gpu, b, kind, c->st));
     HIP_TRY(hipMemcpyAsync(c->col_av.p, av, b, kind, c->st));
     HIP_TRY(hipMemcpyAsync(c->col_mask.p, mask, b, kind, c->st));
-    return 0;
+    HIP_TRY(hipEventRecord(c->ev_cols, c->st));
+    return 0;
+}
+
+static void drop_node_table(fit_ctx* c) {
+    c->have_nodes = c->have_tl = false;
+    c->have_vic = c->have_vtl = false;
 }
 
 int fit_load_nodes(fit_ctx* c, int32_t n, const int32_t* cpu, const int32_t* mem,
                    const int32_t* gpu, const int32_t* av, const uint32_t* mask) {
-    const int rc = load_node_cols(c, n, cpu, mem, gpu, av, mask, hipMemcpyHostToDevice);
-    if (rc) return rc;
-    c->h_mask.assign(mask, mask + n);
-    return load_nodes_common(c, n);
+    int rc = check_node_args(c, n, cpu, mem, gpu, av, mask);
+    if (rc) return rc;
+    drop_node_table(c);
+    HIP_TRY(hipSetDevice(c->device));
+    rc = load_node_cols(c, n, cpu, mem, gpu, av, mask, hipMemcpyHostToDevice);
+    if (!rc) {
+        if (c->layout_matches(n, mask)) {
+            rc = load_nodes_reuse(c);
+        } else {
+            c->lay_ok = false;
+            c->h_mask.assign(mask, mask + n);
+            rc = load_nodes_rebuild(c, n);
+        }
+    }
+    if (rc) c->lay_ok = false;
+    return rc;
+}
+
+static int load_nodes_device(fit_ctx* c, int32_t n, const int32_t* cpu, const int32_t* mem, const int32_t* gpu,
+                             const int32_t* av, const uint32_t* mask) {
+    const bool kept = c->lay_ok && n == c->n;
+    if (kept && n > 0) {
+        if (c->mask_diff.ensure(1) || c->h_mask_diff.ensure(1)) return FIT_E_OOM;
+        HIP_TRY(hipMemsetAsync(c->mask_diff.p, 0, sizeof(uint32_t), c->st));
+        HIP_TRY(launch_mask_diff(c->st, mask, c->col_mask.p, n, c->mask_diff.p));
+        HIP_TRY(hipMemcpyAsync(c->h_mask_diff.p, c->mask_diff.p, sizeof(uint32_t), hipMemcpyDeviceToHost, c->st));
+    }
+    int rc = load_node_cols(c, n, cpu, mem, gpu, av, mask, hipMemcpyDeviceToDevice);
+    if (rc) return rc;
+    if (kept) {
+        if (n > 0) HIP_TRY(hipStreamSynchronize(c->st));
+        if (n == 0 || c->h_mask_diff.p[0] == 0) return load_nodes_reuse(c);
+    }
+    c->lay_ok = false;
+    c->h_mask.resize(n);
+    HIP_TRY(hipMemcpyAsync(c->h_mask.data(), c->col_mask.p, sizeof(uint32_t) * n, hipMemcpyDeviceToHost, c->st));
+    HIP_TRY(hipStreamSynchronize(c->st));
+    return load_nodes_rebuild(c, n);
 }
 
 int fit_load_nodes_device(fit_ctx* c, int32_t n, const int32_t* cpu, const int32_t* mem,
                           const int32_t* gpu, const int32_t* av, const uint32_t* mask) {
-    const int rc = load_node_cols(c, n, cpu, mem, gpu, av, mask, hipMemcpyDeviceToDevice);
-    if (rc) return rc;
-    c->h_mask.resize(n);
-    HIP_TRY(hipMemcpyAsync(c->h_mask.data(), mask, sizeof(uint32_t) * n, hipMemcpyDeviceToHost, c->st));
-    HIP_TRY(hipStreamSynchronize(c->st));
-    return load_nodes_common(c, n);
+    int rc = check_node_args(c, n, cpu, mem, gpu, av, mask);
+    if (rc) return rc;
+    drop_node_table(c);
+    HIP_TRY(hipSetDevice(c->device));
+    rc = load_nodes_device(c, n, cpu, mem, gpu, av, mask);
+    if (rc) c->lay_ok = false;
+    return rc;
 }
 
 int fit_load_partitions(fit_ctx* c, int32_t p, const int32_t* max_time,
@@ -2751,6 +2863,40 @@
     return rc;
 }
 
+struct fit_layout : NodeLayout {
+    std::vector<int32_t> perm;
+};
+
+int fit_layout_create(fit_layout** out) {
+    if (!out) return fail(FIT_E_INVAL, "null out");
+    *out = new (std::nothrow) fit_layout();
+    return *out ? 0 : fail(FIT_E_OOM, "layout allocation");
+}
+
+void fit_layout_destroy(fit_layout* l) { delete l; }
+
+int fit_layout_load(fit_layout* l, int32_t n, const uint32_t* mask) {
+    if (!l || n < 0 || n > FIT_MAX_NODES || (n > 0 && !mask)) return fail(FIT_E_INVAL, "bad layout arguments");
+    if (l->layout_matches(n, mask)) return 1;
+    l->lay_ok = false;
+    l->h_mask.assign(mask, mask + n);
+    const int rc = l->layout_count(n);
+    if (rc) return rc;
+    l->perm.assign(l->nn, 0);
+    l->layout_fill(l->perm.data());
+    l->lay_ok = true;
+    return 0;
+}
+
+int fit_layout_read(const fit_layout* l, int32_t* comp_of_part, int32_t* nb, int32_t* perm) {
+    if (!l || !comp_of_part || !nb || !perm) return fail(FIT_E_INVAL, "null layout argument");
+    if (!l->lay_ok) return fail(FIT_E_STATE, "no layout kept");
+    for (int p = 0; p < 32; ++p) comp_of_part[p] = l->comp_of_part[p];
+    for (int k = 0; k <= l->ncomp; ++k) nb[k] = l->nb[k];
+    if (l->nn) memcpy(perm, l->perm.data(), sizeof(int32_t) * l->nn);
+    return l->ncomp;
+}
+
 }
 
 namespace fitgpu {
diff --git a/slurm-bridge-operator_amd/csrc/fit_device.h b/slurm-bridge-operator_amd/csrc/fit_device.h
--- a/slurm-bridge-operator_amd/csrc/fit_device.h
+++ b/slurm-bridge-operator_amd/csrc/fit_device.h
@@ -373,6 +373,7 @@
 hipError_t launch_gather_nodes(hipStream_t st, const int32_t* cpu, const int32_t* mem,
                                const int32_t* gpu, const int32_t* av, const uint32_t* mask,
                                const int32_t* perm, int32_t nn, NodeRec* rec);
+hipError_t launch_mask_diff(hipStream_t st, const uint32_t* a, const uint32_t* b, int32_t n, uint32_t* flag);
 hipError_t launch_scatter_nodes(hipStream_t st, const NodeRec* rec, int32_t nn, int32_t* cpu,
                                 int32_t* mem, int32_t* gpu);
 size_t engine_lds_bytes(int32_t max_component_nodes);
diff --git a/slurm-bridge-operator_amd/csrc/fit_kernels.hip b/slurm-bridge-operator_amd/csrc/fit_kernels.hip
--- a/slurm-bridge-operator_amd/csrc/fit_kernels.hip
+++ b/slurm-bridge-operator_amd/csrc/fit_kernels.hip
@@ -110,6 +110,13 @@
     r.orig = x;
     r.pad0 = r.pad1 = 0;
     rec[i] = r;
+}
+
+__global__ void k_mask_diff(const uint32_t* __restrict__ a, const uint32_t* __restrict__ b, int32_t n,
+                            uint32_t* __restrict__ flag) {
+    const int i = blockIdx.x * blockDim.x + threadIdx.x;
+    const int d = i < n && a[i] != b[i];
+    if (__syncthreads_or(d) && threadIdx.x == 0) atomicOr(flag, 1u);
 }
 
 __global__ void k_scatter_nodes(const NodeRec* __restrict__ rec, int32_t nn,
@@ -606,6 +613,12 @@
     return hipGetLastError();
 }
 
+hipError_t launch_mask_diff(hipStream_t st, const uint32_t* a, const uint32_t* b, int32_t n, uint32_t* flag) {
+    if (n == 0) return hipSuccess;
+    hipLaunchKernelGGL(k_mask_diff, dim3((n + 255) / 256), dim3(256), 0, st, a, b, n, flag);
+    return hipGetLastError();
+}
+
 hipError_t launch_scatter_nodes(hipStream_t st, const NodeRec* rec, int32_t nn, int32_t* cpu,
                                 int32_t* mem, int32_t* gpu) {
     if (nn == 0) return hipSuccess;
diff --git a/slurm-bridge-operator_amd/fitgpu/_lib.py b/slurm-bridge-operator_amd/fitgpu/_lib.py
--- a/slurm-bridge-operator_amd/fitgpu/_lib.py
+++ b/slurm-bridge-operator_amd/fitgpu/_lib.py
@@ -47,6 +47,7 @@
     "fit_preempt_k", "fit_preempt_k_device", "fit_preempt_k_ms", "fit_preempt_k_message",
     "fit_load_victims_tl", "fit_load_victims_tl_device", "fit_preempt_tl", "fit_preempt_tl_device",
     "fit_preempt_tl_ms",
+    "fit_layout_create", "fit_layout_destroy", "fit_layout_load", "fit_layout_read",
 ]
 
 
@@ -238,6 +239,12 @@
             getattr(L, name).argtypes = [P, i32, P, P, P, P, P, P, P]
         L.fit_preempt_tl_ms.argtypes = [P, C.POINTER(C.c_double)]
         L.fit_read_nodes.argtypes = [P, P, P, P]
+        if hasattr(L, "fit_layout_load"):
+            L.fit_layout_create.argtypes = [C.POINTER(P)]
+            L.fit_layout_destroy.argtypes = [P]
+            L.fit_layout_destroy.restype = None
+            L.fit_layout_load.argtypes = [P, i32, P]
+            L.fit_layout_read.argtypes = [P, P, P, P]
         L.fit_load_timeline.argtypes = [P, i32, i32, P, P, P, P, P]
         L.fit_load_timeline_device.argtypes = [P, i32, i32, P, i64, P, P, P, P]
         for name in ("fit_place_tl", "fit_place_tl_device"):
```

Result: no change. 39.31 million (median of 6 runs) (+0.5%).
